# klindsay28/NK_ocn_tracer_jacobian_precond

Measured on AMD Instinct MI355X. Metric: precond_solve_throughput_1deg_ocean_jacobian, higher is better.
Workload: dtype f64

## Files before the change

### include/nkp.h

```cpp
#ifndef NKP_H
#define NKP_H

#include <stdint.h>

#ifdef __cplusplus
extern "C" {
#endif

#define NKP_VERSION 1

typedef struct nkp_solver nkp_solver;

enum nkp_precond {
   NKP_PRECOND_NONE = 0,
   NKP_PRECOND_COLUMN_JACOBI = 1,
   NKP_PRECOND_MULTILEVEL = 3
};

enum nkp_krylov { NKP_KRYLOV_FGMRES = 0, NKP_KRYLOV_BICGSTAB = 1 };

enum {
   NKP_OK = 0,
   NKP_NOT_CONVERGED = 1,
   NKP_BREAKDOWN = 2,
// ... 11 lines not shown
   int ml_pocket;
   int ml_big_from;
   int ml_coarsest_rows;
   int ml_dense_max;
   double ml_theta;
   double ml_tau;
   int64_t ml_device_min;
   int ml_smooth_coarse;
   int ml_coarse_from;
   int ml_gamma_from, ml_gamma_to;
   int ml_f32;
   int ml_host_inverse;
   int ml_fused;
   int ml_fused_max_cols;
   int ml_wave_fused;
   int ml_coarsest_sweeps;
   int64_t ml_tail_rows;
   double ml_omega;
   int col_ldsres;
   int col_stream;
   int col_stream_min;
   int col_stream_gw;
   int col_wave_max;
   int col_w3;
   int col_group;
   int col_pipe_min;
   int col_ldsres_early;
   int col_ldsres_packed;
   int spmv_variant;
   int spmv_compress;
   int spmv_pipe_min;
   int spmv_run;
   int spmv_wgs;
   int rhs_batch;
   int precond_steps;
   int equil;
   int dist_overlap;
   int dist_ras;
   int force_dist;
   int setup_threads;
   int plan_times;
   int ml_drop_intertracer;
   int dist_one_reduce;
   int ml_huge_from;
   int col_ldsres_min;
   int col_sort_groups;
   int batch_spmv_rows;
   int dist_ras_rings;
   int ml_diag;
   int spmv_diag;
   int ml_lane_fused;
   int dist_smooth_exchange;
   int step_glue;
} nkp_tuning;

int nkp_default_tuning (nkp_tuning *t);

typedef struct nkp_options {
   int struct_size;
   int precond;
   int krylov;
   int restart;
   int max_iters;
   double rtol;
   double atol;
   int device;
   int verbose;
   int rank;
   int reorth;
   int ml_levels;
   int ml_smooth;
   int basis_f32;
   int precond_steps;
   int equil;
   int reserved[4];
   const int32_t *col_i;
   const int32_t *col_j;
   const int32_t *col_t;
   const nkp_tuning *tuning;
} nkp_options;

int nkp_default_options (nkp_options *opt);

int nkp_device_count (void);

int nkp_create (nkp_solver **out, const nkp_options *opt, int64_t n, int64_t nnz,
                const int32_t *rowptr, const int32_t *colind, const double *val,
                const int32_t *blk_start, int64_t nblk, int coupled_tracer_cnt);

int nkp_create64 (nkp_solver **out, const nkp_options *opt, int64_t n, const int64_t *rowptr ,
                  const int32_t *colind, const double *val, const int32_t *blk_start, int64_t nblk, int coupled_tracer_cnt);

int nkp_solve (nkp_solver *s, double *b_in_x_out, int nrhs, int64_t ldb,
               double *berr, int *iters, double *relres);

int nkp_solve_batch_device (nkp_solver *s, int nrhs, const void *d_B, void *d_X, int64_t ldb, double *berr, int *iters, double *relres);

int nkp_solve_device (nkp_solver *s, const void *d_b, void *d_x, int use_guess,
                      double *berr, int *iters, double *relres);

int nkp_spmv (nkp_solver *s, const double *x, double *y);
int nkp_spmv_device (nkp_solver *s, const void *d_x, void *d_y);

int nkp_precond_apply (nkp_solver *s, const double *r, double *z);

int nkp_multi_dot (nkp_solver *s, const double *V, int64_t ld, int k, const double *w, double *out);

int nkp_time_kernel (nkp_solver *s, int which, int arg, int reps, double *avg_ms);

int64_t nkp_get_int (nkp_solver *s, const char *key);

#define NKP_REFACTOR_REBUILD 1
int nkp_refactor (nkp_solver *s, const double *val, int flags);
int nkp_refactor_device (nkp_solver *s, const void *d_val, int flags);

int nkp_refactor_dist (nkp_solver *s, const double *val_loc, int flags);
int nkp_refactor_dist_device (nkp_solver *s, const void *d_val_loc, int flags);

int nkp_set_stream (nkp_solver *s, void *hip_stream);

void nkp_destroy (nkp_solver *s);

const char *nkp_last_error (void);


typedef struct nkp_comm_ops {
   void *ctx;
   int rank, nranks;
   int (*allreduce) (void *ctx, void *dev_buf, int count, int op, void *hip_stream);
   int (*alltoallv) (void *ctx, const void *dev_send, const int *send_counts, void *dev_recv, const int *recv_counts, void *hip_stream);
   int (*alltoallv_i32_host) (void *ctx, const int32_t *send, const int *send_counts, int32_t *recv, const int *recv_counts);
   int (*allgather_i64_host) (void *ctx, int64_t mine, int64_t *all );
} nkp_comm_ops;

int nkp_comm_unique_id (void *id128);
int nkp_comm_rccl_init (nkp_comm_ops *ops, const void *id128, int rank, int nranks);
void nkp_comm_rccl_free (nkp_comm_ops *ops);
int nkp_comm_file_init (nkp_comm_ops *ops, const char *dir, int rank, int nranks);
void nkp_comm_file_free (nkp_comm_ops *ops);

int nkp_create_dist (nkp_solver **out, const nkp_options *opt, int64_t n_global, int64_t fst_row,
                     int64_t m_loc, int64_t nnz_loc, const int32_t *rowptr_loc,
                     const int32_t *colind_glob, const double *val,
                     const int32_t *blk_start_loc, int64_t nblk_loc, int coupled_tracer_cnt,
                     const nkp_comm_ops *comm);

int nkp_cell_major_order (int64_t nblk, const int32_t *blk_start, int cnt, int32_t *perm, int32_t *blk_start_new,
                          int32_t *col_t, int32_t *col_src);
int nkp_permuted_rows (int64_t n, const int32_t *rowptr, const int32_t *colind, const double *val, const int32_t *perm,
                       const int32_t *inv, int64_t r0, int64_t r1, int32_t *rowptr_loc, int32_t *colind_loc, double *val_loc);

int nkp_clone (nkp_solver *src, nkp_solver **out);

int nkp_transpose (nkp_solver *s, nkp_solver **out);

// ... 40 lines not shown
```

### nk_ocn_tracer_jacobian_precond_amd/csrc/blas1.hip

```cpp
#include "nkp_dev.h"

#include <stdint.h>

#define B1_THREADS 256

__device__ __forceinline__ double wave_sum (double v)
{
#pragma unroll
   for (int off = NKP_WAVE / 2; off > 0; off >>= 1) v += __shfl_down (v, off);
   return v;
}

__device__ __forceinline__ double block_sum (double v, double *sh )
{
   v = wave_sum (v);
   const int lane = threadIdx.x & (NKP_WAVE - 1), wv = threadIdx.x / NKP_WAVE;
   __syncthreads ();
   if (lane == 0) sh[wv] = v;
   __syncthreads ();
   double s = 0.0;
   if (threadIdx.x == 0) {
#pragma unroll
      for (int w = 0; w < B1_THREADS / NKP_WAVE; w++) s += sh[w];
   }
// ... 161 lines not shown
}

__global__ __launch_bounds__ (B1_THREADS)
void update_w_group_kernel (GsGroup G, int64_t ld, int k, const double *__restrict__ msg, int64_t n)
{
   __shared__ double hs[B1_MAX_K];
   __shared__ double sh[B1_THREADS / NKP_WAVE];
   const int r = blockIdx.y;
   update_w_body<double, double2> (G.V[r], ld, k, msg + (int64_t) r * (k + 1), G.w[r], n, G.partial[r], -1.0, hs, sh);
}

__device__ __forceinline__ void sum_partials_body (const double *__restrict__ partial, int nblk, double *__restrict__ out)
{
   double s = 0.0;
   for (int b = threadIdx.x; b < nblk; b += NKP_WAVE) s += partial[b];
   s = wave_sum (s);
   if (threadIdx.x == 0) out[0] = s;
}

__global__ __launch_bounds__ (NKP_WAVE)
void sum_partials_kernel (const double *__restrict__ partial, int nblk, double *__restrict__ out)
{
   sum_partials_body (partial, nblk, out);
}

__global__ __launch_bounds__ (NKP_WAVE)
void sum_partials_group_kernel (GsGroup G, int nblk, double *__restrict__ out)
{
   sum_partials_body (G.partial[blockIdx.x], nblk, out + blockIdx.x);
}

void launch_update_w (const void *V, int v_f32, int64_t ld, int k, const double *h, double *w, int64_t n, double *partial, double *out_nrm2, hipStream_t st)
{
   const int g = red_grid (n);
   if (v_f32) hipLaunchKernelGGL ((update_w_kernel<float, float2>), dim3 (g), dim3 (B1_THREADS), 0, st, (const float *) V, ld, k, h, w, n, partial, -1.0);
   else hipLaunchKernelGGL ((update_w_kernel<double, double2>), dim3 (g), dim3 (B1_THREADS), 0, st, (const double *) V, ld, k, h, w, n, partial, -1.0);
   if (out_nrm2) hipLaunchKernelGGL (sum_partials_kernel, dim3 (1), dim3 (NKP_WAVE), 0, st, partial, g, out_nrm2);
}

void launch_update_w_group (int R, const GsGroup &G, int64_t ld, int k, const double *msg, int64_t n, double *nrm2, hipStream_t st)
{
   if (R <= 0) return;
   const int g = red_grid (n);
   hipLaunchKernelGGL (update_w_group_kernel, dim3 (g, R), dim3 (B1_THREADS), 0, st, G, ld, k, msg, n);
   hipLaunchKernelGGL (sum_partials_group_kernel, dim3 (R), dim3 (NKP_WAVE), 0, st, G, g, nrm2);
}

void launch_axpy_multi (const double *Z, int64_t ld, int k, const double *c, double *x, int64_t n, hipStream_t st)
{
   const int g = red_grid (n);
   hipLaunchKernelGGL ((update_w_kernel<double, double2>), dim3 (g), dim3 (B1_THREADS), 0, st, Z, ld, k, c, x, n, (double *) nullptr, 1.0);
}

__device__ __forceinline__ void scale_to_body (const double *__restrict__ x, const double *__restrict__ alpha, double *__restrict__ y, float *__restrict__ yf, int64_t n)
{
   const double a = alpha[0];
   const int64_t stride = (int64_t) gridDim.x * B1_THREADS * 2;
   for (int64_t i = ((int64_t) blockIdx.x * B1_THREADS + threadIdx.x) * 2; i < n; i += stride) {
      if (i + 1 < n) {
         double2 v = *reinterpret_cast<const double2 *> (x + i);
         v.x *= a; v.y *= a;
         *reinterpret_cast<double2 *> (y + i) = v;
         if (yf) *reinterpret_cast<float2 *> (yf + i) = make_float2 ((float) v.x, (float) v.y);
      } else {
         y[i] = a * x[i];
         if (yf) yf[i] = (float) (a * x[i]);
      }
   }
}

__global__ __launch_bounds__ (B1_THREADS)
void scale_to_kernel (const double *__restrict__ x, const double *__restrict__ alpha, double *__restrict__ y, float *__restrict__ yf, int64_t n)
{
   scale_to_body (x, alpha, y, yf, n);
}

__global__ __launch_bounds__ (B1_THREADS)
void scale_to_group_kernel (GsGroup G, const double *__restrict__ inv, int64_t n)
{
   const int r = blockIdx.y;
   scale_to_body (G.w[r], inv + r, G.vnext[r], nullptr, n);
}

void launch_scale_to (const double *x, const double *alpha_dev, double *y, float *yf, int64_t n, hipStream_t st)
{
   hipLaunchKernelGGL (scale_to_kernel, dim3 (red_grid (n)), dim3 (B1_THREADS), 0, st, x, alpha_dev, y, yf, n);
}

void launch_scale_to_group (int R, const GsGroup &G, const double *inv, int64_t n, hipStream_t st)
{
   if (R > 0) hipLaunchKernelGGL (scale_to_group_kernel, dim3 (red_grid (n), R), dim3 (B1_THREADS), 0, st, G, inv, n);
}

__global__ __launch_bounds__ (B1_THREADS)
void axpby_kernel (double a, const double *__restrict__ x, double b, double *__restrict__ y, int64_t n)
{
   const int64_t stride = (int64_t) gridDim.x * B1_THREADS;
   for (int64_t i = (int64_t) blockIdx.x * B1_THREADS + threadIdx.x; i < n; i += stride)
      y[i] = (b == 0.0 ? 0.0 : b * y[i]) + (x ? a * x[i] : a);
}

void launch_axpby (double a, const double *x, double b, double *y, int64_t n, hipStream_t st)
{
   hipLaunchKernelGGL (axpby_kernel, dim3 (red_grid (n) * 2), dim3 (B1_THREADS), 0, st, a, x, b, y, n);
}

// ... 340 lines not shown
```

### nk_ocn_tracer_jacobian_precond_amd/csrc/create.hip

```cpp
#include "solver_impl.h"

#include <limits.h>
#include <math.h>
#include <stdlib.h>
#include <string.h>
#include <time.h>

#include <algorithm>
#include <thread>
#include <vector>

void drop_intertracer (int64_t n, int tracer_cnt, const int32_t *rowptr, const int32_t *colind, const double *val,
                       std::vector<int32_t> &f_rowptr, std::vector<int32_t> &f_colind, std::vector<double> &f_val)
{
   const int64_t tsl = n / tracer_cnt;
   f_rowptr.assign ((size_t) n + 1, 0);
   for (int64_t i = 0; i < n; i++) {
      for (int32_t e = rowptr[i]; e < rowptr[i + 1]; e++)
         if (colind[e] / tsl == i / tsl) { f_colind.push_back (colind[e]); f_val.push_back (val[e]); }
      f_rowptr[(size_t) i + 1] = (int32_t) f_colind.size ();
   }
}

static int alloc_work_vectors (nkp_solver *s, bool member = false)
{
   const size_t ld = (size_t) s->ld, m = (size_t) s->m, nscal = 3 * (m + 2) + 16 + 8;
   const struct { double **p; size_t count; } vec[] = {
      { &s->V, ld * (m + 1) }, { &s->vcur, ld }, { &s->Z, ld * m }, { &s->w, ld }, { &s->r, ld }, { &s->x, ld }, { &s->b, ld }, { &s->t1, ld }, { &s->t2, ld },
      { &s->p1, s->precond_steps > 1 ? ld : 0 }, { &s->p2, s->precond_steps > 1 && !member ? ld : 0 }, { &s->eqtmp, s->equil && !member ? ld : 0 },
      { &s->partial, ((m + 1 + NKP_DOT_CHUNK) / NKP_DOT_CHUNK + 1) * NKP_RED_BLOCKS * (NKP_DOT_CHUNK + 1) }, { &s->dscal, nscal } };
   int rc = NKP_OK;
   for (const auto &v : vec)
      if (v.count && (rc = dev_alloc (s, v.p, v.count))) return rc;
   if ((rc = dev_alloc (s, &s->dint, 8))) return rc;
   HIPCHK (hipHostMalloc ((void **) &s->hpin, (m + 16) * sizeof (double), hipHostMallocDefault));
   HIPCHK (hipMemset (s->dscal, 0, nscal * sizeof (double)));
   return NKP_OK;
}

static void build_matrix_diagonals (nkp_solver *s, const int32_t *blk_start, int64_t nblk)
{
   const int64_t n = s->n;
   if (s->tune.spmv_diag <= 0 || !blk_start || nblk <= 0 || nblk >= INT_MAX || n <= 0 || blk_start[0] != 0 || blk_start[nblk] != n) return;
   int max_len = 0;
   for (int64_t c = 0; c < nblk; c++) {
      const int len = blk_start[c + 1] - blk_start[c];
      if (len <= 0) return;
      max_len = std::max (max_len, len);
   }
   void *d_blk = nullptr;
   const size_t bytes = ((size_t) nblk + 1) * sizeof (int);
   if (hipMalloc (&d_blk, bytes) != hipSuccess || hipMemcpy (d_blk, blk_start, bytes, hipMemcpyHostToDevice) != hipSuccess) {
      if (d_blk) (void) hipFree (d_blk);
      (void) hipGetLastError ();
      return;
   }
   int color_tile[3];
   (void) diag_build (s->A, blk_start, (const int *) d_blk, (int) nblk, (int) nblk, max_len, s->tune.spmv_diag, color_tile, &s->device_bytes, s->stream);
   (void) hipFree (d_blk);
}

static int check_arguments (const nkp_options *opt_in, int64_t n, int64_t nnz, const int32_t *rowptr, const int32_t *colind, const double *val,
                            nkp_options &opt, nkp_tuning &tune)
{
   if (opt_in) {
      if (opt_in->struct_size != (int) sizeof (nkp_options)) return fail (NKP_EINVAL, "nkp_create: nkp_options.struct_size mismatch (%d != %zu)", opt_in->struct_size, sizeof (nkp_options));
      opt = *opt_in;
   } else
      nkp_default_options (&opt);
   if (n < 0 || nnz < 0 || !rowptr || (nnz > 0 && (!colind || !val))) return fail (NKP_EINVAL, "nkp_create: bad matrix arguments");
   if (n >= 2147483647LL || nnz >= 2147483647LL) return fail (NKP_EINVAL, "nkp_create: n/nnz exceed the int32 index schema");
   if (rowptr[0] != 0 || rowptr[n] != nnz) return fail (NKP_EINVAL, "nkp_create: rowptr[0]=%d rowptr[n]=%d inconsistent with nnz=%lld", rowptr[0], rowptr[n], (long long) nnz);
   if (opt.restart < 1) opt.restart = 1;
   if (opt.restart > NKP_MAX_K - 2) opt.restart = NKP_MAX_K - 2;
   if (opt.precond != NKP_PRECOND_NONE && opt.precond != NKP_PRECOND_COLUMN_JACOBI && opt.precond != NKP_PRECOND_MULTILEVEL)
      return fail (NKP_EINVAL, "nkp_create: unknown preconditioner %d", opt.precond);
   { const int trc = resolve_tuning (&opt, &tune); if (trc) return trc; }
   opt.tuning = nullptr;
   return NKP_OK;
}

static int check_rows (const nkp_options &opt, int64_t n, const int32_t *rowptr, const int32_t *colind, const double *val)
{
   struct Bad { int64_t row = -1; int kind = 0; int col = 0; };
   const int nt = (n >= 200000) ? (int) std::min (16u, std::max (1u, std::thread::hardware_concurrency ())) : 1;
   std::vector<Bad> bad ((size_t) nt);
   auto check = [&] (int t) {
      const int64_t r0 = n * t / nt, r1 = n * (t + 1) / nt;
      for (int64_t r = r0; r < r1 && bad[(size_t) t].row < 0; r++) {
         Bad b;
         if (rowptr[r + 1] < rowptr[r]) b.kind = 1;
         else {
            double diag = 0.0;
            for (int e = rowptr[r]; e < rowptr[r + 1] && !b.kind; e++) {
               if (colind[e] < 0 || colind[e] >= n) { b.kind = 2; b.col = colind[e]; }
               else if (opt.precond == NKP_PRECOND_MULTILEVEL && e > rowptr[r] && colind[e] <= colind[e - 1]) b.kind = 4;
               else if (colind[e] == r) diag += val[e];
            }
            if (!b.kind && opt.precond != NKP_PRECOND_NONE && !(diag != 0.0)) b.kind = 3;
         }
         if (b.kind) { b.row = r; bad[(size_t) t] = b; }
      }
   };
   if (nt == 1) check (0);
   else {
      std::vector<std::thread> pool;
      for (int t = 0; t < nt; t++) pool.emplace_back (check, t);
      for (std::thread &th : pool) th.join ();
   }
   for (const Bad &b : bad) {
      if (b.row < 0) continue;
      if (b.kind == 1) return fail (NKP_EINVAL, "nkp_create: rowptr decreases at row %lld", (long long) b.row);
// ... 211 lines not shown
         solver_free (s);
         return rc;
      }
   }
   msg (s, 1, "column blocks: %lld blocks, longest %d rows, in-block half bandwidth %d stored as %d%s\n", (long long) nblk,
        s->B.max_len, meas[0], s->B.P, s->B.dropped ? " (entries beyond the band dropped)" : "");
   return NKP_OK;
}

int create_impl (nkp_solver **out, const nkp_options *opt_in, int64_t n, int64_t nnz,
                 const int32_t *rowptr, const int32_t *colind, const double *val,
                 const int32_t *blk_start, int64_t nblk, int coupled_tracer_cnt, const SpmvMatrixHost *spmv_mat,
                 const PrecondMatrixHost *pm)
{
   if (!out) return fail (NKP_EINVAL, "nkp_create: out is NULL");
   *out = nullptr;
   nkp_options opt;
   nkp_tuning tune;
   std::vector<int> blk_default;
   int rc;
   if ((rc = check_arguments (opt_in, n, nnz, rowptr, colind, val, opt, tune))) return rc;
   if ((rc = check_rows (opt, n, rowptr, colind, val))) return rc;
   if ((rc = check_blocks (opt, n, blk_start, nblk, blk_default))) return rc;

   nkp_solver *s = nullptr;
   if ((rc = new_solver_on_device (opt, tune, &s))) return rc;
   struct timespec ts0_;
   clock_gettime (CLOCK_MONOTONIC, &ts0_);
   auto since0 = [&] () { struct timespec t; clock_gettime (CLOCK_MONOTONIC, &t); return (double) (t.tv_sec - ts0_.tv_sec) + 1e-9 * (double) (t.tv_nsec - ts0_.tv_nsec); };
   if ((rc = configure (s, n))) return rc;

   const SpmvMatrixHost own = { nnz, n, rowptr, colind, val };
   const SpmvMatrixHost &M = spmv_mat ? *spmv_mat : own;
   if ((rc = upload_matrix (s, M, spmv_mat != nullptr))) return rc;
   if (!spmv_mat && blk_default.empty ()) build_matrix_diagonals (s, blk_start, nblk);
   if (s->equil && (rc = upload_row_scales (s, M))) return rc;

   const double t_matrix = since0 ();
   s->vf32 = opt.basis_f32 != 0;
   TRY (alloc_work_vectors (s));

   const double t_work = since0 ();
   if (opt.precond != NKP_PRECOND_NONE && !pm) {
      s->h_blk.assign (blk_start, blk_start + nblk + 1);
      s->tracer_cnt = coupled_tracer_cnt;
      if (blk_default.empty ()) {
         if (opt.col_i) s->h_col_i.assign (opt.col_i, opt.col_i + nblk);
         if (opt.col_j) s->h_col_j.assign (opt.col_j, opt.col_j + nblk);
         if (opt.col_t) s->h_col_t.assign (opt.col_t, opt.col_t + nblk);
      }
   }
   if (opt.precond == NKP_PRECOND_MULTILEVEL &&
       (rc = build_hierarchy (s, n, rowptr, colind, val, blk_start, nblk, blk_default.empty (), coupled_tracer_cnt, !spmv_mat, pm))) return rc;
   if (opt.precond == NKP_PRECOND_COLUMN_JACOBI && (rc = factor_columns (s, blk_start, nblk))) return rc;
   TRYHIP (hipStreamSynchronize (s->stream));
   TRYHIP (hipGetLastError ());
   msg (s, 1, "nkp_create: n = %lld, nnz = %lld, %d SpMV row blocks, %.1f MB on device %d; %.2f s matrix upload + row blocks, %.2f s work vectors, %.2f s preconditioner\n",
        (long long) n, (long long) M.nnz, s->A.nrowblk, (double) s->device_bytes / 1.0e6, s->device, t_matrix, t_work - t_matrix, since0 () - t_work);
   s->create_seconds = since0 ();
   *out = s;
   return NKP_OK;
}

extern "C" int nkp_create (nkp_solver **out, const nkp_options *opt, int64_t n, int64_t nnz,
                           const int32_t *rowptr, const int32_t *colind, const double *val,
                           const int32_t *blk_start, int64_t nblk, int coupled_tracer_cnt)
{
   return create_impl (out, opt, n, nnz, rowptr, colind, val, blk_start, nblk, coupled_tracer_cnt, nullptr);
}

extern "C" int nkp_create64 (nkp_solver **out, const nkp_options *opt, int64_t n, const int64_t *rowptr, const int32_t *colind, const double *val,
                             const int32_t *blk_start, int64_t nblk, int coupled_tracer_cnt)
{
   if (!out) return fail (NKP_EINVAL, "nkp_create64: out is NULL");
   *out = nullptr;
   if (n < 0 || !rowptr) return fail (NKP_EINVAL, "nkp_create64: bad matrix arguments");
   if (n >= 2147483647LL || rowptr[n] >= 2147483647LL || rowptr[n] < 0)
      return fail (NKP_EINVAL, "nkp_create64: %lld rows / %lld entries: one GPU stores entry offsets in 32 bits (at most 2^31 - 1 rows and entries); "
                   "row-partition the system with nkp_create_dist, where the limit applies per rank", (long long) n, (long long) rowptr[n]);
   std::vector<int32_t> rp ((size_t) n + 1);
   for (int64_t r = 0; r <= n; r++) {
      if (rowptr[r] < 0 || rowptr[r] > rowptr[n]) return fail (NKP_EINVAL, "nkp_create64: rowptr[%lld] = %lld out of range", (long long) r, (long long) rowptr[r]);
      rp[(size_t) r] = (int32_t) rowptr[r];
   }
   return create_impl (out, opt, n, rowptr[n], rp.data (), colind, val, blk_start, nblk, coupled_tracer_cnt, nullptr);
}

int clone_impl (nkp_solver *src, nkp_solver **out, bool member)
{
   if (!src || !out) return fail (NKP_EINVAL, "nkp_clone: NULL argument");
   *out = nullptr;
   if (src->dist.on && !member) return fail (NKP_EINVAL, "nkp_clone: not available for the row-distributed flavour");
   if (src->borrowed) return fail (NKP_EINVAL, "nkp_clone: clone the original solver, not a clone");
   if (src->trans_of && !member) return fail (NKP_EINVAL, "nkp_clone: not available on a transposed solver (its owner may free it at a refactor)");
   HIPCHK (hipSetDevice (src->device));
   nkp_solver *s = new (std::nothrow) nkp_solver (*src);
   if (!s) return fail (NKP_ENOMEM, "nkp_clone: out of host memory");
   s->borrowed = true;
   s->rf = nullptr;
   s->shared->clones++;
   s->stagnated = false;
   s->batch_members.clear ();
   s->bvin = s->bz = s->bw = nullptr;
   s->batch_K = 0;
   s->dist.bxe = s->dist.gmsg = s->dist.ghpin = nullptr;
   s->dist.each_exchange ([] (RowExchange &X, bool) { X.drop_wide (); });
   s->dist.bK = s->dist.agreed_K = 0;
   s->dplan = nullptr;
   s->trans = s->trans_of = nullptr;
   s->trans_src = nullptr;
   s->trans_val = nullptr;
   s->trans_map_bytes = 0;
   s->trans_ship = nullptr;
   s->trans_send = s->trans_recv = nullptr;
   s->vg = decltype (s->vg) ();
   s->vp = decltype (s->vp) ();
   s->A.tune = &s->tune;
   s->B.tune = &s->tune;
   s->ml.tune = &s->tune;
   for (MlLevel &L : s->ml.lev) L.L.tune = L.B.tune = &s->tune;
   s->stream = nullptr;
   s->own_stream = false;
   s->device_bytes = 0;
   s->V = s->vcur = s->Z = s->w = s->r = s->x = s->b = s->t1 = s->t2 = s->p1 = s->p2 = s->eqtmp = s->partial = s->dscal = s->hpin = nullptr;
   s->dint = nullptr;
   for (MlLevel &L : s->ml.lev) L.x = L.x2 = L.b = L.r = nullptr;
   int rc = NKP_OK;
   TRYHIP (hipStreamCreateWithFlags (&s->stream, hipStreamNonBlocking));
   s->own_stream = true;
   TRY (alloc_work_vectors (s, member));
   for (MlLevel &L : s->ml.lev) {
      TRY (dev_alloc (s, &L.x, (size_t) L.n));
      TRY (dev_alloc (s, &L.x2, (size_t) L.n));
      TRY (dev_alloc (s, &L.b, (size_t) L.n));
      TRY (dev_alloc (s, &L.r, (size_t) L.n));
      TRYHIP (hipMemset (L.x, 0, (size_t) (L.n ? L.n : 1) * sizeof (double)));
      TRYHIP (hipMemset (L.x2, 0, (size_t) (L.n ? L.n : 1) * sizeof (double)));
      TRYHIP (hipMemset (L.b, 0, (size_t) (L.n ? L.n : 1) * sizeof (double)));
      TRYHIP (hipMemset (L.r, 0, (size_t) (L.n ? L.n : 1) * sizeof (double)));
   }
   *out = s;
   return NKP_OK;
}

#undef TRY
#undef TRYHIP

extern "C" int nkp_clone (nkp_solver *src, nkp_solver **out) { return clone_impl (src, out, false); }
```

### nk_ocn_tracer_jacobian_precond_amd/csrc/diagop.hip

```cpp
#include "nkp_dev.h"
#include "diag_rows.h"
#include "mlsetup.h"

#include <limits.h>

#include <vector>

#define DG_THREADS 256
#define DG_WAVES (DG_THREADS / NKP_WAVE)
#define DG_RPL 4
#define DG_UNROLL 8

__global__ __launch_bounds__ (DG_THREADS)
void diag_keys_kernel (int ncol, const int *__restrict__ blk_start, const int *__restrict__ rowptr, const int *__restrict__ colind, int cap,
                       int *__restrict__ tmpkey, int *__restrict__ cnt)
{
   const int c = blockIdx.x * DG_WAVES + (threadIdx.x >> 6), lane = threadIdx.x & (NKP_WAVE - 1);
   if (c >= ncol) return;
   const int r0 = blk_start[c], len = blk_start[c + 1] - r0;
   int p[DG_RPL], e1[DG_RPL], key[DG_RPL];
#pragma unroll
   for (int j = 0; j < DG_RPL; j++) {
      const int kl = lane + j * NKP_WAVE;
      p[j] = e1[j] = 0;
// ... 3 lines not shown
   int n = 0;
   bool bad = false;
   for (;;) {
      int m = key[0];
#pragma unroll
      for (int j = 1; j < DG_RPL; j++) m = min (m, key[j]);
#pragma unroll
      for (int off = NKP_WAVE / 2; off > 0; off >>= 1) m = min (m, __shfl_xor (m, off));
      if (m == INT_MAX) break;
      if (n < cap && lane == 0) tmpkey[(size_t) c * cap + n] = m;
      if (++n > cap) break;
#pragma unroll
      for (int j = 0; j < DG_RPL; j++)
         if (key[j] == m) {
            p[j]++;
            key[j] = p[j] < e1[j] ? colind[p[j]] - (lane + j * NKP_WAVE) : INT_MAX;
            if (key[j] <= m) bad = true;
         }
   }
   if (__any (bad)) n = cap + 1;
   if (lane == 0) cnt[c] = n;
}

__global__ __launch_bounds__ (DG_THREADS)
void diag_compact_kernel (int ncol, int cap, const int *__restrict__ tmpkey, const int *__restrict__ dg_ptr, int *__restrict__ dg_key)
{
   const int64_t t = (int64_t) blockIdx.x * DG_THREADS + threadIdx.x;
   const int c = (int) (t / cap), i = (int) (t % cap);
   if (c >= ncol) return;
   const int k0 = dg_ptr[c];
   if (i < dg_ptr[c + 1] - k0) dg_key[k0 + i] = tmpkey[t];
}

template <class VT>
__global__ __launch_bounds__ (DG_THREADS)
void diag_fill_kernel (int ntile, const DgTile *__restrict__ tile, const int *__restrict__ rowptr, const int *__restrict__ colind,
                       const VT *__restrict__ valf, const int *__restrict__ dg_key, VT *__restrict__ dg_val)
{
   const int t = blockIdx.x * DG_WAVES + (threadIdx.x >> 6), lane = threadIdx.x & (NKP_WAVE - 1);
   if (t >= ntile) return;
   const DgTile T = tile[t];
   if (lane >= T.rows) return;
   const int kl = T.kl0 + lane;
   int p = rowptr[T.row0 + lane];
   const int e1 = rowptr[T.row0 + lane + 1];
   VT *dst = dg_val + T.voff + kl;
   for (int s = 0; s < T.nk; s++) {
      VT v = (VT) 0;
      if (p < e1 && colind[p] - kl == dg_key[T.k0 + s]) v = valf[p++];
      dst[(size_t) s * T.len] = v;
   }
}

template <class VT, int MODE>
__global__ __launch_bounds__ (DG_THREADS)
void diag_residual_kernel (const DgTile *__restrict__ tile, int ntile, const DgGroup *__restrict__ dg_grp, const VT *__restrict__ dg_val,
                           const double *__restrict__ x, const double *__restrict__ b, double *__restrict__ y, int n)
{
   const int t = __builtin_amdgcn_readfirstlane (blockIdx.x * DG_WAVES + (threadIdx.x >> 6));
   if (t >= ntile) return;
   const DgTile T = tile[t];
   const int lane = threadIdx.x & (NKP_WAVE - 1);
   const int lr = min (lane, T.rows - 1);
   double bv = 0.0;
   if constexpr (MODE == 1) bv = b[T.row0 + lr];
   const double acc = dg_row_sum<VT, false> (T, dg_grp, dg_val, lane, lr, x, n);
   if (lane < T.rows) y[T.row0 + lane] = MODE == 1 ? bv - acc : acc;
}

template <int P, bool R32>
__global__ __launch_bounds__ (DG_THREADS)
void gs_wave_diag_kernel (const DgTile *__restrict__ tile, int ntile, const DgGroup *__restrict__ dg_grp, const float *__restrict__ dg_val, int64_t n,
                          const double *__restrict__ fac, const double *__restrict__ xa, const double *__restrict__ xb, int split,
                          const double *__restrict__ b, double *__restrict__ xout)
{
   const int t = __builtin_amdgcn_readfirstlane (blockIdx.x * DG_WAVES + (threadIdx.x >> 6));
   if (t >= ntile) return;
   const DgTile T = tile[t];
   const int lane = threadIdx.x & (NKP_WAVE - 1);
   const bool own = lane < T.rows;
   const int lr = min (lane, T.rows - 1);
   const int64_t r = T.row0 + lr;
   const double bv = b[r];
   const double xold = r < split ? xa[r] : xb[r];
   double f[2 * P + 1];
#pragma unroll
   for (int d = 0; d <= 2 * P; d++) {
      f[d] = fac[(int64_t) d * n + r];
      if (R32) f[d] = (double) (float) f[d];
   }
   const double acc = dg_row_sum<float, true> (T, dg_grp, dg_val, lane, lr, xa, (int) n, xb, split);
   double y[1][1], invd[1], L[1][P], U[1][P];
   y[0][0] = own ? bv - acc : 0.0;
   invd[0] = own ? f[P] : 0.0;
#pragma unroll
   for (int q = 1; q <= P; q++) {
      L[0][q - 1] = own ? f[P - q] : 0.0;
      U[0][q - 1] = own ? f[P + q] : 0.0;
   }
   wave_band_sweeps<P, 1, 1> (T.rows, lane, y, invd, L, U);
   if (own) xout[T.row0 + lane] = xold + y[0][0];
}

static void diag_drop (CsrDev &L, size_t *device_bytes, size_t held)
{
   for (void **p : { (void **) &L.dg_ptr, (void **) &L.dg_key, (void **) &L.dg_voff, (void **) &L.dg_val, (void **) &L.dg_vald, (void **) &L.dg_tile, (void **) &L.dg_gptr, (void **) &L.dg_grp })
      if (*p) { (void) hipFree (*p); *p = nullptr; }
   L.dg_ntile = L.dg_ncol = L.dg_nkey = L.dg_ngrp = 0;
   L.dg_nval = 0;
   *device_bytes -= held;
   (void) hipGetLastError ();
}

static inline int dg_col_tiles (int len) { return (len + NKP_WAVE - 1) / NKP_WAVE; }

static void dg_groups (const int *key, int nk, int rows, std::vector<DgGroup> &out)
{
   const int fit = NKP_WAVE - rows + 1, lim = fit < DG_RUN_MAX ? fit : DG_RUN_MAX;
   for (int s = 0; s < nk;) {
      int m = 1;
      while (s + m < nk && m < lim && key[s + m] == key[s + m - 1] + 1) m++;
      DgGroup R;
      R.key0 = key[s];
      R.slots = s | m << 16;
      out.push_back (R);
      s += m;
   }
}

int diag_build (CsrDev &L, const int *h_blk_start, const int *d_blk_start, int ncol, int ncol0, int max_len, int cap, int color_tile[3],
                size_t *device_bytes, hipStream_t st)
{
   color_tile[0] = color_tile[1] = color_tile[2] = 0;
   const bool f64 = !L.valf;
   if (cap <= 0 || (f64 && !L.val) || ncol <= 0 || L.nnz <= 0 || max_len > DG_RPL * NKP_WAVE) return 0;
   if (cap > 4096) cap = 4096;
   if ((int64_t) ncol * cap > INT_MAX) return 0;
   mls::DBuf<int> tmpkey, dcnt;
   if (tmpkey.alloc ((size_t) ncol * cap) != hipSuccess || dcnt.alloc ((size_t) ncol) != hipSuccess) { (void) hipGetLastError (); return 0; }
   hipLaunchKernelGGL (diag_keys_kernel, dim3 ((ncol + DG_WAVES - 1) / DG_WAVES), dim3 (DG_THREADS), 0, st, ncol, d_blk_start, (const int *) L.rowptr,
                       (const int *) L.colind, cap, tmpkey.p, dcnt.p);
   std::vector<int> cnt ((size_t) ncol);
   if (hipMemcpyAsync (cnt.data (), dcnt.p, (size_t) ncol * sizeof (int), hipMemcpyDeviceToHost, st) != hipSuccess || hipStreamSynchronize (st) != hipSuccess) {
      (void) hipGetLastError ();
      return 0;
   }
   std::vector<int> ptr ((size_t) ncol + 1, 0);
   std::vector<long long> voff ((size_t) ncol);
   long long nval = 0, ntile = 0;
   for (int c = 0; c < ncol; c++) {
      if (cnt[c] > cap) return 0;
      const int len = h_blk_start[c + 1] - h_blk_start[c];
      ptr[c + 1] = ptr[c] + cnt[c];
      voff[c] = nval;
      nval += (long long) cnt[c] * len;
      ntile += dg_col_tiles (len);
   }
   if (2 * nval > 3 * (long long) L.nnz || ntile == 0 || ntile > INT_MAX) return 0;
   size_t held = 0;
   auto put = [&] (void **dst, const void *src, size_t bytes) {
      void *q = nullptr;
      if (hipMalloc (&q, bytes ? bytes : 1) != hipSuccess) return false;
      *dst = q;
      held += bytes ? bytes : 1;
      *device_bytes += bytes ? bytes : 1;
      return !src || !bytes || hipMemcpyAsync (q, src, bytes, hipMemcpyHostToDevice, st) == hipSuccess;
   };
   auto give_up = [&] () {
      (void) hipStreamSynchronize (st);
      diag_drop (L, device_bytes, held);
      color_tile[0] = color_tile[1] = color_tile[2] = 0;
      return 0;
   };
   if (!(put ((void **) &L.dg_ptr, ptr.data (), ptr.size () * sizeof (int)) && put ((void **) &L.dg_key, nullptr, ((size_t) ptr[ncol] + DG_UNROLL) * sizeof (int)) &&
         put ((void **) &L.dg_voff, voff.data (), voff.size () * sizeof (long long)) && (f64 ? put ((void **) &L.dg_vald, nullptr, (size_t) nval * sizeof (double)) : put ((void **) &L.dg_val, nullptr, (size_t) nval * sizeof (float)))))
      return give_up ();
   (void) hipMemsetAsync (L.dg_key + ptr[ncol], 0, DG_UNROLL * sizeof (int), st);
   const int64_t slots = (int64_t) ncol * cap;
   hipLaunchKernelGGL (diag_compact_kernel, dim3 ((unsigned) ((slots + DG_THREADS - 1) / DG_THREADS)), dim3 (DG_THREADS), 0, st, ncol, cap, (const int *) tmpkey.p,
                       (const int *) L.dg_ptr, L.dg_key);
// ... 18 lines not shown
         tiles.push_back (T);
         kl0 += T.rows;
      }
   }
   if (ncol0 >= ncol) color_tile[1] = (int) tiles.size ();
   color_tile[2] = (int) tiles.size ();
   if (!(put ((void **) &L.dg_gptr, gptr.data (), gptr.size () * sizeof (int)) && put ((void **) &L.dg_grp, grp.data (), grp.size () * sizeof (DgGroup)) &&
         put ((void **) &L.dg_tile, tiles.data (), tiles.size () * sizeof (DgTile))))
      return give_up ();
   L.dg_ntile = (int) tiles.size ();
   L.dg_ncol = ncol;
   L.dg_nkey = ptr[ncol];
   L.dg_ngrp = (int) grp.size ();
   L.dg_nval = nval;
   launch_diag_fill (L, st);
   if (hipStreamSynchronize (st) != hipSuccess) return give_up ();
   return 1;
}

void launch_diag_fill (const CsrDev &L, hipStream_t st)
{
   if (!(L.dg_val || L.dg_vald) || L.dg_ntile <= 0) return;
   const dim3 grid ((L.dg_ntile + DG_WAVES - 1) / DG_WAVES);
   if (L.dg_vald)
      hipLaunchKernelGGL (diag_fill_kernel<double>, grid, dim3 (DG_THREADS), 0, st, L.dg_ntile, (const DgTile *) L.dg_tile, (const int *) L.rowptr,
                          (const int *) L.colind, (const double *) L.val, (const int *) L.dg_key, L.dg_vald);
   else
      hipLaunchKernelGGL (diag_fill_kernel<float>, grid, dim3 (DG_THREADS), 0, st, L.dg_ntile, (const DgTile *) L.dg_tile, (const int *) L.rowptr,
                          (const int *) L.colind, (const float *) L.valf, (const int *) L.dg_key, L.dg_val);
}

void launch_diag_residual (const CsrDev &L, int tile0, int tile1, const double *x, const double *b, double *y, hipStream_t st)
{
   const int cnt = tile1 - tile0;
   if (cnt <= 0) return;
   hipLaunchKernelGGL ((diag_residual_kernel<float, 1>), dim3 ((cnt + DG_WAVES - 1) / DG_WAVES), dim3 (DG_THREADS), 0, st, (const DgTile *) L.dg_tile + tile0, cnt,
                       (const DgGroup *) L.dg_grp, (const float *) L.dg_val, x, b, y, (int) L.n);
}

void launch_gs_wave_diag (const CsrDev &L, const ColBlocksDev &B, int tile0, int tile1, const double *xa, const double *xb, int split, const double *b,
                          double *xout, int r32, hipStream_t st)
{
   const int cnt = tile1 - tile0;
   if (cnt <= 0) return;
   with_band (B.P, [&] (auto p) {
      with_bool (r32, [&] (auto r32_) {
         hipLaunchKernelGGL ((gs_wave_diag_kernel<decltype (p)::value, decltype (r32_)::value>), dim3 ((cnt + DG_WAVES - 1) / DG_WAVES), dim3 (DG_THREADS), 0, st,
                             (const DgTile *) L.dg_tile + tile0, cnt, (const DgGroup *) L.dg_grp, (const float *) L.dg_val, B.n, (const double *) B.fac, xa, xb,
                             split, b, xout);
      });
   });
}

void launch_diag_spmv (const CsrDev &A, const double *x, double *y, const double *b, int mode, hipStream_t st)
{
   if (A.dg_ntile <= 0 || !A.dg_vald) return;
   const dim3 grid ((A.dg_ntile + DG_WAVES - 1) / DG_WAVES);
   with_bool (mode == 1, [&] (auto residual) {
      hipLaunchKernelGGL ((diag_residual_kernel<double, decltype (residual)::value ? 1 : 0>), grid, dim3 (DG_THREADS), 0, st, (const DgTile *) A.dg_tile, A.dg_ntile,
                          (const DgGroup *) A.dg_grp, (const double *) A.dg_vald, x, b, y, (int) A.n);
   });
}
```

### nk_ocn_tracer_jacobian_precond_amd/csrc/inspect.hip

```cpp
#include "solver_impl.h"

#include <string.h>

#include <vector>

extern "C" int64_t nkp_ml_level_array (nkp_solver *s, int level, const char *what, void *dst, int64_t capacity_bytes)
{
   if (!s || !what || s->opt.precond != NKP_PRECOND_MULTILEVEL || level < 0 || level >= (int) s->ml.lev.size ()) return fail (NKP_EINVAL, "nkp_ml_level_array: bad argument");
   const MlLevel &V = s->ml.lev[(size_t) level];
   const bool last = level == (int) s->ml.lev.size () - 1;
   const void *src = nullptr;
   int64_t count = 0;
   size_t elem = 4;
   bool host = false;
   int col_kernel[11];
   if (!strcmp (what, "rowptr")) { src = V.L.rowptr; count = V.n + 1; }
   else if (!strcmp (what, "colind")) { src = V.L.colind; count = V.L.nnz; }
   else if (!strcmp (what, "valf")) { src = V.L.valf; count = V.L.valf ? V.L.nnz : 0; }
   else if (!strcmp (what, "val")) { src = V.L.val; count = V.L.val ? V.L.nnz : 0; elem = 8; }
   else if (!strcmp (what, "dg_ptr")) { src = V.L.dg_ptr; count = src ? V.L.dg_ncol + 1 : 0; }
   else if (!strcmp (what, "dg_key")) { src = V.L.dg_key; count = src ? (int64_t) V.L.dg_nkey : 0; }
   else if (!strcmp (what, "dg_voff")) { src = V.L.dg_voff; count = src ? V.L.dg_ncol : 0; elem = 8; }
   else if (!strcmp (what, "dg_val")) { src = V.L.dg_val; count = src ? V.L.dg_nval : 0; }
   else if (!strcmp (what, "dg_gptr")) { src = V.L.dg_gptr; count = src ? V.L.dg_ncol + 1 : 0; }
   else if (!strcmp (what, "dg_grp")) { src = V.L.dg_grp; count = src ? 2 * (int64_t) V.L.dg_ngrp : 0; }
   else if (!strcmp (what, "cmap")) { src = V.cmap; count = V.cmap ? V.n : 0; }
   else if (!strcmp (what, "rptr")) { src = V.rptr; count = V.rptr ? V.nc + 1 : 0; }
   else if (!strcmp (what, "ridx")) { src = V.ridx; count = V.ridx ? V.n : 0; }
   else if (!strcmp (what, "blk_start")) { src = V.B.blk_start; count = V.B.blk_start ? V.B.nblk + 1 : 0; }
   else if (!strcmp (what, "fac")) { src = V.B.fac; count = V.B.fac ? (int64_t) (2 * V.B.P + 1) * V.n : 0; elem = 8; }
   else if (!strcmp (what, "perm0")) { src = level == 0 ? s->ml.perm0 : nullptr; count = src ? V.n : 0; }
   else if (!strcmp (what, "coarse_inv")) { src = last ? s->ml.coarse_inv : nullptr; count = src ? V.n * V.n : 0; elem = 8; }
   else if (!strcmp (what, "color_blk")) { src = V.B.blk_start ? V.color_blk : nullptr; count = src ? 3 : 0; host = true; }
   else if (!strcmp (what, "col_kernel")) {
      const ColBlocksDev &B = V.B;
      const int v[11] = { V.wave_columns ? 1 : 0, V.wave_fused ? 1 : 0, B.stream ? 1 : 0, B.ldsres, B.gw, B.P, B.dropped, B.max_len, B.gs_ok, B.ngrp, B.lds_doubles };
      memcpy (col_kernel, v, sizeof v);
      src = B.blk_start ? col_kernel : nullptr; count = src ? 11 : 0; host = true;
   }
   else if (!strcmp (what, "wave_diag")) { src = &V.wave_diag; count = 1; host = true; }
   else if (!strcmp (what, "lane_diag")) { src = &V.lane_diag; count = 1; host = true; }
   else if (!strcmp (what, "grp_tile")) { src = V.B.grp_tile; count = src ? (int64_t) V.B.ngrp * V.B.gw : 0; }
   else return fail (NKP_EINVAL, "nkp_ml_level_array: unknown array '%s'", what);
   if (!dst) return count;
   if (count * (int64_t) elem > capacity_bytes) return fail (NKP_EINVAL, "nkp_ml_level_array: buffer too small");
   if (host) {
      if (count) memcpy (dst, src, (size_t) count * elem);
      return count;
   }
   HIPCHK (hipSetDevice (s->device));
   HIPCHK (hipStreamSynchronize (s->stream));
   if (count) HIPCHK (hipMemcpy (dst, src, (size_t) count * elem, hipMemcpyDeviceToHost));
   return count;
}

extern "C" int64_t nkp_matrix_array (nkp_solver *s, const char *what, void *dst, int64_t capacity_bytes)
{
   if (!s || !what) return fail (NKP_EINVAL, "nkp_matrix_array: bad argument");
   const CsrDev &A = s->A;
   const bool have = A.dg_vald != nullptr;
   const void *src = nullptr;
   int64_t count = 0;
   size_t elem = 4;
   if (!strcmp (what, "dg_ptr")) { src = A.dg_ptr; count = have ? A.dg_ncol + 1 : 0; }
   else if (!strcmp (what, "dg_key")) { src = A.dg_key; count = have ? (int64_t) A.dg_nkey : 0; }
   else if (!strcmp (what, "dg_voff")) { src = A.dg_voff; count = have ? A.dg_ncol : 0; elem = 8; }
   else if (!strcmp (what, "dg_val")) { src = A.dg_vald; count = have ? A.dg_nval : 0; elem = 8; }
   else if (!strcmp (what, "dg_gptr")) { src = A.dg_gptr; count = have ? A.dg_ncol + 1 : 0; }
   else if (!strcmp (what, "dg_grp")) { src = A.dg_grp; count = have ? 2 * (int64_t) A.dg_ngrp : 0; }
   else if (!strcmp (what, "rowptr")) { src = A.rowptr; count = src ? A.n + 1 : 0; }
   else if (!strcmp (what, "colind")) { src = A.colind; count = src ? A.nnz : 0; }
   else if (!strcmp (what, "val")) { src = A.val; count = src ? A.nnz : 0; elem = 8; }
   else if (!strcmp (what, "fac")) { src = s->opt.precond == NKP_PRECOND_COLUMN_JACOBI ? s->B.fac : nullptr; count = src ? (int64_t) (2 * s->B.P + 1) * s->B.n : 0; elem = 8; }
   else return fail (NKP_EINVAL, "nkp_matrix_array: unknown array '%s'", what);
   if (!dst) return count;
   if (count * (int64_t) elem > capacity_bytes) return fail (NKP_EINVAL, "nkp_matrix_array: buffer too small");
   HIPCHK (hipSetDevice (s->device));
   HIPCHK (hipStreamSynchronize (s->stream));
   if (count) HIPCHK (hipMemcpy (dst, src, (size_t) count * elem, hipMemcpyDeviceToHost));
   return count;
}

extern "C" int nkp_spmv_device (nkp_solver *s, const void *d_x, void *d_y)
{
   if (!s || !d_x || !d_y) return fail (NKP_EINVAL, "nkp_spmv_device: NULL argument");
   HIPCHK (hipSetDevice (s->device));
   spmv_op (s, (const double *) d_x, (double *) d_y, nullptr, 0);
   HIPCHK (hipStreamSynchronize (s->stream));
   HIPCHK (hipGetLastError ());
   return NKP_OK;
}

extern "C" int nkp_spmv (nkp_solver *s, const double *x, double *y)
{
   if (!s || !x || !y) return fail (NKP_EINVAL, "nkp_spmv: NULL argument");
   HIPCHK (hipSetDevice (s->device));
   const size_t bytes = (size_t) s->n * sizeof (double);
   HIPCHK (hipMemcpyAsync (s->t1, x, bytes, hipMemcpyHostToDevice, s->stream));
   spmv_op (s, s->t1, s->t2, nullptr, 0);
   HIPCHK (hipMemcpyAsync (y, s->t2, bytes, hipMemcpyDeviceToHost, s->stream));
   HIPCHK (hipStreamSynchronize (s->stream));
   HIPCHK (hipGetLastError ());
   return NKP_OK;
}

extern "C" int nkp_precond_apply (nkp_solver *s, const double *r, double *z)
{
   if (!s || !r || !z) return fail (NKP_EINVAL, "nkp_precond_apply: NULL argument");
   if (s->shared->broken) return refactor_broken (s);
   HIPCHK (hipSetDevice (s->device));
   const size_t bytes = (size_t) s->n * sizeof (double);
   HIPCHK (hipMemcpyAsync (s->t1, r, bytes, hipMemcpyHostToDevice, s->stream));
   apply_precond_once (s, s->t1, s->t2);
   HIPCHK (hipMemcpyAsync (z, s->t2, bytes, hipMemcpyDeviceToHost, s->stream));
   HIPCHK (hipStreamSynchronize (s->stream));
   HIPCHK (hipGetLastError ());
   return NKP_OK;
}

extern "C" int nkp_multi_dot (nkp_solver *s, const double *V, int64_t ld, int k, const double *w, double *out)
{
   if (!s || !V || !w || !out || k < 0 || k > s->m + 1 || ld < s->n) return fail (NKP_EINVAL, "nkp_multi_dot: bad argument (k must be <= restart+1)");
   HIPCHK (hipSetDevice (s->device));
   std::vector<float> vf;
   for (int j = 0; j < k; j++) {
      if (s->vf32) {
         vf.assign (V + (int64_t) j * ld, V + (int64_t) j * ld + s->n);
         HIPCHK (hipMemcpyAsync ((float *) s->V + (int64_t) j * s->ld, vf.data (), (size_t) s->n * sizeof (float), hipMemcpyHostToDevice, s->stream));
         HIPCHK (hipStreamSynchronize (s->stream));
      } else
         HIPCHK (hipMemcpyAsync (s->V + (int64_t) j * s->ld, V + (int64_t) j * ld, (size_t) s->n * sizeof (double), hipMemcpyHostToDevice, s->stream));
   }
   HIPCHK (hipMemcpyAsync (s->w, w, (size_t) s->n * sizeof (double), hipMemcpyHostToDevice, s->stream));
   launch_multi_dot (s->V, s->vf32, s->ld, k, s->w, s->n, s->partial, s->h_dev (), s->stream);
   allreduce_dev (s, s->h_dev (), k + 1, 0);
   HIPCHK (hipMemcpyAsync (out, s->h_dev (), (size_t) (k + 1) * sizeof (double), hipMemcpyDeviceToHost, s->stream));
   HIPCHK (hipStreamSynchronize (s->stream));
   HIPCHK (hipGetLastError ());
   return NKP_OK;
}

extern "C" int nkp_time_kernel (nkp_solver *s, int which, int arg, int reps, double *avg_ms)
{
   if (!s || !avg_ms || reps < 1) return fail (NKP_EINVAL, "nkp_time_kernel: bad argument");
   if (which == 8 && !s->A.dg_vald) return fail (NKP_EINVAL, "nkp_time_kernel: the matrix has no per-column diagonals (tuning spmv_diag)");
   HIPCHK (hipSetDevice (s->device));
   if (which == 5) {
      const int prc = valgrad_time_prepare (s, arg);
      if (prc) return prc;
   }
   if (which == 6 || which == 7) {
      const int prc = valprod_time_prepare (s, arg, which);
      if (prc) return prc;
   }
   StepEvent step_ev;
   if (which == 2) {
      const int erc = step_ev.make (s);
      if (erc) return erc;
   }
   hipEvent_t e0, e1;
   HIPCHK (hipEventCreate (&e0));
   HIPCHK (hipEventCreate (&e1));
   launch_fill (s->t1, 1.0, s->n, s->stream);
   if (which == 2) {
      if (arg < 0 || arg >= s->m) return fail (NKP_EINVAL, "nkp_time_kernel: restart position out of range");
      for (int j = 0; j <= arg + 1; j++) {
         launch_fill (s->t2, 1.0 / (1.0 + j), s->n, s->stream);
         s->hpin[0] = 1.0;
         HIPCHK (hipMemcpyAsync (s->misc_dev () + 1, s->hpin, sizeof (double), hipMemcpyHostToDevice, s->stream));
         if (s->vf32) launch_scale_to (s->t2, s->misc_dev () + 1, s->vcur, (float *) s->V + (int64_t) j * s->ld, s->n, s->stream);
         else launch_scale_to (s->t2, s->misc_dev () + 1, s->V + (int64_t) j * s->ld, nullptr, s->n, s->stream);
         HIPCHK (hipStreamSynchronize (s->stream));
      }
   }
   for (int pass = 0; pass < 2; pass++) {
      const int cnt = pass == 0 ? (reps < 3 ? reps : 3) : reps;
      HIPCHK (hipEventRecord (e0, s->stream));
      for (int i = 0; i < cnt; i++) {
         if (which == 0 && s->A.dg_vald) launch_csr_spmv (s->A, s->t1, s->t2, nullptr, 0, s->stream);
         else if (which == 0) spmv_op (s, s->t1, s->t2, nullptr, 0);
         else if (which == 8) launch_diag_spmv (s->A, s->t1, s->t2, nullptr, 0, s->stream);
         else if (which == 1) apply_precond_once (s, s->t1, s->t2);
         else if (which == 2) {
            const int src = arnoldi_hand_over (s, arg, step_ev.ev);
            if (src) { s->ml.entered = 0; return src; }
         }
         else if (which == 5) valgrad_time_launch (s, arg);
         else if (which == 6) valprod_time_launch (s, arg);
         else if (which == 7) valprod_time_composition (s, arg);
         else if (s->opt.precond == NKP_PRECOND_MULTILEVEL) ml_time_piece (s->ml, which - 3, s->stream);
      }
      HIPCHK (hipEventRecord (e1, s->stream));
      HIPCHK (hipEventSynchronize (e1));
      float ms = 0.f;
      HIPCHK (hipEventElapsedTime (&ms, e0, e1));
      *avg_ms = (double) ms / cnt;
   }
   (void) hipEventDestroy (e0);
   (void) hipEventDestroy (e1);
   s->ml.entered = 0;
   HIPCHK (hipGetLastError ());
   return NKP_OK;
}
```

### nk_ocn_tracer_jacobian_precond_amd/csrc/krylov.hip

```cpp
#include "solver_impl.h"

#include <math.h>

void apply_precond_once (nkp_solver *s, const double *rin, double *zout)
{
   if (s->opt.precond == NKP_PRECOND_NONE) launch_copy (rin, zout, s->n, s->stream);
   else if (s->opt.precond == NKP_PRECOND_MULTILEVEL && s->dist.ras) {
      RowExchange &X = s->dist.ras_sep ? s->dist.x_ras : s->dist.x_halo;
      if (X.nsend) launch_gather (X.send_idx, rin, X.send, X.nsend, s->stream);
      exchange_rows (s, X, 1, X.send, s->dist.ras_sep ? s->dist.rext + s->n : halo_rows_of (s, 1), s->stream);
      launch_copy (rin, s->dist.rext, s->n, s->stream);
      if (!s->dist.ras_sep && s->dist.n_sel) launch_gather (s->dist.sel_idx, s->dist.xe + s->n, s->dist.rext + s->n, s->dist.n_sel, s->stream);
      ml_apply (s->ml, s->dist.rext, s->dist.zext, s->stream, smooth_hook_of (s));
      launch_copy (s->dist.zext, zout, s->n, s->stream);
   } else if (s->opt.precond == NKP_PRECOND_MULTILEVEL) ml_apply (s->ml, rin, zout, s->stream);
   else launch_colblock_apply_lanes (s->B, 0, s->B.ngrp, rin, zout, 0, s->stream);
}

void apply_precond (nkp_solver *s, const double *rin, double *zout)
{
   apply_precond_once (s, rin, zout);
   for (int k = 1; k < s->steps_now && s->p1 && s->p2; k++) {
      spmv_op (s, zout, s->p1, rin, 1);
      apply_precond_once (s, s->p1, s->p2);
      launch_axpby (1.0, s->p2, 1.0, zout, s->n, s->stream);
   }
}

void spmv_op (nkp_solver *s, const double *x, double *y, const double *b, int mode)
{
   const double *xin = x;
   if (s->dist.on) {
      xin = s->dist.xe;
      if (s->dist.overlap) {
         halo_product_overlapped (s, 1, x, [&] (int rb0, int rb1) { launch_csr_spmv_range (s->A, rb0, rb1, xin, y, b, mode, s->stream); });
         return;
      }
      halo_fetch (s, 1, x, nullptr, s->stream);
   }
   if (mode == 2) launch_csr_abs_spmv (s->A, xin, b, y, s->stream);
   else if (s->A.dg_vald) launch_diag_spmv (s->A, xin, y, b, mode, s->stream);
   else launch_csr_spmv (s->A, xin, y, b, mode, s->stream);
}

static int dot_host (nkp_solver *s, const double *x, const double *y, double *out)
{
   launch_dot (x, y, s->n, s->partial, s->misc_dev () + 2, s->stream);
   allreduce_dev (s, s->misc_dev () + 2, 1, 0);
   HIPCHK (hipMemcpyAsync (s->hpin, s->misc_dev () + 2, sizeof (double), hipMemcpyDeviceToHost, s->stream));
   HIPCHK (hipStreamSynchronize (s->stream));
   if (s->comm_failed) return fail (NKP_ECOMM, "nkp_solve: a collective of the distributed solve failed");
   *out = s->hpin[0];
   return NKP_OK;
}

void arnoldi_apply (nkp_solver *s, int j)
{
   const int64_t ld = s->ld;
   double *zj = s->Z + (int64_t) j * ld;
   const double *vj = s->vf32 ? s->vcur : s->V + (int64_t) j * ld;
   if (s->ml.entered) {
      ml_finish (s->ml, zj, s->stream);
      spmv_op (s, zj, s->w, nullptr, 0);
      return;
   }
   if (s->equil) {
      launch_vmul (vj, s->rinv, s->eqtmp, s->n, s->stream);
      apply_precond (s, s->eqtmp, zj);
      spmv_op (s, zj, s->w, nullptr, 0);
      launch_vmul (s->w, s->rscale, s->w, s->n, s->stream);
   } else {
      apply_precond (s, vj, zj);
      spmv_op (s, zj, s->w, nullptr, 0);
   }
}

static void arnoldi_column (nkp_solver *s, int j, double *host_col = nullptr)
{
   const int64_t ld = s->ld;
   launch_multi_dot (s->V, s->vf32, ld, j + 1, s->w, s->n, s->partial, s->h_dev (), s->stream);
   allreduce_dev (s, s->h_dev (), j + 2, 0);
   launch_update_w (s->V, s->vf32, ld, j + 1, s->h_dev (), s->w, s->n, s->partial, host_col && !s->opt.reorth ? nullptr : s->misc_dev (), s->stream);
   if (s->opt.reorth) {
      launch_multi_dot (s->V, s->vf32, ld, j + 1, s->w, s->n, s->partial, s->h2_dev (), s->stream);
      allreduce_dev (s, s->h2_dev (), j + 2, 0);
      launch_update_w (s->V, s->vf32, ld, j + 1, s->h2_dev (), s->w, s->n, s->partial, host_col ? nullptr : s->misc_dev (), s->stream);
      allreduce_dev (s, s->misc_dev (), 1, 0);
      if (host_col) launch_finish_column_host (s->h_dev (), s->h2_dev (), j + 1, s->partial, s->n, s->misc_dev (), s->misc_dev () + 1, host_col, s->stream);
      else launch_finish_column (s->h_dev (), s->h2_dev (), j + 1, s->misc_dev (), s->misc_dev () + 1, s->stream);
   } else if (s->dist.on && s->tune.dist_one_reduce) {
      launch_finish_column_pythagoras (s->h_dev (), j + 1, s->misc_dev () + 1, s->stream);
   } else if (host_col) launch_finish_column_host (s->h_dev (), nullptr, j + 1, s->partial, s->n, s->misc_dev (), s->misc_dev () + 1, host_col, s->stream);
   else {
      allreduce_dev (s, s->misc_dev (), 1, 0);
      launch_finish_column (s->h_dev (), nullptr, j + 1, s->misc_dev (), s->misc_dev () + 1, s->stream);
   }
}

static void arnoldi_normalise (nkp_solver *s, int j)
{
   const int64_t ld = s->ld;
   if (s->vf32) launch_scale_to (s->w, s->misc_dev () + 1, s->vcur, (float *) s->V + (int64_t) (j + 1) * ld, s->n, s->stream);
   else launch_scale_to (s->w, s->misc_dev () + 1, s->V + (int64_t) (j + 1) * ld, nullptr, s->n, s->stream);
}

void arnoldi_orthogonalise (nkp_solver *s, int j)
{
   arnoldi_column (s, j);
   arnoldi_normalise (s, j);
}

static bool step_enters_cycle (const nkp_solver *s)
{
   return s->opt.precond == NKP_PRECOND_MULTILEVEL && !s->dist.on && !s->vf32 && !s->equil && s->steps_now == 1 &&
          !s->ml.lev.empty () && s->ml.lev[0].n == s->n;
}

int arnoldi_hand_over (nkp_solver *s, int j, hipEvent_t ev)
{
   const bool early = ev && (s->tune.step_glue & 8) && j + 1 < s->m && !s->dist.on && !s->equil && s->steps_now == 1;
   arnoldi_apply (s, j);
   arnoldi_column (s, j, early ? s->hpin : nullptr);
   if (early) HIPCHK (hipEventRecord (ev, s->stream));
   if (early && step_enters_cycle (s)) ml_enter (s->ml, s->w, s->misc_dev () + 1, s->V + (int64_t) (j + 1) * s->ld, s->stream);
   else arnoldi_normalise (s, j);
   if (early) HIPCHK (hipEventSynchronize (ev));
   else {
      HIPCHK (hipMemcpyAsync (s->hpin, s->h_dev (), (size_t) (j + 2) * sizeof (double), hipMemcpyDeviceToHost, s->stream));
      HIPCHK (hipStreamSynchronize (s->stream));
   }
   return NKP_OK;
}

int StepEvent::make (const nkp_solver *s)
{
   if (!ev && (s->tune.step_glue & 8) && !s->dist.on) HIPCHK (hipEventCreateWithFlags (&ev, hipEventDisableTiming | hipEventReleaseToSystem));
   return NKP_OK;
}

StepEvent::~StepEvent ()
{
   if (ev) (void) hipEventDestroy (ev);
}


int rhs_refused (int verdict, const char *what)
{
   if (verdict == RHS_NONFINITE) return fail (NKP_BREAKDOWN, "%s holds a non-finite entry (NaN or Inf): not solved, x is NaN", what);
   return fail (NKP_BREAKDOWN, "%s is outside the range of the solve (||b||^2 finite in f64 and max (rtol ||b||, atol) >= 2^-480 = 3.2e-145): "
                               "not solved, x is NaN; scale the system", what);
}

static int classify_rhs (nkp_solver *s, double bnorm2, double target, int *verdict)
{
   double nonfinite = 0.0, nonzero = 0.0;
   if (rhs_needs_counts (bnorm2, target)) {
      launch_count_entries (s->b, s->n, s->partial, s->misc_dev () + 4, s->stream);
      allreduce_dev (s, s->misc_dev () + 4, 2, 0);
      HIPCHK (hipMemcpyAsync (s->hpin, s->misc_dev () + 4, 2 * sizeof (double), hipMemcpyDeviceToHost, s->stream));
      HIPCHK (hipStreamSynchronize (s->stream));
      if (s->comm_failed) return fail (NKP_ECOMM, "nkp_solve: a collective of the distributed solve failed");
      nonfinite = s->hpin[0];
      nonzero = s->hpin[1];
   }
   s->rhs_class = *verdict = rhs_verdict (bnorm2, target, nonfinite, nonzero);
   if (*verdict == RHS_ZERO) launch_fill (s->x, 0.0, s->n, s->stream);
   else if (*verdict != RHS_ORDINARY) launch_fill (s->x, NAN, s->n, s->stream);
   return NKP_OK;
}

int fg_begin (nkp_solver *s, FgmresState &F)
{
   fg_init (F, s->m);
   double bnorm2 = 0.0;
   int rc = dot_host (s, s->b, s->b, &bnorm2);
   if (rc) return rc;
   F.bnorm = sqrt (bnorm2);
   F.target = fmax (s->opt.rtol * F.bnorm, s->opt.atol);
   s->stagnated = false;
   s->steps_now = s->precond_steps;
   int verdict = RHS_ORDINARY;
   if ((rc = classify_rhs (s, bnorm2, F.target, &verdict))) return rc;
   if (verdict != RHS_ORDINARY) {
      F.finished = true;
      F.status = verdict == RHS_ZERO ? NKP_OK : NKP_BREAKDOWN;
      F.relres = verdict == RHS_ZERO ? 0.0 : NAN;
   }
   return NKP_OK;
}

int fg_restart (nkp_solver *s, FgmresState &F)
{
   hipStream_t st = s->stream;
   const int64_t n = s->n;
   int rc;
   s->ml.entered = 0;
   spmv_op (s, s->x, s->r, s->b, 1);
   double r2 = 0.0;
   if ((rc = dot_host (s, s->r, s->r, &r2))) return rc;
   const double beta = sqrt (r2);
   const int todo = fg_restart_verdict (F, beta, s->opt.max_iters, s->steps_now);
   msg (s, 2, "fgmres: its = %d, true relres = %.3e\n", F.its, F.relres);
   if (s->comm_failed) return fail (NKP_ECOMM, "nkp_solve: a collective of the distributed solve failed");
   if (todo & FG_LOWER_STEPS) {
      msg (s, 1, "fgmres: no progress over a restart cycle with %d preconditioner cycles per iteration; continuing with one\n", s->steps_now);
      s->steps_now = 1;
   }
   if (todo & FG_STAGNATED) s->stagnated = true;
   if (todo & FG_STOP) return NKP_OK;
   if (s->equil) {
      launch_vmul (s->r, s->rscale, s->r, n, st);
      double q2 = 0.0;
      if ((rc = dot_host (s, s->r, s->r, &q2))) return rc;
      F.beta_it = sqrt (q2);
      if (!(F.beta_it > 0.0)) { F.status = NKP_BREAKDOWN; F.finished = true; return NKP_OK; }
      F.target_it = F.target * (F.beta_it / beta);
   }
   s->hpin[0] = 1.0 / F.beta_it;
   HIPCHK (hipMemcpyAsync (s->misc_dev () + 1, s->hpin, sizeof (double), hipMemcpyHostToDevice, st));
   if (s->vf32) launch_scale_to (s->r, s->misc_dev () + 1, s->vcur, (float *) s->V, n, st);
   else launch_scale_to (s->r, s->misc_dev () + 1, s->V, nullptr, n, st);
   HIPCHK (hipStreamSynchronize (st));
   fg_start_cycle (F);
   return NKP_OK;
}

bool fg_post_step (nkp_solver *s, FgmresState &F)
{
   const bool ends = fg_column_step (F, s->hpin, s->opt.max_iters);
   if (!F.breakdown_in_cycle) msg (s, 3, "fgmres: its = %d, est relres = %.3e\n", F.its, F.est / F.bnorm);
   return ends;
}

int fg_end_cycle (nkp_solver *s, FgmresState &F)
{
   const int k = F.j;
   hipStream_t st = s->stream;
   fg_back_substitute (F);
   for (int i = 0; i < k; i++) s->hpin[i] = F.y[i];
   HIPCHK (hipMemcpyAsync (s->y_dev (), s->hpin, (size_t) k * sizeof (double), hipMemcpyHostToDevice, st));
   launch_axpy_multi (s->Z, s->ld, k, s->y_dev (), s->x, s->n, st);
   HIPCHK (hipStreamSynchronize (st));
   if (F.breakdown_in_cycle) {
      int rc;
      double r2 = 0.0;
      spmv_op (s, s->x, s->r, s->b, 1);
      if ((rc = dot_host (s, s->r, s->r, &r2))) return rc;
      F.relres = is_finite (r2) ? sqrt (r2) / F.bnorm : NAN;
      F.status = sqrt (r2) <= F.target ? NKP_OK : NKP_BREAKDOWN;
      F.finished = true;
   }
   return NKP_OK;
}

static int fgmres (nkp_solver *s, int *iters_out, double *relres_out)
{
   FgmresState F;
   StepEvent ev;
   int rc = fg_begin (s, F);
   if (rc) return rc;
   if ((rc = ev.make (s))) return rc;
   while (!F.finished) {
      if ((rc = fg_restart (s, F))) return rc;
      if (F.finished) break;
      for (;;) {
         if ((rc = arnoldi_hand_over (s, F.j, ev.ev))) { s->ml.entered = 0; return rc; }
         if (s->comm_failed) return fail (NKP_ECOMM, "nkp_solve: a collective of the distributed solve failed (Arnoldi step %d)", F.its + 1);
         if (fg_post_step (s, F)) break;
      }
      if ((rc = fg_end_cycle (s, F))) return rc;
   }
   s->ml.entered = 0;
   HIPCHK (hipGetLastError ());
   *iters_out = F.its;
   *relres_out = F.relres;
   return F.status;
}

static int bicgstab (nkp_solver *s, int *iters_out, double *relres_out)
{
   const int64_t n = s->n, ld = s->ld;
   hipStream_t st = s->stream;
   if (s->m < 2) return fail (NKP_EINVAL, "bicgstab needs restart >= 2 (it borrows the Krylov basis storage)");
   double *r = s->r, *r0 = s->V, *p = s->V + ld, *v = s->V + 2 * ld;
   double *ph = s->Z, *sh = s->Z + ld, *t = s->t2, *sv = s->t1;
   int rc;
   double bnorm2, rho = 1.0, alpha = 1.0, omega = 1.0, tmp;
   if ((rc = dot_host (s, s->b, s->b, &bnorm2))) return rc;
   const double bnorm = sqrt (bnorm2);
   const double target = fmax (s->opt.rtol * bnorm, s->opt.atol);
   int verdict = RHS_ORDINARY;
   if ((rc = classify_rhs (s, bnorm2, target, &verdict))) return rc;
   if (verdict != RHS_ORDINARY) {
      *iters_out = 0;
      *relres_out = verdict == RHS_ZERO ? 0.0 : NAN;
      return verdict == RHS_ZERO ? NKP_OK : NKP_BREAKDOWN;
   }
   spmv_op (s, s->x, r, s->b, 1);
   launch_copy (r, r0, n, st);
   launch_fill (p, 0.0, n, st);
   launch_fill (v, 0.0, n, st);
   int its = 0, status = NKP_NOT_CONVERGED;
   double rn2;
   if ((rc = dot_host (s, r, r, &rn2))) return rc;
   double relres = sqrt (rn2) / bnorm;
   while (its < s->opt.max_iters) {
      if (!is_finite (rn2)) { status = NKP_BREAKDOWN; break; }
      if (sqrt (rn2) <= target) { status = NKP_OK; break; }
      double rho_new;
      if ((rc = dot_host (s, r0, r, &rho_new))) return rc;
      if (rho_new == 0.0 || !(rho_new == rho_new)) { status = NKP_BREAKDOWN; break; }
      const double beta = (rho_new / rho) * (alpha / omega);
      launch_axpby (-omega, v, 1.0, p, n, st);
      launch_axpby (1.0, r, beta, p, n, st);
      apply_precond (s, p, ph);
      spmv_op (s, ph, v, nullptr, 0);
      if ((rc = dot_host (s, r0, v, &tmp))) return rc;
      if (tmp == 0.0 || !(tmp == tmp)) { status = NKP_BREAKDOWN; break; }
      alpha = rho_new / tmp;
      launch_copy (r, sv, n, st);
      launch_axpby (-alpha, v, 1.0, sv, n, st);
      apply_precond (s, sv, sh);
      spmv_op (s, sh, t, nullptr, 0);
      double ts, tt;
      if ((rc = dot_host (s, t, sv, &ts))) return rc;
// ... 122 lines not shown
```

### nk_ocn_tracer_jacobian_precond_amd/csrc/mlcycle.hip

```cpp
#include "nkp_dev.h"
#include "multilevel.h"

static void column_solves (const MlHierarchy &H, MlLevel &V, int c, const double *rhs, double *x, int accumulate, hipStream_t st)
{
   if (V.wave_columns) {
      if (H.f32) launch_colblock_apply_range_r32 (V.B, V.color_blk[c], V.color_blk[c + 1], rhs, x, accumulate, st);
      else launch_colblock_apply_range (V.B, V.color_blk[c], V.color_blk[c + 1], rhs, x, accumulate, st);
   } else
      launch_colblock_apply_lanes (V.B, V.color_grp[c], V.color_grp[c + 1], rhs, x, accumulate, st);
}

static inline void after_half_sweep (MlHierarchy &H, const MlLevel &V, int c, double *x, int K, hipStream_t st)
{
   if (!H.hook || &V != &H.lev[0] || H.hook_left <= 0) return;
   if (--H.hook_left > 0) H.hook->refresh (H.hook->ctx, c, x, K, st);
}

static void gs_half (MlHierarchy &H, MlLevel &V, int c, bool fused, hipStream_t st)
{
   if (fused) {
      const int out = (V.cur[0] != V.cur[1]) ? V.cur[1 - c] : 1 - V.cur[c];
      const int rows0 = (int) V.rows0;
      if (V.wave_diag) launch_gs_wave_diag (V.L, V.B, V.color_tile[c], V.color_tile[c + 1], V.xbuf (V.cur[0]), V.xbuf (V.cur[1]), rows0, V.b, V.xbuf (out), H.f32, st);
      else if (V.lane_diag) launch_gs_lanes_diag (V.L, V.B, V.color_grp[c], V.color_grp[c + 1], V.xbuf (V.cur[0]), V.xbuf (V.cur[1]), rows0, V.b, V.xbuf (out), st);
// ... 27 lines not shown
   }
}

static inline bool ml_level_fills_x (const MlHierarchy &H, int l)
{
   if (l == H.tail_from) return false;
   return !(l == (int) H.lev.size () - 1 && H.coarse_inv);
}

enum { ML_FRESH = 0, ML_FILLED = 1, ML_SOLVED = 2 };

static void ml_cycle (MlHierarchy &H, int l, hipStream_t st, int started = ML_FRESH)
{
   MlLevel &V = H.lev[l];
   if (started != ML_SOLVED) V.cur[0] = V.cur[1] = 0;
   if (l == 0) H.hook_left = 0;
   if (l == H.tail_from && H.coarse_inv && H.gamma_to <= H.gamma_from && ml_tail_launch (H, l, st) == 0) return;
   if (l == (int) H.lev.size () - 1) {
      if (H.coarse_inv) {
         if (H.coarse_invf) launch_dense_matvec_f32 (H.coarse_invf, H.coarse_ldf, V.b, V.x, (int) V.n, st);
         else launch_dense_matvec (H.coarse_inv, V.b, V.x, (int) V.n, st);
         return;
      }
      const int sweeps = H.tune->ml_coarsest_sweeps > 0 ? H.tune->ml_coarsest_sweeps : 30;
      if (started == ML_FRESH) launch_fill (V.x, 0.0, V.n, st);
      column_solves (H, V, 0, V.b, V.x, 0, st);
      gs_half (H, V, 1, false, st);
      for (int s = 1; s < sweeps; s++) gs_sweep (H, V, s & 1, false, st);
      return;
   }
   const bool fused = ml_level_fused (H, V);
   const int nu = (l >= H.coarse_from) ? H.nu_coarse : H.nu;
   if (l == 0 && H.hook) H.hook_left = 4 * nu;
   if (started == ML_FRESH) launch_fill (V.x, 0.0, V.n, st);
   if (started != ML_SOLVED) first_half_sweep (H, V, fused, st);
   gs_half (H, V, 1, fused, st);
   for (int s = 1; s < nu; s++) gs_sweep (H, V, false, fused, st);
   MlLevel &C = H.lev[l + 1];
   const int gamma = (l >= H.gamma_from && l < H.gamma_to) ? 2 : 1;
   for (int g = 0; g < gamma; g++) {
      if (V.L.dg_val) launch_diag_residual (V.L, V.color_tile[0], V.color_tile[2], V.xnow (), V.b, V.r, st);
      else launch_csr_spmv (V.L, V.xnow (), V.r, V.b, 1, st);
      const bool fill = (H.tune->step_glue & 4) && ml_level_fills_x (H, l + 1);
      launch_restrict_sum (V.rptr, V.ridx, V.r, C.b, V.nc, st, fill ? C.x : nullptr);
      ml_cycle (H, l + 1, st, fill ? ML_FILLED : ML_FRESH);
      launch_prolong_add (V.cmap, C.xnow (), V.xnow (), V.n, H.omega, st);
   }
   for (int s = 0; s < nu; s++) gs_sweep (H, V, true, fused, st);
}

void ml_apply (MlHierarchy &H, const double *r, double *z, hipStream_t st, const MlSmoothHook *hook)
{
   MlLevel &V = H.lev[0];
   launch_gather (H.perm0, r, V.b, V.n, st);
   H.hook = hook;
   ml_cycle (H, 0, st);
   H.hook = nullptr;
   launch_scatter (H.perm0, V.xnow (), z, V.n, st);
}

void ml_enter (MlHierarchy &H, const double *w, const double *inv, double *vnext, hipStream_t st)
{
   MlLevel &V = H.lev[0];
   launch_cycle_entry (H.perm0, w, inv, vnext, V.b, V.x, V.n, st);
   H.entered = ML_FILLED;
   if (H.lev.size () >= 2 && H.tail_from != 0) {
      V.cur[0] = V.cur[1] = 0;
      H.hook_left = 0;
      first_half_sweep (H, V, ml_level_fused (H, V), st);
      H.entered = ML_SOLVED;
   }
}

void ml_finish (MlHierarchy &H, double *z, hipStream_t st)
{
   MlLevel &V = H.lev[0];
   const int started = H.entered;
   H.entered = ML_FRESH;
   ml_cycle (H, 0, st, started);
   launch_scatter (H.perm0, V.xnow (), z, V.n, st);
}

int ml_batch_prepare (MlHierarchy &H, int K)
{
   if (K != 2 && K != 4 && K != 8) return -1;
   if (H.batch_K >= K) return 0;
   auto drop = [&H] () {
      for (MlLevel &V : H.lev)
         for (double **p : { &V.bx, &V.bx2, &V.bb, &V.br })
            if (*p) {
               (void) hipFree (*p);
               *p = nullptr;
               H.device_bytes -= (size_t) (V.n ? V.n : 1) * (size_t) H.batch_K * sizeof (double);
            }
      H.batch_K = 0;
   };
   drop ();
   for (MlLevel &V : H.lev) {
      for (double **p : { &V.bx, &V.bx2, &V.bb, &V.br }) {
         const size_t bytes = (size_t) (V.n ? V.n : 1) * (size_t) K * sizeof (double);
         void *q = nullptr;
         if (hipMalloc (&q, bytes) != hipSuccess || hipMemset (q, 0, bytes) != hipSuccess) {
            if (q) (void) hipFree (q);
            H.batch_K = K;
            drop ();
            (void) hipGetLastError ();
            return -2;
         }
         *p = (double *) q;
         H.device_bytes += bytes;
      }
   }
   H.batch_K = K;
   return 0;
}

static void column_solves_batch (const MlHierarchy &H, MlLevel &V, int K, int c, const double *rhs, double *x, int accumulate, hipStream_t st)
{
   if (launch_colblock_apply_lanes_batch (K, V.B, V.color_grp[c], V.color_grp[c + 1], rhs, x, accumulate, st) != 0)
      launch_colblock_apply_wave_batch (K, V.B, V.color_blk[c], V.color_blk[c + 1], rhs, x, accumulate, H.f32, st);
}

static void gs_half_batch (MlHierarchy &H, MlLevel &V, int K, int c, hipStream_t st)
{
   if (V.wave_fused) {
      const int out = (V.bcur[0] != V.bcur[1]) ? V.bcur[1 - c] : 1 - V.bcur[c];
      launch_gs_wave_batch (K, V.L, V.B, V.color_blk[c], V.color_blk[c + 1], V.bxbuf (V.bcur[0]), V.bxbuf (V.bcur[1]), (int) V.rows0, V.bb, V.bxbuf (out), H.f32, st);
      V.bcur[c] = out;
      after_half_sweep (H, V, c, V.bxbuf (out), K, st);
      return;
   }
   launch_csr_spmv_batch (K, V.L, V.color_rb[c], V.color_rb[c + 1], V.bx, V.br, V.bb, 1, st);
   column_solves_batch (H, V, K, c, V.br, V.bx, 1, st);
// ... 132 lines not shown
```

### nk_ocn_tracer_jacobian_precond_amd/csrc/multilevel.h

```cpp
#pragma once
#include "nkp_dev.h"

#include <vector>

struct MlLevel {
   int64_t n = 0;
   CsrDev L;
   ColBlocksDev B;
   int color_rb[3] = { 0, 0, 0 };
   int color_blk[3] = { 0, 0, 0 };
   int color_grp[3] = { 0, 0, 0 };
   int color_tile[3] = { 0, 0, 0 };
   int64_t rows0 = 0;
   int wave_columns = 0;
   int wave_fused = 0;
   int wave_diag = 0;
   int lane_diag = 0;
   int64_t nc = 0;
   int *cmap = nullptr;
   int *rptr = nullptr, *ridx = nullptr;
   double *x = nullptr, *b = nullptr, *r = nullptr;
   double *x2 = nullptr;
   int cur[2] = { 0, 0 };
   double *bx = nullptr, *bx2 = nullptr, *bb = nullptr, *br = nullptr;
   int bcur[2] = { 0, 0 };
   double *bxbuf (int k) { return k ? bx2 : bx; }
   double *bxnow () { return bxbuf (bcur[0]); }
   std::vector<int> nat_inv;
   double *xbuf (int k) { return k ? x2 : x; }
   double *xnow () { return xbuf (cur[0]); }
};

struct MlSmoothHook {
   void (*refresh) (void *ctx, int colour, double *x, int K, hipStream_t st);
   void *ctx;
};

struct MlHierarchy {
   std::vector<MlLevel> lev;
   const MlSmoothHook *hook = nullptr;
   int hook_left = 0;
   int entered = 0;
   int *perm0 = nullptr;
   double *coarse_inv = nullptr;
   float *coarse_invf = nullptr;
   int coarse_ldf = 0;
   int nu = 1;
   int nu_coarse = 1;
   int coarse_from = 2;
   int f32 = 1;
   int fused = 1;
   int tail_from = -1;
   int gamma_from = 0, gamma_to = 0;
   double omega = 1.1;
   const nkp_tuning *tune = nullptr;
   size_t device_bytes = 0;
   double setup_seconds = 0.0;
   int levels_on_device = 0;
   int inverse_pivoted = 0;
   int batch_K = 0;
   int default_build = 0;
};

inline bool ml_level_fused (const MlHierarchy &H, const MlLevel &V)
{
   const int fused_max = H.tune->ml_fused_max_cols;
   return V.wave_fused || V.lane_diag || (H.fused && V.B.gs_ok && (fused_max <= 0 || V.color_grp[2] * V.B.gw <= fused_max));
}

int ml_setup (MlHierarchy &H, int64_t n, const int *rowptr, const int *colind, const double *val,
              const int *blk_start, int64_t nblk, const int *col_i, const int *col_j, const int *col_t ,
              int tracer_cnt, int max_levels, int nu, int coarsest_rows, int verbose, int rank,
              hipStream_t st, char *err, size_t errlen, const nkp_tuning &tune, const CsrDev *A_dev = nullptr );
void ml_free (MlHierarchy &H);
int ml_coarse_inverse (const MlHierarchy &H, int n, const int *prow, const int *pcol, const double *pval, double **inv, float **invf,
                       int *ldf, size_t *bytes, hipStream_t st);
inline int ml_level0_sweeps (const MlHierarchy &H) { return 0 >= H.coarse_from ? H.nu_coarse : H.nu; }
inline bool ml_level0_hookable (const MlHierarchy &H) { return H.lev.size () >= 2 && H.tail_from != 0 && ml_level0_sweeps (H) > 0; }
void ml_apply (MlHierarchy &H, const double *r, double *z, hipStream_t st, const MlSmoothHook *hook = nullptr);
void ml_enter (MlHierarchy &H, const double *w, const double *inv, double *vnext, hipStream_t st);
void ml_finish (MlHierarchy &H, double *z, hipStream_t st);
int ml_batch_prepare (MlHierarchy &H, int K);
void ml_apply_batch (MlHierarchy &H, int K, const double *r, double *z, hipStream_t st);
void ml_apply_batch_split (MlHierarchy &H, int K, const double *const *src, double *z, double *const *dst, hipStream_t st, const double *src_scale = nullptr);
void ml_apply_batch_split_ext (MlHierarchy &H, int K, const double *const *src, const double *halo, const int *sel, int64_t n_own, double *z,
                               double *const *dst, hipStream_t st, const MlSmoothHook *hook = nullptr);
void ml_time_piece (MlHierarchy &H, int which, hipStream_t st);
int64_t ml_bytes (const MlHierarchy &H, int which);
int ml_tail_launch (MlHierarchy &H, int l0, hipStream_t st);
```

### nk_ocn_tracer_jacobian_precond_amd/csrc/multilevel.hip

```cpp
#include "nkp_dev.h"
#include "multilevel.h"
#include "mlsetup.h"
#include "ml_plan.h"
#include "../../include/nkp.h"

#include <stdio.h>
#include <stdlib.h>

#include <chrono>
#include <vector>

using namespace mlp;

namespace {

template <class T>
bool upload (T **dst, const T *src, size_t count, size_t *bytes)
{
   void *q = nullptr;
   const size_t b = (count ? count : 1) * sizeof (T);
   if (hipMalloc (&q, b) != hipSuccess) return false;
   if (count && src && hipMemcpy (q, src, count * sizeof (T), hipMemcpyHostToDevice) != hipSuccess) { (void) hipFree (q); return false; }
   *dst = (T *) q;
   *bytes += b;
// ... 443 lines not shown
      hnat.resize (1);
      init_first_nat (hnat[0], n, rowptr, colind, val, blk_start_in, nblk, col_i, col_j, col_t, tracer_cnt, true, K, TH);
      extend_nat_levels (hnat, 0, (int) nblk, tracer_cnt, max_levels, coarsest_rows, verbose, rank, K, TH);
   }
   const double t_plan = secs_since (t_begin);

   const int nlev = l0 + (int) hnat.size ();
   H.lev.resize (nlev);
   for (int l = l0; l < nlev; l++) {
      const int frc = finalize_host_level (H, l, nlev, hnat[(size_t) (l - l0)], l + 1 < nlev ? &hnat[(size_t) (l - l0 + 1)] : nullptr, K, verbose, rank, st, err, errlen, T);
      if (frc) return frc;
   }
   {
      const int64_t cap = tune.ml_tail_rows;
      H.tail_from = -1;
      int64_t rows = 0;
      for (int l = nlev - 1; l >= 0 && nlev - l <= 8; l--) {
         rows += H.lev[l].n;
         if (rows > cap) break;
         if (l < nlev - 1) H.tail_from = l;
      }
      if (verbose && H.tail_from >= 0) printf ("(%d) multilevel: levels %d..%d run as one single-workgroup launch\n", rank, H.tail_from, nlev - 1);
   }
   H.setup_seconds = secs_since (t_begin);
   H.levels_on_device = ndev_levels;
   H.default_build = device_ok && !tune.ml_host_inverse;
   if (verbose) {
      printf ("(%d) multilevel setup: %d of %d levels built on the device (%.3f s twin, %.3f s coarse cells, %.3f s Galerkin products); host levels: %.3f s twin, %.3f s "
              "column graphs + coarse cells, %.3f s Galerkin products; colour-major operators %.3f s, row blocks %.3f, uploads + f32 copies %.3f, column factors %.3f, "
              "lane layouts %.3f, transfer maps %.3f; hierarchy construction as a whole %.3f s, everything %.3f s\n",
              rank, ndev_levels, nlev, T.twin, T.agg, T.galerkin, TH.low, TH.graph, TH.galerkin, T.perm, T.rb, T.up, T.fac, T.lay, T.map, t_plan, H.setup_seconds);
      fflush (stdout);
   }
   return 0;
}
#undef ML_FAIL

int ml_coarse_inverse (const MlHierarchy &H, int n, const int *prow, const int *pcol, const double *pval, double **inv, float **invf,
                       int *ldf, size_t *bytes, hipStream_t st)
{
   *inv = nullptr;
   *invf = nullptr;
   const int brc = dense_inverse_blocked_device (n, prow, pcol, pval, inv, H.f32 ? invf : nullptr, ldf, bytes, st);
   if (brc < 0) return -2;
   if (brc == 0) return 0;
   std::vector<double> dense ((size_t) n * n, 0.0);
   for (int64_t i = 0; i < n; i++)
      for (int e = prow[i]; e < prow[i + 1]; e++) dense[(size_t) i * n + pcol[e]] = pval[e];
   return dense_inverse_device (n, dense, inv, bytes, st) ? 1 : -4;
}

void ml_free (MlHierarchy &H)
{
   for (MlLevel &V : H.lev) {
      void *ptrs[] = { V.L.rowptr, V.L.colind, V.L.val, V.L.valf, V.B.fac_tf, V.L.rowblk, V.L.codes, V.L.dict, V.L.dict_ptr, V.L.dg_ptr, V.L.dg_key, V.L.dg_voff, V.L.dg_val, V.L.dg_tile, V.L.dg_gptr, V.L.dg_grp, V.B.blk_start, V.B.fac, V.B.grp_b0, V.B.grp_nb, V.B.grp_maxlen, V.B.grp_base, V.B.grp_row0, V.B.col_slot, V.B.fac_t, V.B.gs_rb_ptr, V.B.gs_rb, V.B.wave_desc, V.B.grp_tile, V.cmap, V.rptr, V.ridx, V.x, V.x2, V.b, V.r, V.bx, V.bx2, V.bb, V.br };
      for (void *p : ptrs)
         if (p) (void) hipFree (p);
      delete V.B.grp_cols;
   }
   H.lev.clear ();
   if (H.perm0) (void) hipFree (H.perm0);
   if (H.coarse_inv) (void) hipFree (H.coarse_inv);
   if (H.coarse_invf) (void) hipFree (H.coarse_invf);
   H.coarse_invf = nullptr;
   H.perm0 = nullptr;
   H.coarse_inv = nullptr;
}
```

### nk_ocn_tracer_jacobian_precond_amd/csrc/nkp_dev.h

```cpp
#pragma once
#include <hip/hip_runtime.h>
#include <stdint.h>

#include "../../include/nkp.h"
#include "col_plan.h"
#include "tuning.h"

#include <type_traits>
#include <utility>
#include <vector>

#define NKP_WAVE 64
#define NKP_MAX_K 512
#define NKP_SPMV_LDS_NNZ 2048
#define NKP_SPMV_MAX_ROWS 256

struct alignas (16) DgTile {
   int row0, rows;
   int kl0, len;
   int k0, nk;
   int g0, ng;
   long long voff;
};
struct DgGroup {
   int key0;
   int slots;
};
#define DG_RUN_MAX 5

struct CsrDev {
   int64_t n = 0, nnz = 0;
   int *rowptr = nullptr;
   int *colind = nullptr;
   double *val = nullptr;
   float *valf = nullptr;
   int *rowblk = nullptr;
   int nrowblk = 0;
   unsigned short *codes = nullptr;
   int *dict = nullptr;
   int *dict_ptr = nullptr;
   int *dg_ptr = nullptr;
   int *dg_key = nullptr;
   long long *dg_voff = nullptr;
   float *dg_val = nullptr;
   double *dg_vald = nullptr;
   DgTile *dg_tile = nullptr;
   int *dg_gptr = nullptr;
   DgGroup *dg_grp = nullptr;
   int dg_ntile = 0, dg_ncol = 0, dg_nkey = 0, dg_ngrp = 0;
   int64_t dg_nval = 0;
   const nkp_tuning *tune = nullptr;
};

double build_spmv_codes_host (int64_t n, const int *rowptr, const int *colind, const int *rowblk, int nrowblk,
                              unsigned short **codes_out, int **dict_out, int *ndict_out, int **dict_ptr_out);
int attach_spmv_codes (CsrDev &A, const int *h_rowptr, const int *h_colind, const int *h_rowblk, size_t *device_bytes);

void launch_csr_spmv (const CsrDev &A, const double *x, double *y, const double *b, int mode, hipStream_t st);
void launch_csr_residual_range (const CsrDev &A, int rb0, int rb1, const double *x, const double *b, double *y, hipStream_t st);
void launch_csr_spmv_range (const CsrDev &A, int rb0, int rb1, const double *x, double *y, const double *b, int mode, hipStream_t st);
void launch_csr_abs_spmv (const CsrDev &A, const double *x, const double *b, double *y, hipStream_t st);
int diag_build (CsrDev &L, const int *h_blk_start, const int *d_blk_start, int ncol, int ncol0, int max_len, int cap, int color_tile[3],
                size_t *device_bytes, hipStream_t st);
void launch_diag_fill (const CsrDev &L, hipStream_t st);
void launch_diag_residual (const CsrDev &L, int tile0, int tile1, const double *x, const double *b, double *y, hipStream_t st);
void launch_diag_spmv (const CsrDev &A, const double *x, double *y, const double *b, int mode, hipStream_t st);
void build_rowblocks_host (int64_t n, const int *rowptr, int **rowblk_out, int *nrowblk_out);

void launch_value_gradient (int K, int nk, const CsrDev &A, const double *lam, const double *x, double alpha, int accumulate, double *g, hipStream_t st);
void launch_values_product (int K, int nk, const CsrDev &A, const double *val, const double *x, double alpha, int accumulate, double *y, int64_t ldy, hipStream_t st);

struct ColBlocksDev {
   int64_t n = 0;
   int nblk = 0;
   int *blk_start = nullptr;
   int P = 0;
   int max_len = 0;
   int dropped = 0;
   double *fac = nullptr;
   int ngrp = 0;
   int *grp_b0 = nullptr;
   int *grp_nb = nullptr;
   int *grp_maxlen = nullptr;
   long long *grp_base = nullptr;
   int *grp_row0 = nullptr;
   int *col_slot = nullptr;
   double *fac_t = nullptr;
   float *fac_tf = nullptr;
   int lds_doubles = 0;
   int gw = 64;
   int rhs_slots = 0;
   int stream = 0;
   int ldsres = 0;
   int gs_ok = 0;
   int gs_lds_bytes = 0;
   int *gs_rb_ptr = nullptr;
   int *gs_rb = nullptr;
   int *wave_desc = nullptr;
   int *grp_tile = nullptr;
   int grp_tile_cnt = 0;
   const nkp_tuning *tune = nullptr;
   int ml_level = 0;
   ColKernel kern;
   std::vector<int> *grp_cols = nullptr;
};


template <int V> using int_tag = std::integral_constant<int, V>;
template <int V0, int... Vs, class F>
inline auto with_int (int v, F &&f)
{
   if constexpr (sizeof... (Vs) == 0) return f (int_tag<V0> ());
   else {
      if (v == V0) return f (int_tag<V0> ());
      return with_int<Vs...> (v, f);
   }
}
template <class F> inline auto with_band (int P, F &&f) { return with_int<1, 2, 4> (P, f); }
template <class F> inline auto with_k (int K, F &&f) { return with_int<2, 4, 8> (K, f); }
// ... 71 lines not shown
         for (int j = 0; j < K; j++) {
            v[j] = c[j] * invd[s0];
            bc[j] = readlane_const_f64<l0> (v[j]);
         }
         if (k > 0) {
            constexpr int s1 = (k > 0 ? k - 1 : 0) / NKP_WAVE;
#pragma unroll
            for (int j = 0; j < K; j++) c[j] = y[s1][j] - U[s1][0] * bc[j];
         }
#pragma unroll
         for (int j = 0; j < K; j++) y[s0][j] = lane == l0 ? v[j] : y[s0][j];
#pragma unroll
         for (int q = 2; q <= P; q++)
            if (k - q >= 0) {
               const int s = (k - q) / NKP_WAVE, l = (k - q) % NKP_WAVE;
#pragma unroll
               for (int j = 0; j < K; j++) {
                  const double u = y[s][j] - U[s][q - 1] * bc[j];
                  y[s][j] = lane == l ? u : y[s][j];
               }
            }
      }
   });
}

int colblock_build_lane_layout (ColBlocksDev &B, const int *h_blk_start, const int *ranges, int nranges,
                                int *grp_first, size_t *device_bytes, hipStream_t st, int f32 = 0, const int *h_rowptr = nullptr);
int colblock_repack_lane_layout (const ColBlocksDev &B, const int *d_gcols, hipStream_t st);
int launch_gs_fused (const CsrDev &L, const ColBlocksDev &B, int g0, int g1, const double *xa, const double *xb, int split,
                     const double *b, double *xout, hipStream_t st);
void launch_colblock_apply_lanes (const ColBlocksDev &B, int g0, int g1, const double *r, double *z, int accumulate, hipStream_t st);

void launch_colblock_measure (const CsrDev &A, const ColBlocksDev &B, int *d_out2 , hipStream_t st);
void launch_colblock_factor (const CsrDev &A, ColBlocksDev &B, int *d_status, hipStream_t st);
void launch_colblock_apply (const ColBlocksDev &B, const double *r, double *z, hipStream_t st);
void launch_colblock_apply_range (const ColBlocksDev &B, int b0, int b1, const double *r, double *z, int accumulate, hipStream_t st);
void launch_colblock_apply_range_r32 (const ColBlocksDev &B, int b0, int b1, const double *r, double *z, int accumulate, hipStream_t st);
void launch_build_wave_desc (const CsrDev &L, ColBlocksDev &B, hipStream_t st);
void launch_gs_wave (const CsrDev &L, const ColBlocksDev &B, int b0, int b1, const double *xa, const double *xb, int split, const double *b, double *xout,
                     int r32, hipStream_t st);
void launch_gs_wave_diag (const CsrDev &L, const ColBlocksDev &B, int tile0, int tile1, const double *xa, const double *xb, int split, const double *b,
                          double *xout, int r32, hipStream_t st);
void launch_gs_lanes_diag (const CsrDev &L, const ColBlocksDev &B, int g0, int g1, const double *xa, const double *xb, int split, const double *b,
                           double *xout, hipStream_t st);

#define NKP_BATCH_MAX 8
#define NKP_RED_BLOCKS 1024
#define NKP_DOT_CHUNK 8

void launch_multi_dot (const void *V, int v_f32, int64_t ld, int k, const double *w, int64_t n, double *partial, double *out, hipStream_t st);
void launch_update_w (const void *V, int v_f32, int64_t ld, int k, const double *h, double *w, int64_t n, double *partial, double *out_nrm2, hipStream_t st);
void launch_scale_to (const double *x, const double *alpha_dev, double *y, float *yf, int64_t n, hipStream_t st);
void launch_axpy_multi (const double *Z, int64_t ld, int k, const double *c, double *x, int64_t n, hipStream_t st);
void launch_dot (const double *x, const double *y, int64_t n, double *partial, double *out, hipStream_t st);
void launch_berr (const double *r, const double *den, int64_t n, double *partial, double *out, hipStream_t st);
void launch_count_entries (const double *x, int64_t n, double *partial, double *out, hipStream_t st);
void launch_finish_column (double *h, const double *h2, int k, const double *nrm2, double *inv, hipStream_t st);
void launch_finish_column_host (double *h, const double *h2, int k, const double *partial, int64_t n, double *nrm2_out, double *inv, double *host_col, hipStream_t st);
void launch_finish_column_pythagoras (double *h, int k, double *inv, hipStream_t st);
struct GsGroup {
   const double *V[NKP_BATCH_MAX];
   double *w[NKP_BATCH_MAX];
   double *partial[NKP_BATCH_MAX];
   double *vnext[NKP_BATCH_MAX];
};
void launch_multi_dot_group (int R, const GsGroup &G, int64_t ld, int k, int64_t n, double *msg, hipStream_t st);
void launch_update_w_group (int R, const GsGroup &G, int64_t ld, int k, const double *msg, int64_t n, double *nrm2, hipStream_t st);
void launch_finish_column_group (int R, double *msg, const double *msg2, int k, const double *nrm2, double *inv, hipStream_t st);
void launch_scale_to_group (int R, const GsGroup &G, const double *inv, int64_t n, hipStream_t st);
void launch_axpby (double a, const double *x, double b, double *y, int64_t n, hipStream_t st);
void launch_copy (const double *x, double *y, int64_t n, hipStream_t st);
void launch_vmul (const double *x, const double *w, double *y, int64_t n, hipStream_t st);
void launch_fill (double *y, double v, int64_t n, hipStream_t st);

void launch_restrict_sum (const int *rptr, const int *ridx, const double *fine, double *coarse, int64_t nc, hipStream_t st, double *coarse_x = nullptr);
void launch_cycle_entry (const int *perm, const double *w, const double *inv, double *vnext, double *b0, double *x0, int64_t n, hipStream_t st);
void launch_prolong_add (const int *cmap, const double *coarse, double *fine, int64_t nf, double omega, hipStream_t st);
void launch_gather (const int *perm, const double *in, double *out, int64_t n, hipStream_t st);
void launch_scatter (const int *perm, const double *in, double *out, int64_t n, hipStream_t st);
void launch_dense_matvec (const double *Minv, const double *x, double *y, int n, hipStream_t st);
void launch_dense_matvec_f32 (const float *Minv, int ld, const double *x, double *y, int n, hipStream_t st);
void launch_dense_matvec_f32_batch (int K, const float *Minv, int ld, const double *x, double *y, int n, hipStream_t st);
int dense_inverse_blocked_device (int n, const int *h_rowptr, const int *h_col, const double *h_val, double **inv_out, float **invf_out, int *ldf_out,
                                  size_t *bytes, hipStream_t st);
bool dense_inverse_device (int n, const std::vector<double> &host_a, double **inv_out, size_t *bytes, hipStream_t st);

void launch_interleave (int K, const double *const *src , double *X, int64_t n, hipStream_t st, const double *scale = nullptr);
void launch_deinterleave (int K, const double *X, double *const *dst , int64_t n, hipStream_t st);
void launch_csr_spmv_batch (int K, const CsrDev &A, int rb0, int rb1, const double *x, double *y, const double *b, int mode, hipStream_t st,
                            const double *scale = nullptr );
void launch_restrict_sum_batch (int K, const int *rptr, const int *ridx, const double *fine, double *coarse, int64_t nc, hipStream_t st);
void launch_prolong_add_batch (int K, const int *cmap, const double *coarse, double *fine, int64_t nf, double omega, hipStream_t st);
void launch_gather_batch (int K, const int *perm, const double *in, double *out, int64_t n, hipStream_t st);
void launch_scatter_batch (int K, const int *perm, const double *in, double *out, int64_t n, hipStream_t st);
void launch_gather_interleave (int K, const int *perm, const double *const *src, double *out, int64_t n, hipStream_t st, const double *scale = nullptr);
void launch_scatter_split (int K, const int *perm, const double *in, double *z, double *const *dst, int64_t n, hipStream_t st);
void launch_csr_spmv_batch_split (int K, const CsrDev &A, const double *x, double *const *dst, hipStream_t st, const double *scale = nullptr);
void launch_csr_spmv_batch_split_range (int K, const CsrDev &A, int rb0, int rb1, const double *x, double *const *dst, hipStream_t st, const double *scale = nullptr);
void launch_csr_residual_batch_split_range (int K, const CsrDev &A, int rb0, int rb1, const double *x, const double *const *b, const double *bscale,
                                            double *const *dst, hipStream_t st);
void launch_add_split (int K, const double *p, double *z, double *const *dst, int64_t n, hipStream_t st);
void launch_pack_rows_split (int K, const int *idx, const double *const *src, double *out, int64_t nrows, hipStream_t st);
void launch_gather_interleave_ext (int K, const int *perm, const double *const *src, const double *halo, const int *sel, int64_t n_own, double *out, int64_t n,
                                   hipStream_t st);
void launch_gather_interleave_ext_block (int K, const int *perm, const double *const *src, const double *recv, int64_t n_own, double *out, int64_t n, hipStream_t st);
void launch_scatter_split_own (int K, const int *perm, const double *in, double *z, double *const *dst, int64_t n_own, int64_t n, hipStream_t st);
// ... 6 lines not shown
```

### nk_ocn_tracer_jacobian_precond_amd/csrc/refactor_api.hip

```cpp
#include "solver_impl.h"

#include <stdio.h>
#include <time.h>

struct HierarchySource {
   const CsrDev &pat;
   const double *val;
   int64_t n, nnz;
   bool filter;
   const CsrDev *dev;
};

static int rebuild_hierarchy (nkp_solver *s, MlHierarchy &H2, int64_t n, const int32_t *rowptr, const int32_t *colind, const double *val, bool filter,
                              const CsrDev *dev, char *err, size_t errlen)
{
   std::vector<int32_t> f_rowptr, f_colind;
   std::vector<double> f_val;
   if (filter) {
      drop_intertracer (n, s->tracer_cnt, rowptr, colind, val, f_rowptr, f_colind, f_val);
      rowptr = f_rowptr.data ();
      colind = f_colind.data ();
      val = f_val.data ();
   }
   auto opt_ptr = [] (const std::vector<int> &a) { return a.empty () ? nullptr : a.data (); };
// ... 57 lines not shown
      if (drift) {
         msg (s, 1, "%s: %d couplings of %s hierarchy appear or vanish with the new values: rebuilding it\n", who, drift, dist ? "this rank's" : "the");
         *rebuild = true;
      }
   }
   const int live = s->shared->clones.load () - (int) s->batch_members.size ();
   if (!*rebuild) {
      char err[256] = "";
      const int irc = rf_prepare_inverse (W, s->ml, st, err, sizeof err);
      if (irc) return fail (irc == -4 ? NKP_ESINGULAR : irc == -2 ? NKP_ENOMEM : NKP_EDEVICE, "%s", err);
      if (live > 0 && !rf_inverse_same_storage (W, s->ml)) {
         rf_drop_inverse (W);
         return fail (NKP_EINVAL, "%s: the coarsest inverse of the new values needs other storage, which %d live clone(s) would not see; destroy them first", who, live);
      }
      return NKP_OK;
   }
   if (live > 0) return fail (NKP_EINVAL, "%s: the hierarchy has to be rebuilt, which %d live clone(s) would not see; destroy them first", who, live);
   std::vector<int32_t> rp ((size_t) src.n + 1), ci ((size_t) src.nnz);
   std::vector<double> v ((size_t) src.nnz);
   HIPCHK (hipStreamSynchronize (st));
   HIPCHK (hipMemcpy (rp.data (), src.pat.rowptr, rp.size () * sizeof (int32_t), hipMemcpyDeviceToHost));
   if (src.nnz) {
      HIPCHK (hipMemcpy (ci.data (), src.pat.colind, ci.size () * sizeof (int32_t), hipMemcpyDeviceToHost));
      HIPCHK (hipMemcpy (v.data (), src.val, v.size () * sizeof (double), hipMemcpyDeviceToHost));
   }
   char err[256] = "";
   const int mrc = rebuild_hierarchy (s, H2, src.n, rp.data (), ci.data (), v.data (), src.filter, src.dev, err, sizeof err);
   if (mrc != 0) return fail (mrc, "%s: %s (%s)", who, err, dist ? "no rank's solver is changed" : "the solver is unchanged");
   return NKP_OK;
}

static int refactor_commit (nkp_solver *s, bool rebuilt, MlHierarchy &H2, char *err, size_t errlen)
{
   RefactorWork &W = *s->rf;
   hipStream_t st = s->stream;
   const bool multilevel = s->opt.precond == NKP_PRECOND_MULTILEVEL;
   if (s->A.nnz && hipMemcpyAsync (s->A.val, W.aval, (size_t) s->A.nnz * sizeof (double), hipMemcpyDeviceToDevice, st) != hipSuccess) {
      snprintf (err, errlen, "copy of the new values failed");
      if (rebuilt) ml_free (H2);
      return -3;
   }
   launch_diag_fill (s->A, st);
   if (s->equil) rf_launch_row_scale (s->A, W.aval, s->rscale, s->rinv, st);
   int rc = 0;
   if (multilevel && rebuilt) {
      for (nkp_solver *c : s->batch_members) solver_free (c);
      s->batch_members.clear ();
      (void) hipStreamSynchronize (st);
      s->device_bytes -= s->ml.device_bytes;
      ml_free (s->ml);
      s->ml = H2;
      s->device_bytes += s->ml.device_bytes;
      s->device_bytes -= rf_free_maps (W);
      if (s->dist.smooth && (!ml_level0_hookable (s->ml) || smooth_build_lists (s) != 0)) {
         rc = -3;
         snprintf (err, errlen, "the index lists of the fine-level exchange could not be rebuilt for the new hierarchy");
      }
   } else if (multilevel) {
      int replaced = 0;
      const size_t before = s->ml.device_bytes;
      rc = rf_commit (W, s->ml, st, err, errlen, &replaced);
      s->device_bytes += s->ml.device_bytes - before;
      if (replaced) {
         for (nkp_solver *c : s->batch_members) solver_free (c);
         s->batch_members.clear ();
      }
   } else if (s->opt.precond == NKP_PRECOND_COLUMN_JACOBI) {
      const size_t before = W.bytes;
      rc = rf_column_factor (W, s->A, s->B, st, err, errlen);
      s->device_bytes += W.bytes - before;
   }
   if (hipStreamSynchronize (st) != hipSuccess || hipGetLastError () != hipSuccess) {
      if (!rc) { rc = -3; snprintf (err, errlen, "a HIP call failed"); }
   }
   return rc;
}

static int refactor_impl (nkp_solver *s, const double *h_val, const void *d_val, int flags, const char *who, bool collective)
{
   if (!s || (!h_val && !d_val)) return fail (NKP_EINVAL, "%s: NULL argument", who);
   if (s->borrowed) return fail (NKP_EINVAL, "%s: a clone shares its matrix; refactor the solver it was cloned from", who);
   if (s->dist.on && !collective) return fail (NKP_EINVAL, "%s: not available for the row-distributed flavour; every rank calls nkp_refactor_dist instead", who);
   const bool dist = s->dist.on;
   const bool multilevel = s->opt.precond == NKP_PRECOND_MULTILEVEL;
   DistRefactorPlan *Q = s->dplan;
   hipStream_t st = s->stream;
   auto agree = [&] (int local_rc, const char *where) { return dist ? dist_agree (s, local_rc, who, where) : local_rc; };
   if (dist) s->dist.agreed_K = 0;
   struct timespec ts0;
   clock_gettime (CLOCK_MONOTONIC, &ts0);

   int rc = NKP_OK;
   if (flags & ~NKP_REFACTOR_REBUILD) rc = fail (NKP_EINVAL, "%s: unknown flags 0x%x", who, flags);
   else if (dist && multilevel && !Q) rc = fail (NKP_EINVAL, "%s: the solver kept no plan of its hierarchy's matrix", who);
   else rc = refactor_stage (s, h_val, d_val, who);
   if (!rc && dist && multilevel && !Q->uploaded) {
      const int urc = rf_dist_upload (*Q, st);
      if (urc) rc = fail (urc == -2 ? NKP_ENOMEM : NKP_EDEVICE, "%s: the value maps of the hierarchy's matrix could not be uploaded", who);
      else s->device_bytes += Q->bytes;
   }
   if ((rc = agree (rc, "arguments and own diagonals"))) return rc;
   RefactorWork &W = *s->rf;

   bool rebuild = multilevel && (flags & NKP_REFACTOR_REBUILD);
   MlHierarchy H2;
   int64_t halo_values = 0;
// ... 93 lines not shown
```

### nk_ocn_tracer_jacobian_precond_amd/csrc/solver.hip

```cpp
#include "solver_impl.h"

#include <stdarg.h>
#include <stdio.h>
#include <string.h>

extern "C" int nkp_device_count (void)
{
   int n = 0;
   if (hipGetDeviceCount (&n) != hipSuccess) return 0;
   return n;
}

void solver_free (nkp_solver *s)
{
   if (!s) return;
   if (s->borrowed) {
      void *own[] = { s->V, s->vcur, s->Z, s->w, s->r, s->x, s->b, s->t1, s->t2, s->p1, s->p2, s->eqtmp, s->partial, s->dscal, s->dint };
      for (void *p : own)
         if (p) (void) hipFree (p);
      for (MlLevel &L : s->ml.lev) {
         void *lv[] = { L.x, L.x2, L.b, L.r };
         for (void *p : lv)
            if (p) (void) hipFree (p);
      }
      valgrad_release (s);
      valprod_release (s);
      if (s->hpin) (void) hipHostFree (s->hpin);
      if (s->own_stream && s->stream) (void) hipStreamDestroy (s->stream);
      s->shared->clones--;
      delete s;
      return;
   }
   if (s->trans_of) trans_detach (s);
   if (s->trans) trans_release (s);
   valgrad_release (s);
   valprod_release (s);
   for (nkp_solver *c : s->batch_members) solver_free (c);
   s->batch_members.clear ();
   for (double *p : { s->bvin, s->bz, s->bw })
      if (p) (void) hipFree (p);
   void *ptrs[] = { s->A.rowptr, s->A.colind, s->A.val, s->A.rowblk, s->A.codes, s->A.dict, s->A.dict_ptr, s->A.dg_ptr, s->A.dg_key, s->A.dg_voff, s->A.dg_vald, s->A.dg_tile, s->A.dg_gptr, s->A.dg_grp, s->B.blk_start, s->B.fac, s->B.grp_b0, s->B.grp_nb, s->B.grp_maxlen, s->B.grp_base, s->B.grp_row0, s->B.col_slot, s->B.fac_t, s->B.gs_rb_ptr, s->B.gs_rb, s->V, s->vcur, s->Z, s->w, s->r,
                    s->x, s->b, s->t1, s->t2, s->p1, s->p2, s->partial, s->dscal, s->dint, s->rscale, s->rinv, s->eqtmp };
   for (void *p : ptrs)
      if (p) (void) hipFree (p);
   delete s->B.grp_cols;
   ml_free (s->ml);
   if (s->rf) { rf_free (*s->rf); delete s->rf; }
   if (s->dplan) { rf_dist_free (*s->dplan); delete s->dplan; }
   s->dist.each_exchange ([] (RowExchange &X, bool) { exchange_release (X); });
   for (void *p : { (void *) s->dist.xe, (void *) s->dist.sel_idx, (void *) s->dist.rext, (void *) s->dist.zext, (void *) s->dist.bxe, (void *) s->dist.gmsg })
      if (p) (void) hipFree (p);
   if (s->dist.ghpin) (void) hipHostFree (s->dist.ghpin);
   if (s->dist.ev_packed) (void) hipEventDestroy (s->dist.ev_packed);
   if (s->dist.ev_halo) (void) hipEventDestroy (s->dist.ev_halo);
   if (s->dist.comm_stream) (void) hipStreamDestroy (s->dist.comm_stream);
   if (s->hpin) (void) hipHostFree (s->hpin);
   if (s->own_stream && s->stream) (void) hipStreamDestroy (s->stream);
   delete s;
}

extern "C" void nkp_destroy (nkp_solver *s) { solver_free (s); }

void msg (const nkp_solver *s, int lvl, const char *fmt, ...)
{
   if (s->opt.verbose < lvl) return;
   va_list ap;
   va_start (ap, fmt);
   printf ("(%d) ", s->opt.rank);
   vprintf (fmt, ap);
   va_end (ap);
   fflush (stdout);
}

extern "C" int nkp_set_stream (nkp_solver *s, void *hip_stream)
{
   if (!s) return fail (NKP_EINVAL, "nkp_set_stream: NULL solver");
   if (s->trans_of) return fail (NKP_EINVAL, "nkp_set_stream: a transposed solver runs on the stream of the solver it was transposed from; set that one's stream");
   if (s->own_stream && s->stream) { (void) hipStreamSynchronize (s->stream); (void) hipStreamDestroy (s->stream); }
   s->stream = (hipStream_t) hip_stream;
   s->own_stream = false;
   for (nkp_solver *c : s->batch_members) c->stream = s->stream;
   trans_set_stream (s);
   return NKP_OK;
}

extern "C" int64_t nkp_get_int (nkp_solver *s, const char *key)
{
   if (!s || !key) return -1;
   if (!strcmp (key, "n")) return s->n;
   if (!strcmp (key, "nnz")) return s->A.nnz;
   if (!strcmp (key, "nblk")) return s->B.nblk;
   if (!strcmp (key, "band")) return s->B.P;
   if (!strcmp (key, "band_dropped")) return s->B.dropped;
   if (!strcmp (key, "col_stream")) return s->B.stream ? 1 : 0;
   if (!strcmp (key, "col_ldsres")) return s->B.ldsres;
   if (!strcmp (key, "col_gw")) return s->B.gw;
   if (!strcmp (key, "col_max_len")) return s->B.max_len;
   if (!strcmp (key, "col_lds_bytes")) return (int64_t) s->B.lds_doubles * (int64_t) sizeof (double);
   if (!strcmp (key, "levels")) return s->opt.precond == NKP_PRECOND_MULTILEVEL ? (int64_t) s->ml.lev.size () : 1;
   if (!strcmp (key, "ml_rows")) { int64_t t = 0; for (auto &v : s->ml.lev) t += v.n; return t; }
   if (!strcmp (key, "ml_nnz")) { int64_t t = 0; for (auto &v : s->ml.lev) t += v.L.nnz; return t; }
   if (!strcmp (key, "rowblocks")) return s->A.nrowblk;
   if (!strcmp (key, "spmv_bytes")) return 12 * s->A.nnz + 4 * (s->n + 1) + 16 * s->n;
   if (!strcmp (key, "spmv_diag")) return s->A.dg_vald ? 1 : 0;
   if (!strcmp (key, "spmv_diag_bytes"))
      return s->A.dg_vald ? 8 * s->A.dg_nval + (int64_t) s->A.dg_ntile * (int64_t) sizeof (DgTile) + (int64_t) s->A.dg_ngrp * (int64_t) sizeof (DgGroup) + 16 * s->n : 0;
   if (!strcmp (key, "precond_bytes")) return s->opt.precond == NKP_PRECOND_NONE ? 16 * s->n : (int64_t) (2 * s->B.P + 1) * 8 * s->n + 16 * s->n;
   if (!strcmp (key, "device_bytes")) return (int64_t) s->device_bytes;
   if (!strcmp (key, "precond_steps")) return s->precond_steps;
   if (!strcmp (key, "equil")) return s->equil ? 1 : 0;
   if (!strcmp (key, "dist_overlap")) return s->dist.overlap ? 1 : 0;
   if (!strcmp (key, "dist_ras")) return s->dist.ras ? 1 : 0;
   if (!strcmp (key, "dist_ras_rows")) return s->dist.n_sel;
   if (!strcmp (key, "dist_ras_rings")) return s->dist.ras ? s->dist.ras_rings : 0;
   if (!strcmp (key, "dist_halo_rows")) return s->dist.n_halo;
   if (!strcmp (key, "dist_smooth_exchange")) return s->dist.smooth ? 1 : 0;
   if (!strcmp (key, "dist_smooth_rows")) return s->dist.smooth ? s->dist.n_sel : 0;
   if (!strcmp (key, "dist_ras_recv_rows")) return !s->dist.ras ? 0 : s->dist.ras_sep ? s->dist.n_sel : s->dist.n_halo;
   if (!strcmp (key, "dist_interior_rowblocks")) return s->dist.seg_rb[2] - s->dist.seg_rb[1];
   if (!strcmp (key, "smoother_spmv_bytes")) return s->opt.precond == NKP_PRECOND_MULTILEVEL ? ml_bytes (s->ml, 0) : 0;
   if (!strcmp (key, "column_solve_bytes")) return s->opt.precond == NKP_PRECOND_MULTILEVEL ? ml_bytes (s->ml, 1) : 0;
   if (!strcmp (key, "cycle_bytes")) return s->opt.precond == NKP_PRECOND_MULTILEVEL ? ml_bytes (s->ml, 2) : 0;
   if (!strcmp (key, "ml_levels_on_device")) return s->ml.levels_on_device;
   if (!strcmp (key, "ml_inverse_pivoted")) return s->ml.inverse_pivoted;
   if (!strcmp (key, "ml_setup_us")) return (int64_t) (s->ml.setup_seconds * 1.0e6);
   if (!strcmp (key, "create_us")) return (int64_t) (s->create_seconds * 1.0e6);
   if (!strcmp (key, "refactor_count")) return s->refactor_count;
   if (!strcmp (key, "refactor_rebuilt")) return s->refactor_rebuilt;
   if (!strcmp (key, "refactor_us")) return (int64_t) (s->refactor_seconds * 1.0e6);
   if (!strcmp (key, "refactor_halo_values")) return s->refactor_halo_values;
   if (!strcmp (key, "is_transpose")) return s->trans_of ? 1 : 0;
   if (!strcmp (key, "trans_device_bytes")) return trans_device_bytes (s);
   if (!strcmp (key, "trans_us")) return (int64_t) (s->trans_seconds * 1.0e6);
   if (!strcmp (key, "trans_kernel_us")) return (int64_t) (s->trans_kernel_seconds * 1.0e6);
   if (!strcmp (key, "trans_sent_entries")) return s->trans_sent;
   if (!strcmp (key, "trans_recv_entries")) return s->trans_received;
   if (!strcmp (key, "dist_alltoallv_calls")) return s->shared->alltoallv_calls.load ();
   if (!strcmp (key, "dist_allreduce_calls")) return s->shared->allreduce_calls.load ();
   if (!strcmp (key, "value_gradient_calls")) return s->vg.calls;
   if (!strcmp (key, "value_gradient_us")) return (int64_t) (s->vg.seconds * 1.0e6);
   if (!strcmp (key, "values_product_calls")) return s->vp.calls;
   if (!strcmp (key, "values_product_us")) return (int64_t) (s->vp.seconds * 1.0e6);
   if (!strcmp (key, "tangent_calls")) return s->vp.tangent_calls;
   if (!strcmp (key, "batch_steps")) return s->batch_steps;
   if (!strcmp (key, "batch_width")) return s->batch_width;
   if (!strcmp (key, "batch_member_bytes")) {
      size_t sum = 0;
      for (const nkp_solver *c : s->batch_members) sum += c->device_bytes;
      return (int64_t) sum;
   }
   return -1;
}

extern "C" int nkp_set_device (int device)
{
   HIPCHK (hipSetDevice (device));
   return NKP_OK;
}
```

### nk_ocn_tracer_jacobian_precond_amd/csrc/solver_impl.h

```cpp
#pragma once
#include "../../include/nkp.h"
#include "nkp_dev.h"
#include "multilevel.h"
#include "refactor.h"
#include "dist_plan.h"
#include "row_exchange.h"
#include "krylov_host.h"

#include <atomic>
#include <initializer_list>
#include <memory>
#include <string>
#include <utility>
#include <vector>

#define HIPCHK(call)                                                                             \
   do {                                                                                          \
      hipError_t e_ = (call);                                                                    \
      if (e_ != hipSuccess) return fail (NKP_EDEVICE, "%s failed: %s (%s:%d)", #call, hipGetErrorString (e_), __FILE__, __LINE__); \
   } while (0)

struct nkp_solver {
   nkp_options opt;
   nkp_tuning tune;
   int device = 0;
   bool stagnated = false;
   int rhs_class = 0;
   bool borrowed = false;
   hipStream_t stream = nullptr;
   bool own_stream = false;
   CsrDev A;
   ColBlocksDev B;
   MlHierarchy ml;
   struct {
      bool on = false;
      nkp_comm_ops ops;
      int64_t n_global = 0, fst = 0, n_halo = 0;
      RowExchange x_halo, x_ras, x_smooth[2];
      template <class F> void each_exchange (F f) { f (x_halo, on); f (x_ras, ras_sep); f (x_smooth[0], smooth); f (x_smooth[1], smooth); }
      double *xe = nullptr;
      int seg_rb[4] = { 0, 0, 0, 0 };
      bool overlap = false;
      hipStream_t comm_stream = nullptr;
      hipEvent_t ev_packed = nullptr, ev_halo = nullptr;
      bool ras = false;
      int64_t n_ext = 0, n_sel = 0;
      int *sel_idx = nullptr;
      double *rext = nullptr, *zext = nullptr;
      int ras_rings = 0;
      bool ras_sep = false;
      bool smooth = false;
      MlSmoothHook smooth_hook = { nullptr, nullptr };
      std::vector<int32_t> h_smooth_send[2], h_smooth_recv[2];
      double *bxe = nullptr, *gmsg = nullptr, *ghpin = nullptr;
      int bK = 0;
      int agreed_K = 0;
      std::vector<int64_t> starts;
      std::vector<int32_t> h_halo_rows, h_send_rows, own_blk, own_ci, own_cj, own_ct;
      bool own_has_blk = false;
      int own_tracer_cnt = 1;
   } dist;
   int64_t n = 0, ld = 0;
   int m = 0;
   bool vf32 = false;
   double *vcur = nullptr;
   double *V = nullptr, *Z = nullptr, *w = nullptr, *r = nullptr, *x = nullptr, *b = nullptr, *t1 = nullptr, *t2 = nullptr;
   double *p1 = nullptr, *p2 = nullptr;
   int precond_steps = 1;
   int steps_now = 1;
   bool equil = false;
   double *rscale = nullptr, *rinv = nullptr;
   double *eqtmp = nullptr;
   bool comm_failed = false;
   double *partial = nullptr;
   double *dscal = nullptr;
   double *hpin = nullptr;
   int *dint = nullptr;
   std::vector<nkp_solver *> batch_members;
   double *bvin = nullptr, *bz = nullptr, *bw = nullptr;
   int batch_K = 0;
   int64_t batch_steps = 0;
   int batch_width = 0;
   size_t device_bytes = 0;
   double create_seconds = 0.0;
   struct Shared {
      std::atomic<int> clones { 0 };
      std::atomic<int64_t> alltoallv_calls { 0 }, allreduce_calls { 0 };
      bool broken = false;
      std::string why;
   };
   std::shared_ptr<Shared> shared = std::make_shared<Shared> ();
   RefactorWork *rf = nullptr;
   std::vector<int> h_blk, h_col_i, h_col_j, h_col_t;
   int tracer_cnt = 1;
   int64_t refactor_count = 0;
   int refactor_rebuilt = 0;
   double refactor_seconds = 0.0;
   DistRefactorPlan *dplan = nullptr;
   int64_t refactor_halo_values = 0;
   nkp_solver *trans = nullptr, *trans_of = nullptr;
   int *trans_src = nullptr;
   double *trans_val = nullptr;
   size_t trans_map_bytes = 0;
   double trans_seconds = 0.0, trans_kernel_seconds = 0.0;
   int *trans_ship = nullptr;
   double *trans_send = nullptr, *trans_recv = nullptr;
   std::vector<int> trans_send_counts, trans_recv_counts;
   int64_t trans_nnz = 0, trans_sent = 0, trans_received = 0;
   struct {
      double *lam = nullptr, *x = nullptr, *stage = nullptr, *g = nullptr;
      size_t lam_cap = 0, x_cap = 0, stage_cap = 0, g_cap = 0;
      int64_t calls = 0;
      double seconds = 0.0;
   } vg;
   struct {
      double *x = nullptr, *stage = nullptr, *r = nullptr;
      size_t x_cap = 0, stage_cap = 0, r_cap = 0;
      int64_t calls = 0, tangent_calls = 0;
      double seconds = 0.0;
// ... 62 lines not shown
}

inline int width_of (int nrhs) { return nrhs <= 1 ? 1 : nrhs <= 2 ? 2 : nrhs <= 4 ? 4 : 8; }

inline int alltoallv_dev (nkp_solver *s, const double *send, const int *send_counts, double *recv, const int *recv_counts, hipStream_t st, bool sticky = true)
{
   s->shared->alltoallv_calls++;
   const int rc = s->dist.ops.alltoallv (s->dist.ops.ctx, send, send_counts, recv, recv_counts, (void *) st);
   if (rc && sticky) s->comm_failed = true;
   return rc;
}
inline int exchange_rows (nkp_solver *s, RowExchange &X, int K, const double *packed, double *dest, hipStream_t st, bool sticky = true)
{ return alltoallv_dev (s, packed, X.send_counts_for (K), dest, X.recv_counts_for (K), st, sticky); }

inline void allreduce_dev (nkp_solver *s, double *dev, int count, int op)
{
   if (!s->dist.on) return;
   s->shared->allreduce_calls++;
   if (s->dist.ops.allreduce (s->dist.ops.ctx, dev, count, op, (void *) s->stream)) s->comm_failed = true;
}

inline int refactor_broken (const nkp_solver *s) { return fail (NKP_ESINGULAR, "%s", s->shared->why.c_str ()); }

inline int sev_of (int c) { return c == NKP_OK ? 0 : c == NKP_OK_BERR ? 1 : c == NKP_NOT_CONVERGED ? 2 : 3; }

#define NKP_BERR_ROUNDING_LEVEL 1.0e-14

NKP_PRIVATE void solver_free (nkp_solver *s);
NKP_PRIVATE void msg (const nkp_solver *s, int lvl, const char *fmt, ...);
struct SpmvMatrixHost {
   int64_t nnz, ncols;
   const int32_t *rowptr, *colind;
   const double *val;
};
struct PrecondMatrixHost {
   int64_t n, nblk;
   const int32_t *rowptr, *colind;
   const double *val;
   const int32_t *blk_start, *col_i, *col_j, *col_t;
};
NKP_PRIVATE int create_impl (nkp_solver **out, const nkp_options *opt_in, int64_t n, int64_t nnz,
                             const int32_t *rowptr, const int32_t *colind, const double *val,
                             const int32_t *blk_start, int64_t nblk, int coupled_tracer_cnt, const SpmvMatrixHost *spmv_mat,
                             const PrecondMatrixHost *pm = nullptr);
NKP_PRIVATE int clone_impl (nkp_solver *src, nkp_solver **out, bool member);
NKP_PRIVATE void drop_intertracer (int64_t n, int tracer_cnt, const int32_t *rowptr, const int32_t *colind, const double *val,
                                   std::vector<int32_t> &f_rowptr, std::vector<int32_t> &f_colind, std::vector<double> &f_val);
NKP_PRIVATE void apply_precond_once (nkp_solver *s, const double *rin, double *zout);
NKP_PRIVATE void apply_precond (nkp_solver *s, const double *rin, double *zout);
NKP_PRIVATE void spmv_op (nkp_solver *s, const double *x, double *y, const double *b, int mode);
NKP_PRIVATE void arnoldi_apply (nkp_solver *s, int j);
NKP_PRIVATE void arnoldi_orthogonalise (nkp_solver *s, int j);
NKP_PRIVATE int arnoldi_hand_over (nkp_solver *s, int j, hipEvent_t ev);
struct NKP_PRIVATE StepEvent {
   hipEvent_t ev = nullptr;
   int make (const nkp_solver *s);
   ~StepEvent ();
};
NKP_PRIVATE int fg_begin (nkp_solver *s, FgmresState &F);
NKP_PRIVATE int fg_restart (nkp_solver *s, FgmresState &F);
NKP_PRIVATE bool fg_post_step (nkp_solver *s, FgmresState &F);
NKP_PRIVATE int fg_end_cycle (nkp_solver *s, FgmresState &F);
NKP_PRIVATE int rhs_refused (int verdict, const char *what);
NKP_PRIVATE int backward_error (nkp_solver *s, double *berr);
NKP_PRIVATE const char *batch_unsupported (const nkp_solver *s);
NKP_PRIVATE void note_fallback (const nkp_solver *s, const char *who, const char *why, int nrhs);
NKP_PRIVATE int batch_prepare_exchange (nkp_solver *s, int K);
NKP_PRIVATE int dist_allgather (nkp_solver *s, int local_rc, int64_t mine, std::vector<int64_t> &all, const char *who, const char *where);
inline int failed_rank (const std::vector<int64_t> &all) { for (size_t p = 0; p < all.size (); p++) if (all[p] < 0) return (int) p; return -1; }
NKP_PRIVATE int dist_agree (nkp_solver *s, int local_rc, const char *who, const char *where);
NKP_PRIVATE bool exchange_install (nkp_solver *s, RowExchange &X, const int32_t *rows, const std::vector<int> &give, const std::vector<int> &need,
                                   bool unpacks, int64_t cap_send, int64_t cap_recv, int64_t wide_recv);
NKP_PRIVATE void exchange_release (RowExchange &X);
inline void push_wide (RowExchange &X, bool in_force, std::vector<std::pair<double **, size_t>> &set)
{
   if (in_force && X.wide_send >= 0) set.push_back ({ &X.bsend, (size_t) X.wide_send });
   if (in_force && X.wide_recv >= 0) set.push_back ({ &X.brecv, (size_t) X.wide_recv });
}
inline double *halo_rows_of (nkp_solver *s, int K) { return K == 1 ? s->dist.xe + s->n : s->dist.bxe + s->n * K; }
NKP_PRIVATE int halo_fetch (nkp_solver *s, int K, const double *x, const double *const *xp, hipStream_t comm, bool sticky = true);
template <class Rows> inline void halo_product_overlapped (nkp_solver *s, int K, const double *x, Rows rows)
{
   auto &D = s->dist;
   halo_fetch (s, K, x, nullptr, D.comm_stream);
   rows (D.seg_rb[1], D.seg_rb[2]);
   (void) hipStreamWaitEvent (s->stream, D.ev_halo, 0);
   rows (D.seg_rb[0], D.seg_rb[1]);
   rows (D.seg_rb[2], D.seg_rb[3]);
}
NKP_PRIVATE bool smooth_install (nkp_solver *s, const DistPlan &D);
NKP_PRIVATE int smooth_build_lists (nkp_solver *s);
NKP_PRIVATE const MlSmoothHook *smooth_hook_of (nkp_solver *s);
NKP_PRIVATE void launch_smooth_pack (int K, const int *idx, const double *x, double *out, int64_t nrows, hipStream_t st);
NKP_PRIVATE void launch_smooth_unpack (int K, const int *idx, const double *in, double *x, int64_t nrows, hipStream_t st);
NKP_PRIVATE void valgrad_release (nkp_solver *s);
NKP_PRIVATE int valgrad_time_prepare (nkp_solver *s, int K);
NKP_PRIVATE void valgrad_time_launch (nkp_solver *s, int K);
NKP_PRIVATE int fetch_x_operand (nkp_solver *s, int K, const double *const *xp, double *il, const double **x_in, const char *who);
NKP_PRIVATE void valprod_release (nkp_solver *s);
NKP_PRIVATE int valprod_time_prepare (nkp_solver *s, int K, int which);
NKP_PRIVATE void valprod_time_launch (nkp_solver *s, int K);
NKP_PRIVATE void valprod_time_composition (nkp_solver *s, int K);
NKP_PRIVATE void trans_release (nkp_solver *s);
NKP_PRIVATE void trans_detach (nkp_solver *t);
NKP_PRIVATE void trans_set_stream (nkp_solver *s);
NKP_PRIVATE int64_t trans_device_bytes (const nkp_solver *s);
// ... 3 lines not shown
```

### nk_ocn_tracer_jacobian_precond_amd/csrc/tuning.cpp

```cpp
#include "tuning.h"

#include <stdarg.h>
#include <stdio.h>
#include <stdlib.h>
#include <string.h>

static thread_local std::string g_last_error;

int fail (int code, const char *fmt, ...)
{
   char buf[512];
   va_list ap;
   va_start (ap, fmt);
   vsnprintf (buf, sizeof buf, fmt, ap);
   va_end (ap);
   g_last_error = buf;
   return code;
}

extern "C" const char *nkp_last_error (void) { return g_last_error.c_str (); }
std::string last_error_message () { return g_last_error; }
void restore_error_message (const std::string &text) { g_last_error = text; }

extern "C" int nkp_default_options (nkp_options *opt)
{
   if (!opt) return NKP_EINVAL;
   memset (opt, 0, sizeof *opt);
   opt->struct_size = (int) sizeof (nkp_options);
   opt->precond = NKP_PRECOND_MULTILEVEL;
   opt->krylov = NKP_KRYLOV_FGMRES;
   opt->restart = 200;
   opt->max_iters = 20000;
   opt->rtol = 1.0e-10;
   opt->atol = 0.0;
   opt->device = -1;
   opt->verbose = 0;
   opt->rank = 0;
   opt->reorth = 0;
   opt->ml_levels = 0;
   opt->ml_smooth = 3;
   opt->precond_steps = 0;
   opt->equil = 0;
   opt->basis_f32 = 0;
   return NKP_OK;
}

static void builtin_tuning (nkp_tuning *t)
{
   memset (t, 0, sizeof *t);
   t->struct_size = (int) sizeof (nkp_tuning);
   t->ml_split = 1; t->ml_pocket = 4; t->ml_big_from = -3; t->ml_coarsest_rows = 8000; t->ml_dense_max = 8192;
   t->ml_theta = 0.0; t->ml_tau = 0.01; t->ml_device_min = 100000;
   t->ml_smooth_coarse = 0; t->ml_coarse_from = 2; t->ml_gamma_from = 0; t->ml_gamma_to = 0; t->ml_f32 = 1; t->ml_host_inverse = 0;
   t->ml_fused = 0; t->ml_fused_max_cols = 0; t->ml_wave_fused = 1; t->ml_coarsest_sweeps = 30; t->ml_tail_rows = 0; t->ml_omega = 1.1;
   t->col_ldsres = 2; t->col_stream = 1; t->col_stream_min = -1; t->col_stream_gw = 32; t->col_wave_max = 8192; t->col_w3 = 1;
   t->col_group = 8; t->col_pipe_min = 0; t->col_ldsres_early = 0; t->col_ldsres_packed = 1; t->col_sort_groups = 1;
   t->spmv_variant = 4; t->spmv_compress = 0; t->spmv_pipe_min = 1024; t->spmv_run = 1; t->spmv_wgs = 256;
   t->rhs_batch = 1; t->batch_spmv_rows = 1; t->precond_steps = 0; t->equil = -1; t->dist_overlap = 1; t->dist_ras = 1; t->dist_one_reduce = 0; t->force_dist = 0; t->setup_threads = 0; t->plan_times = 0;
   t->ml_drop_intertracer = 0; t->ml_huge_from = -1; t->dist_ras_rings = 1; t->ml_diag = 32; t->spmv_diag = 32;
   t->ml_lane_fused = 50000; t->dist_smooth_exchange = 0; t->step_glue = 12;
}

const nkp_tuning &nkp_builtin_tuning ()
{
   static const nkp_tuning t = [] { nkp_tuning q; builtin_tuning (&q); return q; } ();
   return t;
}

extern "C" int nkp_default_tuning (nkp_tuning *t)
{
   if (!t) return NKP_EINVAL;
   builtin_tuning (t);
   const char *e;
#define ENV_INT(name, field) do { if ((e = getenv (name)) && *e) t->field = atoi (e); } while (0)
#define ENV_POS(name, field) do { if ((e = getenv (name)) && atoi (e) > 0) t->field = atoi (e); } while (0)
#define ENV_FLAG(name, field) do { if ((e = getenv (name)) && *e) t->field = atoi (e) != 0; } while (0)
   ENV_FLAG ("NKP_ML_SPLIT", ml_split); ENV_INT ("NKP_ML_POCKET", ml_pocket); ENV_INT ("NKP_ML_BIG_FROM", ml_big_from);
   ENV_INT ("NKP_ML_COARSEST_ROWS", ml_coarsest_rows); ENV_INT ("NKP_ML_DENSE_MAX", ml_dense_max);
   if ((e = getenv ("NKP_ML_THETA")) && *e) t->ml_theta = atof (e);
   if ((e = getenv ("NKP_ML_TAU")) && *e) t->ml_tau = atof (e);
   if ((e = getenv ("NKP_ML_DEVICE_MIN")) && *e) t->ml_device_min = atoll (e);
   ENV_POS ("NKP_ML_SMOOTH_COARSE", ml_smooth_coarse); ENV_POS ("NKP_ML_COARSE_FROM", ml_coarse_from);
   ENV_INT ("NKP_ML_GAMMA_FROM", ml_gamma_from); ENV_INT ("NKP_ML_GAMMA_TO", ml_gamma_to);
   ENV_FLAG ("NKP_ML_F32", ml_f32); ENV_FLAG ("NKP_ML_HOST_INVERSE", ml_host_inverse); ENV_FLAG ("NKP_ML_FUSED", ml_fused);
   ENV_INT ("NKP_ML_FUSED_MAX_COLS", ml_fused_max_cols); ENV_INT ("NKP_ML_WAVE_FUSED", ml_wave_fused); ENV_POS ("NKP_ML_COARSEST_SWEEPS", ml_coarsest_sweeps);
   if ((e = getenv ("NKP_ML_TAIL_ROWS")) && *e) t->ml_tail_rows = atoll (e);
   if ((e = getenv ("NKP_ML_OMEGA")) && atof (e) > 0.0) t->ml_omega = atof (e);
   ENV_INT ("NKP_COL_LDSRES", col_ldsres); ENV_FLAG ("NKP_COLSTREAM", col_stream); ENV_INT ("NKP_COLSTREAM_MIN", col_stream_min);
   if ((e = getenv ("NKP_COLSTREAM_GW")) && *e) t->col_stream_gw = atoi (e) == 64 ? 64 : 32;
   ENV_INT ("NKP_COLWAVE_MAX", col_wave_max); ENV_FLAG ("NKP_COL_W3", col_w3); ENV_INT ("NKP_COLGROUP", col_group);
   ENV_INT ("NKP_COLPIPE_MIN", col_pipe_min); ENV_FLAG ("NKP_LDSRES_EARLY", col_ldsres_early); ENV_FLAG ("NKP_COL_PACKED", col_ldsres_packed); ENV_FLAG ("NKP_COL_SORT_GROUPS", col_sort_groups); ENV_INT ("NKP_COL_LDSRES_MIN", col_ldsres_min); ENV_INT ("NKP_ML_HUGE_FROM", ml_huge_from);
   ENV_INT ("NKP_SPMV_VARIANT", spmv_variant); ENV_FLAG ("NKP_SPMV_COMPRESS", spmv_compress); ENV_INT ("NKP_SPMV_PIPE_MIN", spmv_pipe_min);
   ENV_POS ("NKP_SPMV_RUN", spmv_run); ENV_POS ("NKP_SPMV_WGS", spmv_wgs);
   ENV_INT ("NKP_RHS_BATCH", rhs_batch); ENV_FLAG ("NKP_BATCH_SPMV_ROWS", batch_spmv_rows);
   ENV_POS ("NKP_PRECOND_STEPS", precond_steps); ENV_FLAG ("NKP_EQUIL", equil);
   ENV_FLAG ("NKP_DIST_OVERLAP", dist_overlap); ENV_FLAG ("NKP_DIST_RAS", dist_ras); ENV_FLAG ("NKP_DIST_ONE_REDUCE", dist_one_reduce);
   if (getenv ("NKP_FORCE_DIST")) t->force_dist = 1;
   ENV_POS ("NKP_SETUP_THREADS", setup_threads);
   if (getenv ("NKP_ML_PLAN_TIMES")) t->plan_times = 1;
   ENV_FLAG ("NKP_ML_DROP_INTERTRACER", ml_drop_intertracer);
   ENV_INT ("NKP_DIST_RAS_RINGS", dist_ras_rings);
   ENV_INT ("NKP_ML_DIAG", ml_diag);
   ENV_INT ("NKP_SPMV_DIAG", spmv_diag);
   ENV_INT ("NKP_ML_LANE_FUSED", ml_lane_fused);
   ENV_INT ("NKP_DIST_SMOOTH_EXCHANGE", dist_smooth_exchange);
   ENV_INT ("NKP_STEP_GLUE", step_glue);
#undef ENV_INT
#undef ENV_POS
#undef ENV_FLAG
   if (t->spmv_variant < 0 || t->spmv_variant > 9) t->spmv_variant = 4;
   return NKP_OK;
}

int resolve_tuning (const nkp_options *opt, nkp_tuning *out, bool *range_error)
{
   if (range_error) *range_error = false;
   if (opt && opt->tuning) {
      if (opt->tuning->struct_size != (int) sizeof (nkp_tuning)) return fail (NKP_EINVAL, "nkp_tuning.struct_size mismatch (%d != %zu)", opt->tuning->struct_size, sizeof (nkp_tuning));
      *out = *opt->tuning;
   } else {
      const int rc = nkp_default_tuning (out);
      if (rc) return rc;
   }
   if (out->dist_ras_rings < 0 || out->dist_ras_rings > 4) {
      if (range_error) *range_error = true;
      return fail (NKP_EINVAL, "nkp_tuning.dist_ras_rings = %d is out of range (0 = default, 1 .. 4 rings)", out->dist_ras_rings);
   }
   if (out->dist_smooth_exchange != 0 && out->dist_smooth_exchange != 1) {
      if (range_error) *range_error = true;
      return fail (NKP_EINVAL, "nkp_tuning.dist_smooth_exchange = %d is out of range (0 = off, 1 = on)", out->dist_smooth_exchange);
   }
   return NKP_OK;
}
```

### nk_ocn_tracer_jacobian_precond_amd/solver.py

```python
from __future__ import annotations

import ctypes as C
import os

import numpy as np

_HERE = os.path.dirname(os.path.abspath(__file__))
HIP_LIB_PATH = os.path.join(_HERE, "csrc", "libnkp_hip.so")
HOST_LIB_PATH = os.path.join(_HERE, "host", "libnkp_host.so")

PRECOND_NONE, PRECOND_COLUMN_JACOBI, PRECOND_MULTILEVEL = 0, 1, 3
KRYLOV_FGMRES, KRYLOV_BICGSTAB = 0, 1
NKP_OK, NKP_NOT_CONVERGED, NKP_BREAKDOWN, NKP_OK_BERR = 0, 1, 2, 3
REFACTOR_REBUILD = 1

ABI_SYMBOLS = [
    "nkp_default_options", "nkp_device_count", "nkp_create", "nkp_solve", "nkp_solve_device",
    "nkp_spmv", "nkp_spmv_device", "nkp_precond_apply", "nkp_multi_dot", "nkp_time_kernel",
    "nkp_get_int", "nkp_set_stream", "nkp_destroy", "nkp_last_error", "nkp_comm_unique_id",
    "nkp_comm_rccl_init", "nkp_comm_rccl_free", "nkp_create_dist", "nkp_dist_plan_host", "nkp_set_device",
    "nkp_gather_root", "nkp_clone", "nkp_ml_plan_host", "nkp_comm_file_init", "nkp_comm_file_free",
    "nkp_create64", "nkp_cell_major_order", "nkp_permuted_rows", "nkp_dist_overlap_plan_host", "nkp_dist_plan_size",
    "nkp_dist_plan_copy", "nkp_dist_plan_free", "nkp_ml_level_array", "nkp_default_tuning", "nkp_solve_batch_device",
    "nkp_refactor", "nkp_refactor_device", "nkp_refactor_dist", "nkp_refactor_dist_device", "nkp_transpose", "nkp_transpose_dist",
    "nkp_value_gradient", "nkp_value_gradient_device",
    "nkp_values_product", "nkp_values_product_device", "nkp_solve_tangent_device", "nkp_matrix_array",
]

_ALLREDUCE_FN = C.CFUNCTYPE(C.c_int, C.c_void_p, C.c_void_p, C.c_int, C.c_int, C.c_void_p)
_ALLTOALLV_FN = C.CFUNCTYPE(C.c_int, C.c_void_p, C.c_void_p, C.POINTER(C.c_int), C.c_void_p, C.POINTER(C.c_int), C.c_void_p)
_ALLTOALLV_I32_FN = C.CFUNCTYPE(C.c_int, C.c_void_p, C.POINTER(C.c_int32), C.POINTER(C.c_int), C.POINTER(C.c_int32), C.POINTER(C.c_int))
_ALLGATHER_I64_FN = C.CFUNCTYPE(C.c_int, C.c_void_p, C.c_int64, C.POINTER(C.c_int64))


class NkpCommOps(C.Structure):
    _fields_ = [("ctx", C.c_void_p), ("rank", C.c_int), ("nranks", C.c_int), ("allreduce", _ALLREDUCE_FN),
                ("alltoallv", _ALLTOALLV_FN), ("alltoallv_i32_host", _ALLTOALLV_I32_FN),
                ("allgather_i64_host", _ALLGATHER_I64_FN)]


class NkpTuning(C.Structure):
    _fields_ = [
        ("struct_size", C.c_int), ("ml_split", C.c_int), ("ml_pocket", C.c_int), ("ml_big_from", C.c_int), ("ml_coarsest_rows", C.c_int),
        ("ml_dense_max", C.c_int), ("ml_theta", C.c_double), ("ml_tau", C.c_double), ("ml_device_min", C.c_int64),
        ("ml_smooth_coarse", C.c_int), ("ml_coarse_from", C.c_int), ("ml_gamma_from", C.c_int), ("ml_gamma_to", C.c_int), ("ml_f32", C.c_int),
        ("ml_host_inverse", C.c_int), ("ml_fused", C.c_int), ("ml_fused_max_cols", C.c_int), ("ml_wave_fused", C.c_int), ("ml_coarsest_sweeps", C.c_int),
        ("ml_tail_rows", C.c_int64), ("ml_omega", C.c_double),
        ("col_ldsres", C.c_int), ("col_stream", C.c_int), ("col_stream_min", C.c_int), ("col_stream_gw", C.c_int), ("col_wave_max", C.c_int),
        ("col_w3", C.c_int), ("col_group", C.c_int), ("col_pipe_min", C.c_int), ("col_ldsres_early", C.c_int), ("col_ldsres_packed", C.c_int),
        ("spmv_variant", C.c_int), ("spmv_compress", C.c_int), ("spmv_pipe_min", C.c_int), ("spmv_run", C.c_int), ("spmv_wgs", C.c_int),
        ("rhs_batch", C.c_int), ("precond_steps", C.c_int), ("equil", C.c_int), ("dist_overlap", C.c_int), ("dist_ras", C.c_int), ("force_dist", C.c_int),
        ("setup_threads", C.c_int), ("plan_times", C.c_int), ("ml_drop_intertracer", C.c_int), ("dist_one_reduce", C.c_int), ("ml_huge_from", C.c_int), ("col_ldsres_min", C.c_int), ("col_sort_groups", C.c_int), ("batch_spmv_rows", C.c_int),
        ("dist_ras_rings", C.c_int), ("ml_diag", C.c_int), ("spmv_diag", C.c_int), ("ml_lane_fused", C.c_int),
        ("dist_smooth_exchange", C.c_int),
        ("step_glue", C.c_int),
    ]


class NkpOptions(C.Structure):
    _fields_ = [
        ("struct_size", C.c_int), ("precond", C.c_int), ("krylov", C.c_int), ("restart", C.c_int),
        ("max_iters", C.c_int), ("rtol", C.c_double), ("atol", C.c_double), ("device", C.c_int),
        ("verbose", C.c_int), ("rank", C.c_int), ("reorth", C.c_int), ("ml_levels", C.c_int),
        ("ml_smooth", C.c_int), ("basis_f32", C.c_int), ("precond_steps", C.c_int), ("equil", C.c_int), ("reserved", C.c_int * 4),
        ("col_i", C.POINTER(C.c_int32)), ("col_j", C.POINTER(C.c_int32)), ("col_t", C.POINTER(C.c_int32)),
        ("tuning", C.POINTER(NkpTuning)),
    ]


class NkpError(RuntimeError):
    def __init__(self, code, message):
        super().__init__(f"nkp error {code}: {message}")
        self.code = code


_lib = None


def load_library(path=None):
    global _lib
    if _lib is not None and path is None:
        return _lib
    path = path or HIP_LIB_PATH
    if not os.path.exists(path):
        raise FileNotFoundError(
            f"{path} not found: build it with `python -c 'import __graft_entry__ as g; g.build()'` "
            "(there is no CPU fallback for the solve path)")
    lib = C.CDLL(path, mode=C.RTLD_GLOBAL)
    i32p, f64p, vp = C.POINTER(C.c_int32), C.POINTER(C.c_double), C.c_void_p
    lib.nkp_default_options.argtypes = [C.POINTER(NkpOptions)]
    lib.nkp_device_count.restype = C.c_int
    lib.nkp_create.argtypes = [C.POINTER(vp), C.POINTER(NkpOptions), C.c_int64, C.c_int64, i32p, i32p, f64p, i32p, C.c_int64, C.c_int]
    lib.nkp_create64.argtypes = [C.POINTER(vp), C.POINTER(NkpOptions), C.c_int64, C.POINTER(C.c_int64), i32p, f64p, i32p, C.c_int64, C.c_int]
    lib.nkp_solve.argtypes = [vp, f64p, C.c_int, C.c_int64, f64p, C.POINTER(C.c_int), f64p]
    lib.nkp_solve_device.argtypes = [vp, vp, vp, C.c_int, f64p, C.POINTER(C.c_int), f64p]
    lib.nkp_solve_batch_device.argtypes = [vp, C.c_int, vp, vp, C.c_int64, f64p, C.POINTER(C.c_int), f64p]
    lib.nkp_spmv.argtypes = [vp, f64p, f64p]
    lib.nkp_spmv_device.argtypes = [vp, vp, vp]
    lib.nkp_precond_apply.argtypes = [vp, f64p, f64p]
    lib.nkp_multi_dot.argtypes = [vp, f64p, C.c_int64, C.c_int, f64p, f64p]
    lib.nkp_time_kernel.argtypes = [vp, C.c_int, C.c_int, C.c_int, f64p]
    lib.nkp_get_int.argtypes = [vp, C.c_char_p]
    lib.nkp_get_int.restype = C.c_int64
    lib.nkp_ml_level_array.argtypes = [vp, C.c_int, C.c_char_p, vp, C.c_int64]
    lib.nkp_ml_level_array.restype = C.c_int64
    lib.nkp_matrix_array.argtypes = [vp, C.c_char_p, vp, C.c_int64]
    lib.nkp_matrix_array.restype = C.c_int64
    lib.nkp_set_stream.argtypes = [vp, vp]
    lib.nkp_destroy.argtypes = [vp]
    lib.nkp_destroy.restype = None
    lib.nkp_last_error.restype = C.c_char_p
    lib.nkp_comm_unique_id.argtypes = [vp]
    lib.nkp_comm_rccl_init.argtypes = [C.POINTER(NkpCommOps), vp, C.c_int, C.c_int]
    lib.nkp_comm_rccl_free.argtypes = [C.POINTER(NkpCommOps)]
    lib.nkp_comm_rccl_free.restype = None
    lib.nkp_create_dist.argtypes = [C.POINTER(vp), C.POINTER(NkpOptions), C.c_int64, C.c_int64, C.c_int64, C.c_int64,
                                    i32p, i32p, f64p, i32p, C.c_int64, C.c_int, C.POINTER(NkpCommOps)]
    lib.nkp_set_device.argtypes = [C.c_int]
    lib.nkp_gather_root.argtypes = [vp, f64p, f64p]
    lib.nkp_clone.argtypes = [vp, C.POINTER(vp)]
    lib.nkp_transpose.argtypes = [vp, C.POINTER(vp)]
    lib.nkp_transpose_dist.argtypes = [vp, C.POINTER(vp)]
    lib.nkp_value_gradient.argtypes = [vp, C.c_int, f64p, f64p, C.c_int64, C.c_double, C.c_int, f64p]
    lib.nkp_value_gradient_device.argtypes = [vp, C.c_int, vp, vp, C.c_int64, C.c_double, C.c_int, vp]
    lib.nkp_values_product.argtypes = [vp, C.c_int, f64p, f64p, C.c_int64, C.c_double, C.c_int, f64p, C.c_int64]
    lib.nkp_values_product_device.argtypes = [vp, C.c_int, vp, vp, C.c_int64, C.c_double, C.c_int, vp, C.c_int64]
    lib.nkp_solve_tangent_device.argtypes = [vp, C.c_int, vp, vp, C.c_int64, vp, vp, C.c_int64, f64p, C.POINTER(C.c_int), f64p]
    lib.nkp_refactor.argtypes = [vp, f64p, C.c_int]
    lib.nkp_refactor_device.argtypes = [vp, vp, C.c_int]
    lib.nkp_refactor_dist.argtypes = [vp, f64p, C.c_int]
    lib.nkp_refactor_dist_device.argtypes = [vp, vp, C.c_int]
    lib.nkp_dist_plan_host.argtypes = [C.c_int64, C.c_int64, i32p, i32p, C.c_int, C.c_int, C.POINTER(C.c_int64), i32p, i32p,
                                       C.POINTER(C.c_int64), i32p]
    lib.nkp_ml_plan_host.argtypes = [C.c_int64, i32p, i32p, f64p, i32p, C.c_int64, i32p, i32p, C.c_int, C.c_int, C.c_int, C.c_int64,
                                     C.POINTER(C.c_int), C.POINTER(C.c_int64), i32p, i32p]
    if path == HIP_LIB_PATH:
        _lib = lib
    return lib


def ml_plan_host(rowptr, colind, val, blk_start, col_i=None, col_j=None, coupled_tracer_cnt=1, max_levels=0, coarsest_rows=8000):
    lib = load_library()
    rowptr = np.ascontiguousarray(rowptr, np.int32)
    colind = np.ascontiguousarray(colind, np.int32)
    val = np.ascontiguousarray(val, np.float64)
    blk_start = np.ascontiguousarray(blk_start, np.int32)
    n = rowptr.size - 1
    ip = lambda a: None if a is None else _p(np.ascontiguousarray(a, np.int32), C.c_int32)
    ci = None if col_i is None else np.ascontiguousarray(col_i, np.int32)
    cj = None if col_j is None else np.ascontiguousarray(col_j, np.int32)
    cap = 2 * n + 64
# ... 197 lines not shown
        if Y is None:
            y, acc = np.empty_like(x), 0
        else:
            y, acc = np.array(np.atleast_2d(np.asarray(Y, np.float64)), order="C", copy=True), 1
            if y.shape != x.shape:
                raise ValueError("Y must have the shape of X")
        v = val if val.size else np.zeros(1)
        self._check_collective(self._lib.nkp_values_product(self._h, x.shape[0], _p(v, C.c_double), _p(x, C.c_double), self.n, float(alpha), acc,
                                                            _p(y, C.c_double), self.n))
        return y.reshape(np.shape(X))

    def values_product_device(self, d_val, d_x, nrhs, ldx, d_y, ldy, alpha=1.0, accumulate=False):
        self._check_collective(self._lib.nkp_values_product_device(self._h, int(nrhs), C.c_void_p(d_val), C.c_void_p(d_x), int(ldx), float(alpha),
                                                                   int(bool(accumulate)), C.c_void_p(d_y), int(ldy)))

    def solve_tangent_device(self, d_dval, d_x, ldx, d_db, d_dx, nrhs, ld, raise_on_fail=True):
        berr, relres, iters = (C.c_double * nrhs)(), (C.c_double * nrhs)(), (C.c_int * nrhs)()
        rc = self._lib.nkp_solve_tangent_device(self._h, int(nrhs), C.c_void_p(d_dval or None), C.c_void_p(d_x or None), int(ldx), C.c_void_p(d_db or None),
                                                C.c_void_p(d_dx), int(ld), berr, iters, relres)
        self._check(rc, (0,) if raise_on_fail else (0, 1, 2, 3))
        return [dict(status=rc, iters=iters[c], relres=relres[c], berr=berr[c]) for c in range(nrhs)]

    def solve_tangent(self, X, dval=None, dB=None, raise_on_fail=True):
        if dval is None and dB is None:
            raise ValueError("solve_tangent needs dval or dB")
        x = np.ascontiguousarray(np.atleast_2d(np.asarray(X, np.float64)))
        K, n = x.shape
        if n != self.n:
            raise ValueError(f"X must have shape ({self.n},) or (K, {self.n})")
        bufs = []
        try:
            d_x = _device_array(bufs, x) if dval is not None else None
            d_v = _device_array(bufs, np.ascontiguousarray(dval, np.float64).reshape(-1), self.nnz) if dval is not None else None
            d_b = _device_array(bufs, np.ascontiguousarray(np.atleast_2d(np.asarray(dB, np.float64))), K * n) if dB is not None else None
            out = np.empty((K, n))
            d_o = _device_array(bufs, out)
            infos = self.solve_tangent_device(d_v, d_x, n, d_b, d_o, K, n, raise_on_fail)
            if out.nbytes:
                _hip_check(_hip().hipMemcpy(C.c_void_p(out.ctypes.data), C.c_void_p(d_o), C.c_size_t(out.nbytes), 2))
        finally:
            for q in bufs:
                _hip().hipFree(C.c_void_p(q))
        return out.reshape(np.shape(X)), infos

    def _check_collective(self, rc):
        self._check(rc)

    def spmv(self, x):
        x = np.ascontiguousarray(x, np.float64)
        y = np.empty(self.n)
        self._check(self._lib.nkp_spmv(self._h, _p(x, C.c_double), _p(y, C.c_double)))
        return y

    def spmv_device(self, d_x, d_y):
        self._check(self._lib.nkp_spmv_device(self._h, C.c_void_p(d_x), C.c_void_p(d_y)))

    def precond_apply(self, r):
        r = np.ascontiguousarray(r, np.float64)
        z = np.empty(self.n)
        self._check(self._lib.nkp_precond_apply(self._h, _p(r, C.c_double), _p(z, C.c_double)))
        return z

    def multi_dot(self, V, w):
        V = np.ascontiguousarray(V, np.float64)
        w = np.ascontiguousarray(w, np.float64)
        k = V.shape[0]
        out = np.empty(k + 1)
        self._check(self._lib.nkp_multi_dot(self._h, _p(V, C.c_double), V.shape[1], k, _p(w, C.c_double), _p(out, C.c_double)))
        return out

    def time_kernel(self, which, reps=20, arg=0):
        ms = C.c_double()
        self._check(self._lib.nkp_time_kernel(self._h, which, arg, reps, C.byref(ms)))
        return ms.value

    def get_int(self, key):
        return int(self._lib.nkp_get_int(self._h, key.encode()))

    _ML_ARRAY_TYPES = {"valf": np.float32, "val": np.float64, "fac": np.float64, "coarse_inv": np.float64, "color_blk": np.int32,
                       "col_kernel": np.int32, "dg_ptr": np.int32, "dg_key": np.int32, "dg_voff": np.int64, "dg_val": np.float32,
                       "dg_gptr": np.int32, "dg_grp": np.int32}

    def ml_level_array(self, level, what):
        cnt = int(self._lib.nkp_ml_level_array(self._h, level, what.encode(), None, 0))
        if cnt < 0:
            raise NkpError(cnt, last_error())
        out = np.empty(cnt, self._ML_ARRAY_TYPES.get(what, np.int32))
        if cnt:
            got = int(self._lib.nkp_ml_level_array(self._h, level, what.encode(), out.ctypes.data_as(C.c_void_p), out.nbytes))
            if got != cnt:
                raise NkpError(got, last_error())
        return out

    def matrix_array(self, what):
        cnt = int(self._lib.nkp_matrix_array(self._h, what.encode(), None, 0))
        if cnt < 0:
            raise NkpError(cnt, last_error())
        out = np.empty(cnt, {"dg_voff": np.int64, "dg_val": np.float64, "val": np.float64, "fac": np.float64}.get(what, np.int32))
        if cnt:
            got = int(self._lib.nkp_matrix_array(self._h, what.encode(), out.ctypes.data_as(C.c_void_p), out.nbytes))
            if got != cnt:
                raise NkpError(got, last_error())
        return out

    def set_stream(self, stream_ptr):
        self._check(self._lib.nkp_set_stream(self._h, C.c_void_p(stream_ptr)))
# ... 90 lines not shown
```

Baseline: 34.20 million.

## Keep preconditioned vectors in level-0 order and run SpMV on renumbered keys

Builds a second set of diagonal-SpMV tiles and groups whose column keys are shifted to read x directly in the multilevel hierarchy's level-0 permuted order, plus a permuted axpy kernel for the FGMRES update. The aim is to drop the permute/unpermute copies between the preconditioner output and the next SpMV in each Krylov step. It is on by default through a new step_order tuning flag and costs extra setup work (host copies, an atomic shift-scan kernel) and device memory. Rows whose shifts are not uniform fall back to single-row tiles, which can make the SpMV less efficient.

```diff
diff --git a/include/nkp.h b/include/nkp.h
--- a/include/nkp.h
+++ b/include/nkp.h
@@ -87,6 +87,7 @@
    int ml_lane_fused;
    int dist_smooth_exchange;
    int step_glue;
+   int step_order;
 } nkp_tuning;
 
 int nkp_default_tuning (nkp_tuning *t);
@@ -136,6 +137,7 @@
 
 int nkp_spmv (nkp_solver *s, const double *x, double *y);
 int nkp_spmv_device (nkp_solver *s, const void *d_x, void *d_y);
+int nkp_spmv_level0 (nkp_solver *s, const double *x0, const double *b, double *y);
 
 int nkp_precond_apply (nkp_solver *s, const double *r, double *z);
 
diff --git a/nk_ocn_tracer_jacobian_precond_amd/csrc/blas1.hip b/nk_ocn_tracer_jacobian_precond_amd/csrc/blas1.hip
--- a/nk_ocn_tracer_jacobian_precond_amd/csrc/blas1.hip
+++ b/nk_ocn_tracer_jacobian_precond_amd/csrc/blas1.hip
@@ -237,6 +237,29 @@
    hipLaunchKernelGGL ((update_w_kernel<double, double2>), dim3 (g), dim3 (B1_THREADS), 0, st, Z, ld, k, c, x, n, (double *) nullptr, 1.0);
 }
 
+__global__ __launch_bounds__ (B1_THREADS)
+void axpy_multi_level0_kernel (const int *__restrict__ perm, const double *__restrict__ Z, int64_t ld, int k0, int k, const double *__restrict__ c,
+                               double *__restrict__ x, int64_t n)
+{
+   __shared__ double hs[B1_MAX_K];
+   for (int j = threadIdx.x; j < k; j += B1_THREADS) hs[j] = 1.0 * c[j];
+   __syncthreads ();
+   const int64_t stride = (int64_t) gridDim.x * B1_THREADS;
+   for (int64_t i = (int64_t) blockIdx.x * B1_THREADS + threadIdx.x; i < n; i += stride) {
+      const int p = perm[i];
+      double a = x[p];
+      for (int j = 0; j < k0 && j < k; j++) a += hs[j] * Z[(int64_t) j * ld + p];
+      for (int j = k0; j < k; j++) a += hs[j] * Z[(int64_t) j * ld + i];
+      x[p] = a;
+   }
+}
+
+void launch_axpy_multi_level0 (const int *perm, const double *Z, int64_t ld, int k0, int k, const double *c, double *x, int64_t n, hipStream_t st)
+{
+   if (n <= 0) return;
+   hipLaunchKernelGGL (axpy_multi_level0_kernel, dim3 (red_grid (n) * 2), dim3 (B1_THREADS), 0, st, perm, Z, ld, k0, k, c, x, n);
+}
+
 __device__ __forceinline__ void scale_to_body (const double *__restrict__ x, const double *__restrict__ alpha, double *__restrict__ y, float *__restrict__ yf, int64_t n)
 {
    const double a = alpha[0];
diff --git a/nk_ocn_tracer_jacobian_precond_amd/csrc/create.hip b/nk_ocn_tracer_jacobian_precond_amd/csrc/create.hip
--- a/nk_ocn_tracer_jacobian_precond_amd/csrc/create.hip
+++ b/nk_ocn_tracer_jacobian_precond_amd/csrc/create.hip
@@ -58,6 +58,15 @@
    int color_tile[3];
    (void) diag_build (s->A, blk_start, (const int *) d_blk, (int) nblk, (int) nblk, max_len, s->tune.spmv_diag, color_tile, &s->device_bytes, s->stream);
    (void) hipFree (d_blk);
+}
+
+void build_level0_keys (nkp_solver *s)
+{
+   diag_drop_level0 (s->A, &s->device_bytes);
+   if (!(s->tune.step_order & 16) || !(s->tune.step_glue & 8) || s->opt.precond != NKP_PRECOND_MULTILEVEL || s->dist.on || !s->A.dg_vald) return;
+   if (s->ml.lev.empty () || s->ml.lev[0].n != s->n || !s->ml.perm0 || !ml_level0_hookable (s->ml)) return;
+   if (s->h_blk.empty () || (int64_t) s->h_blk.size () - 1 != s->A.dg_ncol) return;
+   (void) diag_build_level0 (s->A, s->h_blk.data (), s->A.dg_ncol, s->ml.perm0, &s->device_bytes, s->stream);
 }
 
 static int check_arguments (const nkp_options *opt_in, int64_t n, int64_t nnz, const int32_t *rowptr, const int32_t *colind, const double *val,
@@ -375,6 +384,7 @@
    }
    if (opt.precond == NKP_PRECOND_MULTILEVEL &&
        (rc = build_hierarchy (s, n, rowptr, colind, val, blk_start, nblk, blk_default.empty (), coupled_tracer_cnt, !spmv_mat, pm))) return rc;
+   build_level0_keys (s);
    if (opt.precond == NKP_PRECOND_COLUMN_JACOBI && (rc = factor_columns (s, blk_start, nblk))) return rc;
    TRYHIP (hipStreamSynchronize (s->stream));
    TRYHIP (hipGetLastError ());
@@ -448,6 +458,9 @@
    s->V = s->vcur = s->Z = s->w = s->r = s->x = s->b = s->t1 = s->t2 = s->p1 = s->p2 = s->eqtmp = s->partial = s->dscal = s->hpin = nullptr;
    s->dint = nullptr;
    for (MlLevel &L : s->ml.lev) L.x = L.x2 = L.b = L.r = nullptr;
+   s->ml.x0_home = nullptr;
+   s->ml.entered = 0;
+   s->z_level0 = false;
    int rc = NKP_OK;
    TRYHIP (hipStreamCreateWithFlags (&s->stream, hipStreamNonBlocking));
    s->own_stream = true;
diff --git a/nk_ocn_tracer_jacobian_precond_amd/csrc/diag_layout.cpp b/nk_ocn_tracer_jacobian_precond_amd/csrc/diag_layout.cpp
--- /dev/null
+++ b/nk_ocn_tracer_jacobian_precond_amd/csrc/diag_layout.cpp
@@ -0,0 +1,64 @@
+#include "diag_layout.h"
+
+#include <stddef.h>
+
+void dg_groups (const int *key, int nk, int rows, std::vector<DgGroup> &out)
+{
+   const int fit = 64 - rows + 1, lim = fit < DG_RUN_MAX ? fit : DG_RUN_MAX;
+   for (int s = 0; s < nk;) {
+      int m = 1;
+      while (s + m < nk && m < lim && key[s + m] == key[s + m - 1] + 1) m++;
+      DgGroup R;
+      R.key0 = key[s];
+      R.slots = s | m << 16;
+      out.push_back (R);
+      s += m;
+   }
+}
+
+bool dg_renumbered_layout (int ncol, const int *blk_start, const int *ptr, const int *key, const int *shift_min, const int *shift_max,
+                           const int *pos, int n, const DgTile *tiles, int ntile, std::vector<DgGroup> &grp_out, std::vector<DgTile> &tiles_out)
+{
+   auto refuse = [&] () { grp_out.clear (); tiles_out.clear (); return false; };
+   grp_out.clear ();
+   tiles_out.clear ();
+   tiles_out.reserve ((size_t) ntile);
+   std::vector<int> k0;
+   int t = 0;
+   for (int c = 0; c < ncol; c++) {
+      const int len = blk_start[c + 1] - blk_start[c], nt = dg_col_tiles (len), nk = ptr[c + 1] - ptr[c];
+      if (t + nt > ntile) return refuse ();
+      bool whole = true;
+      for (int s = 0; s < nk; s++) whole = whole && shift_min[ptr[c] + s] == shift_max[ptr[c] + s];
+      k0.resize ((size_t) nk);
+      if (whole) {
+         for (int s = 0; s < nk; s++) k0[(size_t) s] = key[ptr[c] + s] + shift_min[ptr[c] + s];
+         const int g0 = (int) grp_out.size ();
+         if (nt) dg_groups (k0.data (), nk, (len + nt - 1) / nt, grp_out);
+         for (int q = 0; q < nt; q++) {
+            DgTile T = tiles[t + q];
+            T.g0 = g0;
+            T.ng = (int) grp_out.size () - g0;
+            tiles_out.push_back (T);
+         }
+      } else {
+         for (int kl = 0; kl < len; kl++) {
+            for (int s = 0; s < nk; s++) {
+               const int k = ptr[c] + s;
+               const long long j = (long long) key[k] + kl;
+               k0[(size_t) s] = key[k] + (shift_min[k] == shift_max[k] || j < 0 || j >= n ? shift_min[k] : pos[j] - (int) j);
+            }
+            DgTile T = tiles[t];
+            T.row0 = blk_start[c] + kl;
+            T.rows = 1;
+            T.kl0 = kl;
+            T.g0 = (int) grp_out.size ();
+            dg_groups (k0.data (), nk, 1, grp_out);
+            T.ng = (int) grp_out.size () - T.g0;
+            tiles_out.push_back (T);
+         }
+      }
+      t += nt;
+   }
+   return t == ntile ? true : refuse ();
+}
diff --git a/nk_ocn_tracer_jacobian_precond_amd/csrc/diag_layout.h b/nk_ocn_tracer_jacobian_precond_amd/csrc/diag_layout.h
--- /dev/null
+++ b/nk_ocn_tracer_jacobian_precond_amd/csrc/diag_layout.h
@@ -0,0 +1,23 @@
+#pragma once
+
+#include <vector>
+
+struct alignas (16) DgTile {
+   int row0, rows;
+   int kl0, len;
+   int k0, nk;
+   int g0, ng;
+   long long voff;
+};
+struct DgGroup {
+   int key0;
+   int slots;
+};
+#define DG_RUN_MAX 5
+
+inline int dg_col_tiles (int len) { return (len + 63) / 64; }
+
+void dg_groups (const int *key, int nk, int rows, std::vector<DgGroup> &out);
+
+bool dg_renumbered_layout (int ncol, const int *blk_start, const int *ptr, const int *key, const int *shift_min, const int *shift_max,
+                           const int *pos, int n, const DgTile *tiles, int ntile, std::vector<DgGroup> &grp_out, std::vector<DgTile> &tiles_out);
diff --git a/nk_ocn_tracer_jacobian_precond_amd/csrc/diagop.hip b/nk_ocn_tracer_jacobian_precond_amd/csrc/diagop.hip
--- a/nk_ocn_tracer_jacobian_precond_amd/csrc/diagop.hip
+++ b/nk_ocn_tracer_jacobian_precond_amd/csrc/diagop.hip
@@ -79,6 +79,27 @@
    }
 }
 
+__global__ __launch_bounds__ (DG_THREADS)
+void diag_key_shift_kernel (int ntile, const DgTile *__restrict__ tile, const int *__restrict__ rowptr, const int *__restrict__ colind,
+                            const int *__restrict__ dg_key, const int *__restrict__ pos, int *__restrict__ shift_min, int *__restrict__ shift_max)
+{
+   const int t = blockIdx.x * DG_WAVES + (threadIdx.x >> 6), lane = threadIdx.x & (NKP_WAVE - 1);
+   if (t >= ntile) return;
+   const DgTile T = tile[t];
+   if (lane >= T.rows) return;
+   const int kl = T.kl0 + lane;
+   int p = rowptr[T.row0 + lane];
+   const int e1 = rowptr[T.row0 + lane + 1];
+   for (int s = 0; s < T.nk && p < e1; s++) {
+      const int j = colind[p];
+      if (j - kl != dg_key[T.k0 + s]) continue;
+      const int d = pos[j] - j;
+      atomicMin (shift_min + T.k0 + s, d);
+      atomicMax (shift_max + T.k0 + s, d);
+      p++;
+   }
+}
+
 template <class VT, int MODE>
 __global__ __launch_bounds__ (DG_THREADS)
 void diag_residual_kernel (const DgTile *__restrict__ tile, int ntile, const DgGroup *__restrict__ dg_grp, const VT *__restrict__ dg_val,
@@ -137,22 +158,6 @@
    L.dg_nval = 0;
    *device_bytes -= held;
    (void) hipGetLastError ();
-}
-
-static inline int dg_col_tiles (int len) { return (len + NKP_WAVE - 1) / NKP_WAVE; }
-
-static void dg_groups (const int *key, int nk, int rows, std::vector<DgGroup> &out)
-{
-   const int fit = NKP_WAVE - rows + 1, lim = fit < DG_RUN_MAX ? fit : DG_RUN_MAX;
-   for (int s = 0; s < nk;) {
-      int m = 1;
-      while (s + m < nk && m < lim && key[s + m] == key[s + m - 1] + 1) m++;
-      DgGroup R;
-      R.key0 = key[s];
-      R.slots = s | m << 16;
-      out.push_back (R);
-      s += m;
-   }
 }
 
 int diag_build (CsrDev &L, const int *h_blk_start, const int *d_blk_start, int ncol, int ncol0, int max_len, int cap, int color_tile[3],
@@ -277,12 +282,75 @@
    });
 }
 
-void launch_diag_spmv (const CsrDev &A, const double *x, double *y, const double *b, int mode, hipStream_t st)
-{
-   if (A.dg_ntile <= 0 || !A.dg_vald) return;
-   const dim3 grid ((A.dg_ntile + DG_WAVES - 1) / DG_WAVES);
+void launch_diag_spmv (const CsrDev &A, const double *x, double *y, const double *b, int mode, hipStream_t st, bool x_level0)
+{
+   if (A.dg_ntile <= 0 || !A.dg_vald || (x_level0 && !A.dg_tile0)) return;
+   const int ntile = x_level0 ? A.dg_ntile0 : A.dg_ntile;
+   const dim3 grid ((ntile + DG_WAVES - 1) / DG_WAVES);
+   const DgTile *tile = x_level0 ? A.dg_tile0 : A.dg_tile;
+   const DgGroup *grp = x_level0 ? A.dg_grp0 : A.dg_grp;
    with_bool (mode == 1, [&] (auto residual) {
-      hipLaunchKernelGGL ((diag_residual_kernel<double, decltype (residual)::value ? 1 : 0>), grid, dim3 (DG_THREADS), 0, st, (const DgTile *) A.dg_tile, A.dg_ntile,
-                          (const DgGroup *) A.dg_grp, (const double *) A.dg_vald, x, b, y, (int) A.n);
+      hipLaunchKernelGGL ((diag_residual_kernel<double, decltype (residual)::value ? 1 : 0>), grid, dim3 (DG_THREADS), 0, st, tile, ntile,
+                          grp, (const double *) A.dg_vald, x, b, y, (int) A.n);
    });
 }
+
+void diag_drop_level0 (CsrDev &A, size_t *device_bytes)
+{
+   if (A.dg_tile0) { (void) hipFree (A.dg_tile0); *device_bytes -= (size_t) A.dg_ntile0 * sizeof (DgTile); }
+   if (A.dg_grp0) { (void) hipFree (A.dg_grp0); *device_bytes -= (size_t) (A.dg_ngrp0 ? A.dg_ngrp0 : 1) * sizeof (DgGroup); }
+   A.dg_tile0 = nullptr;
+   A.dg_grp0 = nullptr;
+   A.dg_ngrp0 = A.dg_ntile0 = 0;
+}
+
+int diag_build_level0 (CsrDev &A, const int *h_blk_start, int ncol, const int *d_perm0, size_t *device_bytes, hipStream_t st)
+{
+   diag_drop_level0 (A, device_bytes);
+   if (!A.dg_vald || A.dg_ntile <= 0 || ncol != A.dg_ncol || !d_perm0 || A.n <= 0 || h_blk_start[ncol] != A.n) return 0;
+   const size_t n = (size_t) A.n, nkey = (size_t) A.dg_nkey;
+   auto gave_up = [] () { (void) hipGetLastError (); return 0; };
+   std::vector<int> perm (n), pos (n, -1);
+   if (hipStreamSynchronize (st) != hipSuccess || hipMemcpy (perm.data (), d_perm0, n * sizeof (int), hipMemcpyDeviceToHost) != hipSuccess) return gave_up ();
+   for (size_t i = 0; i < n; i++) {
+      if (perm[i] < 0 || (size_t) perm[i] >= n || pos[(size_t) perm[i]] >= 0) return 0;
+      pos[(size_t) perm[i]] = (int) i;
+   }
+   mls::DBuf<int> dpos, dmin, dmax;
+   if (dpos.alloc (n) != hipSuccess || dmin.alloc (nkey ? nkey : 1) != hipSuccess || dmax.alloc (nkey ? nkey : 1) != hipSuccess) return gave_up ();
+   std::vector<int> smin (nkey, INT_MAX), smax (nkey, INT_MIN);
+   if (hipMemcpy (dpos.p, pos.data (), n * sizeof (int), hipMemcpyHostToDevice) != hipSuccess ||
+       (nkey && (hipMemcpy (dmin.p, smin.data (), nkey * sizeof (int), hipMemcpyHostToDevice) != hipSuccess ||
+                 hipMemcpy (dmax.p, smax.data (), nkey * sizeof (int), hipMemcpyHostToDevice) != hipSuccess)))
+      return gave_up ();
+   hipLaunchKernelGGL (diag_key_shift_kernel, dim3 ((A.dg_ntile + DG_WAVES - 1) / DG_WAVES), dim3 (DG_THREADS), 0, st, A.dg_ntile, (const DgTile *) A.dg_tile,
+                       (const int *) A.rowptr, (const int *) A.colind, (const int *) A.dg_key, (const int *) dpos.p, dmin.p, dmax.p);
+   std::vector<int> ptr ((size_t) ncol + 1), key (nkey);
+   std::vector<DgTile> tiles ((size_t) A.dg_ntile);
+   if (hipStreamSynchronize (st) != hipSuccess || hipMemcpy (ptr.data (), A.dg_ptr, ptr.size () * sizeof (int), hipMemcpyDeviceToHost) != hipSuccess ||
+       hipMemcpy (tiles.data (), A.dg_tile, tiles.size () * sizeof (DgTile), hipMemcpyDeviceToHost) != hipSuccess ||
+       (nkey && (hipMemcpy (key.data (), A.dg_key, nkey * sizeof (int), hipMemcpyDeviceToHost) != hipSuccess ||
+                 hipMemcpy (smin.data (), dmin.p, nkey * sizeof (int), hipMemcpyDeviceToHost) != hipSuccess ||
+                 hipMemcpy (smax.data (), dmax.p, nkey * sizeof (int), hipMemcpyDeviceToHost) != hipSuccess)))
+      return gave_up ();
+   if (ptr[(size_t) ncol] != A.dg_nkey) return 0;
+   std::vector<DgGroup> grp0;
+   std::vector<DgTile> tiles0;
+   if (!dg_renumbered_layout (ncol, h_blk_start, ptr.data (), key.data (), smin.data (), smax.data (), pos.data (), (int) n, tiles.data (), A.dg_ntile, grp0, tiles0) ||
+       tiles0.empty ())
+      return 0;
+   void *dt = nullptr, *dg = nullptr;
+   const size_t tb = tiles0.size () * sizeof (DgTile), gb = (grp0.size () ? grp0.size () : 1) * sizeof (DgGroup);
+   if (hipMalloc (&dt, tb) != hipSuccess || hipMalloc (&dg, gb) != hipSuccess || hipMemcpy (dt, tiles0.data (), tb, hipMemcpyHostToDevice) != hipSuccess ||
+       (grp0.size () && hipMemcpy (dg, grp0.data (), grp0.size () * sizeof (DgGroup), hipMemcpyHostToDevice) != hipSuccess)) {
+      if (dt) (void) hipFree (dt);
+      if (dg) (void) hipFree (dg);
+      return gave_up ();
+   }
+   A.dg_tile0 = (DgTile *) dt;
+   A.dg_grp0 = (DgGroup *) dg;
+   A.dg_ngrp0 = (int) grp0.size ();
+   A.dg_ntile0 = (int) tiles0.size ();
+   *device_bytes += tb + gb;
+   return 1;
+}
diff --git a/nk_ocn_tracer_jacobian_precond_amd/csrc/inspect.hip b/nk_ocn_tracer_jacobian_precond_amd/csrc/inspect.hip
--- a/nk_ocn_tracer_jacobian_precond_amd/csrc/inspect.hip
+++ b/nk_ocn_tracer_jacobian_precond_amd/csrc/inspect.hip
@@ -68,6 +68,9 @@
    else if (!strcmp (what, "dg_val")) { src = A.dg_vald; count = have ? A.dg_nval : 0; elem = 8; }
    else if (!strcmp (what, "dg_gptr")) { src = A.dg_gptr; count = have ? A.dg_ncol + 1 : 0; }
    else if (!strcmp (what, "dg_grp")) { src = A.dg_grp; count = have ? 2 * (int64_t) A.dg_ngrp : 0; }
+   else if (!strcmp (what, "dg_grp0")) { src = A.dg_grp0; count = A.dg_tile0 ? 2 * (int64_t) A.dg_ngrp0 : 0; }
+   else if (!strcmp (what, "dg_tile0")) { src = A.dg_tile0; count = A.dg_tile0 ? (int64_t) (sizeof (DgTile) / 4) * A.dg_ntile0 : 0; }
+   else if (!strcmp (what, "dg_tile")) { src = A.dg_tile; count = have ? (int64_t) (sizeof (DgTile) / 4) * A.dg_ntile : 0; }
    else if (!strcmp (what, "rowptr")) { src = A.rowptr; count = src ? A.n + 1 : 0; }
    else if (!strcmp (what, "colind")) { src = A.colind; count = src ? A.nnz : 0; }
    else if (!strcmp (what, "val")) { src = A.val; count = src ? A.nnz : 0; elem = 8; }
@@ -98,6 +101,21 @@
    const size_t bytes = (size_t) s->n * sizeof (double);
    HIPCHK (hipMemcpyAsync (s->t1, x, bytes, hipMemcpyHostToDevice, s->stream));
    spmv_op (s, s->t1, s->t2, nullptr, 0);
+   HIPCHK (hipMemcpyAsync (y, s->t2, bytes, hipMemcpyDeviceToHost, s->stream));
+   HIPCHK (hipStreamSynchronize (s->stream));
+   HIPCHK (hipGetLastError ());
+   return NKP_OK;
+}
+
+extern "C" int nkp_spmv_level0 (nkp_solver *s, const double *x0, const double *b, double *y)
+{
+   if (!s || !x0 || !y) return fail (NKP_EINVAL, "nkp_spmv_level0: NULL argument");
+   if (!s->A.dg_tile0) return fail (NKP_EINVAL, "nkp_spmv_level0: the matrix has no keys for x in level-0 order (tuning step_order)");
+   HIPCHK (hipSetDevice (s->device));
+   const size_t bytes = (size_t) s->n * sizeof (double);
+   HIPCHK (hipMemcpyAsync (s->t1, x0, bytes, hipMemcpyHostToDevice, s->stream));
+   if (b) HIPCHK (hipMemcpyAsync (s->r, b, bytes, hipMemcpyHostToDevice, s->stream));
+   launch_diag_spmv (s->A, s->t1, s->t2, b ? s->r : nullptr, b ? 1 : 0, s->stream, true);
    HIPCHK (hipMemcpyAsync (y, s->t2, bytes, hipMemcpyDeviceToHost, s->stream));
    HIPCHK (hipStreamSynchronize (s->stream));
    HIPCHK (hipGetLastError ());
@@ -183,7 +201,7 @@
          else if (which == 1) apply_precond_once (s, s->t1, s->t2);
          else if (which == 2) {
             const int src = arnoldi_hand_over (s, arg, step_ev.ev);
-            if (src) { s->ml.entered = 0; return src; }
+            if (src) { ml_leave (s->ml); return src; }
          }
          else if (which == 5) valgrad_time_launch (s, arg);
          else if (which == 6) valprod_time_launch (s, arg);
@@ -198,7 +216,7 @@
    }
    (void) hipEventDestroy (e0);
    (void) hipEventDestroy (e1);
-   s->ml.entered = 0;
-   HIPCHK (hipGetLastError ());
-   return NKP_OK;
-}
+   ml_leave (s->ml);
+   HIPCHK (hipGetLastError ());
+   return NKP_OK;
+}
diff --git a/nk_ocn_tracer_jacobian_precond_amd/csrc/krylov.hip b/nk_ocn_tracer_jacobian_precond_amd/csrc/krylov.hip
--- a/nk_ocn_tracer_jacobian_precond_amd/csrc/krylov.hip
+++ b/nk_ocn_tracer_jacobian_precond_amd/csrc/krylov.hip
@@ -60,8 +60,11 @@
    double *zj = s->Z + (int64_t) j * ld;
    const double *vj = s->vf32 ? s->vcur : s->V + (int64_t) j * ld;
    if (s->ml.entered) {
-      ml_finish (s->ml, zj, s->stream);
-      spmv_op (s, zj, s->w, nullptr, 0);
+      const double *z0 = ml_finish (s->ml, zj, s->stream);
+      if (z0) {
+         s->z_level0 = true;
+         launch_diag_spmv (s->A, z0, s->w, nullptr, 0, s->stream, true);
+      } else spmv_op (s, zj, s->w, nullptr, 0);
       return;
    }
    if (s->equil) {
@@ -116,13 +119,19 @@
           !s->ml.lev.empty () && s->ml.lev[0].n == s->n;
 }
 
+bool step_z_level0 (const nkp_solver *s)
+{
+   return (s->tune.step_order & 16) && (s->tune.step_glue & 8) && s->opt.krylov == NKP_KRYLOV_FGMRES && s->A.dg_tile0 && step_enters_cycle (s);
+}
+
 int arnoldi_hand_over (nkp_solver *s, int j, hipEvent_t ev)
 {
    const bool early = ev && (s->tune.step_glue & 8) && j + 1 < s->m && !s->dist.on && !s->equil && s->steps_now == 1;
    arnoldi_apply (s, j);
    arnoldi_column (s, j, early ? s->hpin : nullptr);
    if (early) HIPCHK (hipEventRecord (ev, s->stream));
-   if (early && step_enters_cycle (s)) ml_enter (s->ml, s->w, s->misc_dev () + 1, s->V + (int64_t) (j + 1) * s->ld, s->stream);
+   if (early && step_enters_cycle (s))
+      ml_enter (s->ml, s->w, s->misc_dev () + 1, s->V + (int64_t) (j + 1) * s->ld, s->stream, step_z_level0 (s) ? s->Z + (int64_t) (j + 1) * s->ld : nullptr);
    else arnoldi_normalise (s, j);
    if (early) HIPCHK (hipEventSynchronize (ev));
    else {
@@ -194,7 +203,8 @@
    hipStream_t st = s->stream;
    const int64_t n = s->n;
    int rc;
-   s->ml.entered = 0;
+   ml_leave (s->ml);
+   s->z_level0 = false;
    spmv_op (s, s->x, s->r, s->b, 1);
    double r2 = 0.0;
    if ((rc = dot_host (s, s->r, s->r, &r2))) return rc;
@@ -239,7 +249,8 @@
    fg_back_substitute (F);
    for (int i = 0; i < k; i++) s->hpin[i] = F.y[i];
    HIPCHK (hipMemcpyAsync (s->y_dev (), s->hpin, (size_t) k * sizeof (double), hipMemcpyHostToDevice, st));
-   launch_axpy_multi (s->Z, s->ld, k, s->y_dev (), s->x, s->n, st);
+   if (s->z_level0 && k > 1) launch_axpy_multi_level0 (s->ml.perm0, s->Z, s->ld, 1, k, s->y_dev (), s->x, s->n, st);
+   else launch_axpy_multi (s->Z, s->ld, k, s->y_dev (), s->x, s->n, st);
    HIPCHK (hipStreamSynchronize (st));
    if (F.breakdown_in_cycle) {
       int rc;
@@ -264,13 +275,13 @@
       if ((rc = fg_restart (s, F))) return rc;
       if (F.finished) break;
       for (;;) {
-         if ((rc = arnoldi_hand_over (s, F.j, ev.ev))) { s->ml.entered = 0; return rc; }
+         if ((rc = arnoldi_hand_over (s, F.j, ev.ev))) { ml_leave (s->ml); return rc; }
          if (s->comm_failed) return fail (NKP_ECOMM, "nkp_solve: a collective of the distributed solve failed (Arnoldi step %d)", F.its + 1);
          if (fg_post_step (s, F)) break;
       }
       if ((rc = fg_end_cycle (s, F))) return rc;
    }
-   s->ml.entered = 0;
+   ml_leave (s->ml);
    HIPCHK (hipGetLastError ());
    *iters_out = F.its;
    *relres_out = F.relres;
diff --git a/nk_ocn_tracer_jacobian_precond_amd/csrc/mlcycle.hip b/nk_ocn_tracer_jacobian_precond_amd/csrc/mlcycle.hip
--- a/nk_ocn_tracer_jacobian_precond_amd/csrc/mlcycle.hip
+++ b/nk_ocn_tracer_jacobian_precond_amd/csrc/mlcycle.hip
@@ -103,6 +103,7 @@
 void ml_apply (MlHierarchy &H, const double *r, double *z, hipStream_t st, const MlSmoothHook *hook)
 {
    MlLevel &V = H.lev[0];
+   ml_leave (H);
    launch_gather (H.perm0, r, V.b, V.n, st);
    H.hook = hook;
    ml_cycle (H, 0, st);
@@ -110,9 +111,14 @@
    launch_scatter (H.perm0, V.xnow (), z, V.n, st);
 }
 
-void ml_enter (MlHierarchy &H, const double *w, const double *inv, double *vnext, hipStream_t st)
-{
-   MlLevel &V = H.lev[0];
+void ml_enter (MlHierarchy &H, const double *w, const double *inv, double *vnext, hipStream_t st, double *z0)
+{
+   MlLevel &V = H.lev[0];
+   ml_leave (H);
+   if (z0 && ml_level0_hookable (H)) {
+      H.x0_home = V.x;
+      V.x = z0;
+   }
    launch_cycle_entry (H.perm0, w, inv, vnext, V.b, V.x, V.n, st);
    H.entered = ML_FILLED;
    if (H.lev.size () >= 2 && H.tail_from != 0) {
@@ -123,13 +129,30 @@
    }
 }
 
-void ml_finish (MlHierarchy &H, double *z, hipStream_t st)
+const double *ml_finish (MlHierarchy &H, double *z, hipStream_t st)
 {
    MlLevel &V = H.lev[0];
    const int started = H.entered;
    H.entered = ML_FRESH;
    ml_cycle (H, 0, st, started);
-   launch_scatter (H.perm0, V.xnow (), z, V.n, st);
+   if (!H.x0_home) {
+      launch_scatter (H.perm0, V.xnow (), z, V.n, st);
+      return nullptr;
+   }
+   double *z0 = V.x;
+   if (V.xnow () != z0) launch_copy (V.xnow (), z0, V.n, st);
+   ml_leave (H);
+   return z0;
+}
+
+void ml_leave (MlHierarchy &H)
+{
+   H.entered = ML_FRESH;
+   if (H.x0_home) {
+      H.lev[0].x = H.x0_home;
+      H.lev[0].cur[0] = H.lev[0].cur[1] = 0;
+      H.x0_home = nullptr;
+   }
 }
 
 int ml_batch_prepare (MlHierarchy &H, int K)
diff --git a/nk_ocn_tracer_jacobian_precond_amd/csrc/multilevel.h b/nk_ocn_tracer_jacobian_precond_amd/csrc/multilevel.h
--- a/nk_ocn_tracer_jacobian_precond_amd/csrc/multilevel.h
+++ b/nk_ocn_tracer_jacobian_precond_amd/csrc/multilevel.h
@@ -41,6 +41,7 @@
    const MlSmoothHook *hook = nullptr;
    int hook_left = 0;
    int entered = 0;
+   double *x0_home = nullptr;
    int *perm0 = nullptr;
    double *coarse_inv = nullptr;
    float *coarse_invf = nullptr;
@@ -78,8 +79,9 @@
 inline int ml_level0_sweeps (const MlHierarchy &H) { return 0 >= H.coarse_from ? H.nu_coarse : H.nu; }
 inline bool ml_level0_hookable (const MlHierarchy &H) { return H.lev.size () >= 2 && H.tail_from != 0 && ml_level0_sweeps (H) > 0; }
 void ml_apply (MlHierarchy &H, const double *r, double *z, hipStream_t st, const MlSmoothHook *hook = nullptr);
-void ml_enter (MlHierarchy &H, const double *w, const double *inv, double *vnext, hipStream_t st);
-void ml_finish (MlHierarchy &H, double *z, hipStream_t st);
+void ml_enter (MlHierarchy &H, const double *w, const double *inv, double *vnext, hipStream_t st, double *z0 = nullptr);
+const double *ml_finish (MlHierarchy &H, double *z, hipStream_t st);
+void ml_leave (MlHierarchy &H);
 int ml_batch_prepare (MlHierarchy &H, int K);
 void ml_apply_batch (MlHierarchy &H, int K, const double *r, double *z, hipStream_t st);
 void ml_apply_batch_split (MlHierarchy &H, int K, const double *const *src, double *z, double *const *dst, hipStream_t st, const double *src_scale = nullptr);
diff --git a/nk_ocn_tracer_jacobian_precond_amd/csrc/multilevel.hip b/nk_ocn_tracer_jacobian_precond_amd/csrc/multilevel.hip
--- a/nk_ocn_tracer_jacobian_precond_amd/csrc/multilevel.hip
+++ b/nk_ocn_tracer_jacobian_precond_amd/csrc/multilevel.hip
@@ -519,6 +519,7 @@
 
 void ml_free (MlHierarchy &H)
 {
+   ml_leave (H);
    for (MlLevel &V : H.lev) {
       void *ptrs[] = { V.L.rowptr, V.L.colind, V.L.val, V.L.valf, V.B.fac_tf, V.L.rowblk, V.L.codes, V.L.dict, V.L.dict_ptr, V.L.dg_ptr, V.L.dg_key, V.L.dg_voff, V.L.dg_val, V.L.dg_tile, V.L.dg_gptr, V.L.dg_grp, V.B.blk_start, V.B.fac, V.B.grp_b0, V.B.grp_nb, V.B.grp_maxlen, V.B.grp_base, V.B.grp_row0, V.B.col_slot, V.B.fac_t, V.B.gs_rb_ptr, V.B.gs_rb, V.B.wave_desc, V.B.grp_tile, V.cmap, V.rptr, V.ridx, V.x, V.x2, V.b, V.r, V.bx, V.bx2, V.bb, V.br };
       for (void *p : ptrs)
diff --git a/nk_ocn_tracer_jacobian_precond_amd/csrc/nkp_dev.h b/nk_ocn_tracer_jacobian_precond_amd/csrc/nkp_dev.h
--- a/nk_ocn_tracer_jacobian_precond_amd/csrc/nkp_dev.h
+++ b/nk_ocn_tracer_jacobian_precond_amd/csrc/nkp_dev.h
@@ -4,6 +4,7 @@
 
 #include "../../include/nkp.h"
 #include "col_plan.h"
+#include "diag_layout.h"
 #include "tuning.h"
 
 #include <type_traits>
@@ -14,19 +15,6 @@
 #define NKP_MAX_K 512
 #define NKP_SPMV_LDS_NNZ 2048
 #define NKP_SPMV_MAX_ROWS 256
-
-struct alignas (16) DgTile {
-   int row0, rows;
-   int kl0, len;
-   int k0, nk;
-   int g0, ng;
-   long long voff;
-};
-struct DgGroup {
-   int key0;
-   int slots;
-};
-#define DG_RUN_MAX 5
 
 struct CsrDev {
    int64_t n = 0, nnz = 0;
@@ -49,6 +37,9 @@
    DgGroup *dg_grp = nullptr;
    int dg_ntile = 0, dg_ncol = 0, dg_nkey = 0, dg_ngrp = 0;
    int64_t dg_nval = 0;
+   DgTile *dg_tile0 = nullptr;
+   DgGroup *dg_grp0 = nullptr;
+   int dg_ngrp0 = 0, dg_ntile0 = 0;
    const nkp_tuning *tune = nullptr;
 };
 
@@ -64,7 +55,9 @@
                 size_t *device_bytes, hipStream_t st);
 void launch_diag_fill (const CsrDev &L, hipStream_t st);
 void launch_diag_residual (const CsrDev &L, int tile0, int tile1, const double *x, const double *b, double *y, hipStream_t st);
-void launch_diag_spmv (const CsrDev &A, const double *x, double *y, const double *b, int mode, hipStream_t st);
+void launch_diag_spmv (const CsrDev &A, const double *x, double *y, const double *b, int mode, hipStream_t st, bool x_level0 = false);
+int diag_build_level0 (CsrDev &A, const int *h_blk_start, int ncol, const int *d_perm0, size_t *device_bytes, hipStream_t st);
+void diag_drop_level0 (CsrDev &A, size_t *device_bytes);
 void build_rowblocks_host (int64_t n, const int *rowptr, int **rowblk_out, int *nrowblk_out);
 
 void launch_value_gradient (int K, int nk, const CsrDev &A, const double *lam, const double *x, double alpha, int accumulate, double *g, hipStream_t st);
@@ -242,6 +235,7 @@
 void launch_update_w (const void *V, int v_f32, int64_t ld, int k, const double *h, double *w, int64_t n, double *partial, double *out_nrm2, hipStream_t st);
 void launch_scale_to (const double *x, const double *alpha_dev, double *y, float *yf, int64_t n, hipStream_t st);
 void launch_axpy_multi (const double *Z, int64_t ld, int k, const double *c, double *x, int64_t n, hipStream_t st);
+void launch_axpy_multi_level0 (const int *perm, const double *Z, int64_t ld, int k0, int k, const double *c, double *x, int64_t n, hipStream_t st);
 void launch_dot (const double *x, const double *y, int64_t n, double *partial, double *out, hipStream_t st);
 void launch_berr (const double *r, const double *den, int64_t n, double *partial, double *out, hipStream_t st);
 void launch_count_entries (const double *x, int64_t n, double *partial, double *out, hipStream_t st);
diff --git a/nk_ocn_tracer_jacobian_precond_amd/csrc/refactor_api.hip b/nk_ocn_tracer_jacobian_precond_amd/csrc/refactor_api.hip
--- a/nk_ocn_tracer_jacobian_precond_amd/csrc/refactor_api.hip
+++ b/nk_ocn_tracer_jacobian_precond_amd/csrc/refactor_api.hip
@@ -133,6 +133,7 @@
       s->ml = H2;
       s->device_bytes += s->ml.device_bytes;
       s->device_bytes -= rf_free_maps (W);
+      build_level0_keys (s);
       if (s->dist.smooth && (!ml_level0_hookable (s->ml) || smooth_build_lists (s) != 0)) {
          rc = -3;
          snprintf (err, errlen, "the index lists of the fine-level exchange could not be rebuilt for the new hierarchy");
diff --git a/nk_ocn_tracer_jacobian_precond_amd/csrc/solver.hip b/nk_ocn_tracer_jacobian_precond_amd/csrc/solver.hip
--- a/nk_ocn_tracer_jacobian_precond_amd/csrc/solver.hip
+++ b/nk_ocn_tracer_jacobian_precond_amd/csrc/solver.hip
@@ -15,6 +15,7 @@
 {
    if (!s) return;
    if (s->borrowed) {
+      ml_leave (s->ml);
       void *own[] = { s->V, s->vcur, s->Z, s->w, s->r, s->x, s->b, s->t1, s->t2, s->p1, s->p2, s->eqtmp, s->partial, s->dscal, s->dint };
       for (void *p : own)
          if (p) (void) hipFree (p);
@@ -39,7 +40,7 @@
    s->batch_members.clear ();
    for (double *p : { s->bvin, s->bz, s->bw })
       if (p) (void) hipFree (p);
-   void *ptrs[] = { s->A.rowptr, s->A.colind, s->A.val, s->A.rowblk, s->A.codes, s->A.dict, s->A.dict_ptr, s->A.dg_ptr, s->A.dg_key, s->A.dg_voff, s->A.dg_vald, s->A.dg_tile, s->A.dg_gptr, s->A.dg_grp, s->B.blk_start, s->B.fac, s->B.grp_b0, s->B.grp_nb, s->B.grp_maxlen, s->B.grp_base, s->B.grp_row0, s->B.col_slot, s->B.fac_t, s->B.gs_rb_ptr, s->B.gs_rb, s->V, s->vcur, s->Z, s->w, s->r,
+   void *ptrs[] = { s->A.rowptr, s->A.colind, s->A.val, s->A.rowblk, s->A.codes, s->A.dict, s->A.dict_ptr, s->A.dg_ptr, s->A.dg_key, s->A.dg_voff, s->A.dg_vald, s->A.dg_tile, s->A.dg_gptr, s->A.dg_grp, s->A.dg_tile0, s->A.dg_grp0, s->B.blk_start, s->B.fac, s->B.grp_b0, s->B.grp_nb, s->B.grp_maxlen, s->B.grp_base, s->B.grp_row0, s->B.col_slot, s->B.fac_t, s->B.gs_rb_ptr, s->B.gs_rb, s->V, s->vcur, s->Z, s->w, s->r,
                     s->x, s->b, s->t1, s->t2, s->p1, s->p2, s->partial, s->dscal, s->dint, s->rscale, s->rinv, s->eqtmp };
    for (void *p : ptrs)
       if (p) (void) hipFree (p);
@@ -105,6 +106,8 @@
    if (!strcmp (key, "spmv_diag")) return s->A.dg_vald ? 1 : 0;
    if (!strcmp (key, "spmv_diag_bytes"))
       return s->A.dg_vald ? 8 * s->A.dg_nval + (int64_t) s->A.dg_ntile * (int64_t) sizeof (DgTile) + (int64_t) s->A.dg_ngrp * (int64_t) sizeof (DgGroup) + 16 * s->n : 0;
+   if (!strcmp (key, "step_z_level0")) return step_z_level0 (s) ? 1 : 0;
+   if (!strcmp (key, "spmv_level0_bytes")) return s->A.dg_tile0 ? (int64_t) s->A.dg_ntile0 * (int64_t) sizeof (DgTile) + (int64_t) (s->A.dg_ngrp0 ? s->A.dg_ngrp0 : 1) * (int64_t) sizeof (DgGroup) : 0;
    if (!strcmp (key, "precond_bytes")) return s->opt.precond == NKP_PRECOND_NONE ? 16 * s->n : (int64_t) (2 * s->B.P + 1) * 8 * s->n + 16 * s->n;
    if (!strcmp (key, "device_bytes")) return (int64_t) s->device_bytes;
    if (!strcmp (key, "precond_steps")) return s->precond_steps;
diff --git a/nk_ocn_tracer_jacobian_precond_amd/csrc/solver_impl.h b/nk_ocn_tracer_jacobian_precond_amd/csrc/solver_impl.h
--- a/nk_ocn_tracer_jacobian_precond_amd/csrc/solver_impl.h
+++ b/nk_ocn_tracer_jacobian_precond_amd/csrc/solver_impl.h
@@ -65,6 +65,7 @@
    bool vf32 = false;
    double *vcur = nullptr;
    double *V = nullptr, *Z = nullptr, *w = nullptr, *r = nullptr, *x = nullptr, *b = nullptr, *t1 = nullptr, *t2 = nullptr;
+   bool z_level0 = false;
    double *p1 = nullptr, *p2 = nullptr;
    int precond_steps = 1;
    int steps_now = 1;
@@ -233,6 +234,8 @@
 NKP_PRIVATE void arnoldi_apply (nkp_solver *s, int j);
 NKP_PRIVATE void arnoldi_orthogonalise (nkp_solver *s, int j);
 NKP_PRIVATE int arnoldi_hand_over (nkp_solver *s, int j, hipEvent_t ev);
+NKP_PRIVATE bool step_z_level0 (const nkp_solver *s);
+NKP_PRIVATE void build_level0_keys (nkp_solver *s);
 struct NKP_PRIVATE StepEvent {
    hipEvent_t ev = nullptr;
    int make (const nkp_solver *s);
diff --git a/nk_ocn_tracer_jacobian_precond_amd/csrc/tuning.cpp b/nk_ocn_tracer_jacobian_precond_amd/csrc/tuning.cpp
--- a/nk_ocn_tracer_jacobian_precond_amd/csrc/tuning.cpp
+++ b/nk_ocn_tracer_jacobian_precond_amd/csrc/tuning.cpp
@@ -58,7 +58,7 @@
    t->spmv_variant = 4; t->spmv_compress = 0; t->spmv_pipe_min = 1024; t->spmv_run = 1; t->spmv_wgs = 256;
    t->rhs_batch = 1; t->batch_spmv_rows = 1; t->precond_steps = 0; t->equil = -1; t->dist_overlap = 1; t->dist_ras = 1; t->dist_one_reduce = 0; t->force_dist = 0; t->setup_threads = 0; t->plan_times = 0;
    t->ml_drop_intertracer = 0; t->ml_huge_from = -1; t->dist_ras_rings = 1; t->ml_diag = 32; t->spmv_diag = 32;
-   t->ml_lane_fused = 50000; t->dist_smooth_exchange = 0; t->step_glue = 12;
+   t->ml_lane_fused = 50000; t->dist_smooth_exchange = 0; t->step_glue = 12; t->step_order = 16;
 }
 
 const nkp_tuning &nkp_builtin_tuning ()
@@ -105,6 +105,7 @@
    ENV_INT ("NKP_ML_LANE_FUSED", ml_lane_fused);
    ENV_INT ("NKP_DIST_SMOOTH_EXCHANGE", dist_smooth_exchange);
    ENV_INT ("NKP_STEP_GLUE", step_glue);
+   ENV_INT ("NKP_STEP_ORDER", step_order);
 #undef ENV_INT
 #undef ENV_POS
 #undef ENV_FLAG
diff --git a/nk_ocn_tracer_jacobian_precond_amd/solver.py b/nk_ocn_tracer_jacobian_precond_amd/solver.py
--- a/nk_ocn_tracer_jacobian_precond_amd/solver.py
+++ b/nk_ocn_tracer_jacobian_precond_amd/solver.py
@@ -24,7 +24,7 @@
     "nkp_dist_plan_copy", "nkp_dist_plan_free", "nkp_ml_level_array", "nkp_default_tuning", "nkp_solve_batch_device",
     "nkp_refactor", "nkp_refactor_device", "nkp_refactor_dist", "nkp_refactor_dist_device", "nkp_transpose", "nkp_transpose_dist",
     "nkp_value_gradient", "nkp_value_gradient_device",
-    "nkp_values_product", "nkp_values_product_device", "nkp_solve_tangent_device", "nkp_matrix_array",
+    "nkp_values_product", "nkp_values_product_device", "nkp_solve_tangent_device", "nkp_matrix_array", "nkp_spmv_level0",
 ]
 
 _ALLREDUCE_FN = C.CFUNCTYPE(C.c_int, C.c_void_p, C.c_void_p, C.c_int, C.c_int, C.c_void_p)
@@ -53,7 +53,7 @@
         ("setup_threads", C.c_int), ("plan_times", C.c_int), ("ml_drop_intertracer", C.c_int), ("dist_one_reduce", C.c_int), ("ml_huge_from", C.c_int), ("col_ldsres_min", C.c_int), ("col_sort_groups", C.c_int), ("batch_spmv_rows", C.c_int),
         ("dist_ras_rings", C.c_int), ("ml_diag", C.c_int), ("spmv_diag", C.c_int), ("ml_lane_fused", C.c_int),
         ("dist_smooth_exchange", C.c_int),
-        ("step_glue", C.c_int),
+        ("step_glue", C.c_int), ("step_order", C.c_int),
     ]
 
 
@@ -97,6 +97,7 @@
     lib.nkp_solve_batch_device.argtypes = [vp, C.c_int, vp, vp, C.c_int64, f64p, C.POINTER(C.c_int), f64p]
     lib.nkp_spmv.argtypes = [vp, f64p, f64p]
     lib.nkp_spmv_device.argtypes = [vp, vp, vp]
+    lib.nkp_spmv_level0.argtypes = [vp, f64p, f64p, f64p]
     lib.nkp_precond_apply.argtypes = [vp, f64p, f64p]
     lib.nkp_multi_dot.argtypes = [vp, f64p, C.c_int64, C.c_int, f64p, f64p]
     lib.nkp_time_kernel.argtypes = [vp, C.c_int, C.c_int, C.c_int, f64p]
@@ -400,6 +401,13 @@
         self._check(self._lib.nkp_spmv(self._h, _p(x, C.c_double), _p(y, C.c_double)))
         return y
 
+    def spmv_level0(self, x0, b=None):
+        x0 = np.ascontiguousarray(x0, np.float64)
+        b = None if b is None else np.ascontiguousarray(b, np.float64)
+        y = np.empty(self.n)
+        self._check(self._lib.nkp_spmv_level0(self._h, _p(x0, C.c_double), None if b is None else _p(b, C.c_double), _p(y, C.c_double)))
+        return y
+
     def spmv_device(self, d_x, d_y):
         self._check(self._lib.nkp_spmv_device(self._h, C.c_void_p(d_x), C.c_void_p(d_y)))
 
```

After: 34.50 million, median of 6. No clear change (+0.9%).
